# ut-vision/Rot-MVGaze

Hardware: AMD Instinct MI355X
Metric: multi-view samples/sec (fwd+bwd), BxVx3x224x224 (higher is better)
Workload: dtype f32; 1 GPU; C3: ResNet-50, V=4, B=128 per GPU, 3x224x224, fwd+loss+bwd; backbone=ResNet-50, views=4, batch_per_gpu=128, global_batch=128, image=3x224x224, parallelism=dp1, weights=random init, seed 0 (kaiming-normal convs, default Linear), rccl_ranks=1, step_launch=eager: every kernel queued from Python

## Files before the change

### include/rotmvgaze.h

```cpp
#ifndef ROTMVGAZE_H
#define ROTMVGAZE_H

#include <stddef.h>
#include <stdint.h>

#ifdef __cplusplus
extern "C" {
#endif

#define MVG_ABI_VERSION 10

int mvg_abi_version(void);
const char *mvg_last_error(void);
int mvg_device_cus(void);
int mvg_set_scratch(void *ptr, size_t bytes, void *stream);
size_t mvg_scratch_bytes(void);
void *mvg_stream_create_low_priority(void);
int mvg_set_reserved_cus(int n);

enum {
  MVG_K_CONV_FPROP = 0, MVG_K_CONV_DGRAD = 1, MVG_K_CONV_WGRAD = 2, MVG_K_WGRAD_REDUCE = 3,
  MVG_K_BN_FINALIZE = 4, MVG_K_BN_APPLY = 5, MVG_K_BN_BWD_REDUCE = 6, MVG_K_BN_BWD_APPLY = 7,
  MVG_K_POOL = 8, MVG_K_LAYOUT = 9, MVG_K_LINEAR_FPROP = 10, MVG_K_LINEAR_DGRAD = 11,
  MVG_K_LINEAR_WGRAD = 12, MVG_K_ROTCAT = 13, MVG_K_COLSUM = 14, MVG_K_LOSS = 15,
// ... 126 lines not shown
                           int inverse, void *stream);
int mvg_relative_rotation(const float *rot, const int32_t *vi, const int32_t *vj, float *rel,
                          int batch, int views, int dirs, void *stream);

int mvg_rotcat_fwd(const float *img_feat , const float *feat ,
                   const float *rel , const int32_t *view_of,
                   const int32_t *src_of, float *x , int batch, int dirs,
                   int cf, int nvec, void *stream);
int mvg_rotcat_bwd(const float *dx, const float *rel, const int32_t *src_of, float *dfeat, int batch,
                   int dirs, int cf, int nvec, void *stream);
int mvg_rotcat_ext_fwd(const float *img_feat, const float *feat, const float *rel_apply,
                       const float *rel_append, const int32_t *view_of, const int32_t *src_of,
                       float *x, int ld, int batch, int dirs, int cf, int nvec, void *stream);
int mvg_rotcat_ext_bwd(const float *dx, int ld, const float *rel, const int32_t *src_of, float *dfeat,
                       int batch, int dirs, int cf, int nvec, void *stream);
int mvg_ibn_scales(const float *a , const float *feat ,
                   const int32_t *view_of, const int32_t *src_of, float *running_mean, int training,
                   float momentum, float eps, float *scales, int batch, int dirs, int nvec,
                   void *stream);
int mvg_paircat_fwd(const float *a, const float *feat, const float *rel, const float *scales,
                    const int32_t *view_of, const int32_t *src_of, float *x, int batch, int dirs,
                    int nvec, void *stream);
int mvg_paircat_bwd(const float *dx, const float *rel, const float *scales, const int32_t *src_of,
                    float *da_dir, float *dfeat, int batch, int dirs, int nvec, void *stream);
int mvg_segment_sum(const float *x, int64_t row_stride, int width, const int32_t *seg_of, float *out,
                    int batch, int dirs, int segments, int accumulate, void *stream);

int mvg_axpby(const float *x, float *y, float a, float b, int64_t n, void *stream);
int mvg_scale_by(const float *x, const float *scale, float *out, int64_t n, void *stream);

int mvg_linear_skinny_fwd(const float *x, const float *w, const float *bias, float *y, int rows, int k,
                          int nout, void *stream);
int mvg_linear_skinny_bwd(const float *dy, const float *x, const float *w, const float *mask, float *dx,
                          float *dw, float *db, int rows, int k, int nout, int accumulate, float *dx_absmax, void *stream);

int mvg_adam_step(float *param, const float *grad, float *exp_avg, float *exp_avg_sq, int64_t n, float lr,
                  float beta1, float beta2, float eps, float weight_decay, int step, void *stream);
int mvg_adam_step_dev(float *param, const float *grad, float *exp_avg, float *exp_avg_sq, int64_t n, const float *lr_dev,
                      float *state3, float beta1, float beta2, float eps, float weight_decay, void *stream);

int mvg_gaze_angular_loss(const float *pred, const float *gt, int n, float row_weight,
                          float *loss, int accumulate, float *dpred, float *theta_out, void *stream);

int mvg_gaze_lp_loss(const float *pred, const float *label, int n, int p, float *loss, float *dpred, void *stream);
int mvg_gaze_angular_loss_multi(const float *pred, const float *gt, int iters, int dirs, int batch, const float *host_weights,
                                float *loss, float *dpred, void *stream);

int mvg_mt19937_seed(uint32_t *host_state , uint64_t seed);
int64_t mvg_pair_index_build(uint32_t *host_state, const int64_t *host_file_rows, int n_files,
                             int camera_tag, int64_t *host_out , int64_t capacity);


int mvg_cast_weights_bf16(const mvg_conv_desc *d, const float *w, int cin_src, void *w_krsc, void *w_crsk,
                          void *stream);
int mvg_conv_fprop_bf16(const mvg_conv_desc *d, const void *x, const void *wgt, void *y, const float *bias,
                        int relu, float *stats, void *stream);
int mvg_conv_stats_partials_bf16(const mvg_conv_desc *d, int32_t *out_rows_per_partial);
int mvg_conv_fprop_bf16_affine(const mvg_conv_desc *d, const void *x, const void *wgt, void *out, const float *scale,
                               const float *shift, const void *residual, int relu, void *stream);
int mvg_conv_dgrad_bf16(const mvg_conv_desc *d, const void *dy, const void *wgt_crsk, void *dx,
                        const void *mask, const void *addend, void *stream);
int mvg_conv_dgrad_bn_partials_bf16(const mvg_conv_desc *d);
int mvg_conv_dgrad_bf16_bnreduce(const mvg_conv_desc *d, const void *dy, const void *wgt_crsk, void *dx, const void *addend,
                                 const void *bn_y, const uint8_t *bn_bits, const float *bn_mean, const float *bn_invstd,
                                 const float *relu_scale, const float *relu_shift, float *partials, float *s1, float *s2,
                                 float *dgamma, float *dbeta, int accumulate, void *stream);
int mvg_stem_rowwindow_bf16(const float *x_nchw, void *xw, int64_t images, int h, int w, void *stream);
int mvg_stem_fprop_bf16(const mvg_conv_desc *d, const void *xw, const void *w_fold, void *y, float *stats, void *stream);
int mvg_stem_wgrad_splits_bf16(const mvg_conv_desc *d);
int mvg_stem_wgrad_bf16(const mvg_conv_desc *d, const void *xw, const void *dy, float *dw_fold, float *workspace, int splits,
                        int accumulate, void *stream);
int mvg_conv_wgrad_bf16(const mvg_conv_desc *d, const void *x, const void *dy, float *dw, float *workspace,
                        int splits, int accumulate, void *stream);
int mvg_conv_wgrad_splits_bf16(const mvg_conv_desc *d);
int mvg_conv_wgrad_bf16_slabs(const mvg_conv_desc *d, const void *x, const void *dy, float *workspace, int splits, void *stream);
int mvg_linear_fprop_mixed(const float *x, const void *w_bf16, const float *bias, int relu, float *y, int rows, int fin,
                           int fout, void *stream);
int mvg_linear_dgrad_mixed(const float *dy, const void *wt_bf16, const float *mask, const float *addend, float *dx,
                           int rows, int fin, int fout, void *stream);
int mvg_linear_wgrad_mixed(const float *x, const float *dy, float *dw, float *db, int rows, int fin, int fout,
                           float *workspace, int splits, int accumulate, void *stream);
int mvg_bn_apply_bf16(const uint16_t *y, const float *scale, const float *shift, const uint16_t *residual,
                      const float *res_scale, const float *res_shift, int relu, uint16_t *out, int groups,
                      int64_t rows_per_group, int c, void *stream);
int mvg_bn_bwd_reduce_bf16(const uint16_t *g, const uint16_t *act, const uint16_t *y, const float *mean,
                           const float *invstd, const float *relu_scale, const float *relu_shift, int groups,
                           int64_t rows_per_group, int c, float *s1, float *s2, float *dgamma, float *dbeta,
                           int accumulate, float *workspace, uint16_t *dz_out, void *stream);
int mvg_bn_bwd_apply_bf16(const uint16_t *g, const uint16_t *act, const uint16_t *y, const float *mean,
                          const float *invstd, const float *gamma, const float *s1, const float *s2,
                          const float *relu_scale, const float *relu_shift, int groups, int64_t rows_per_group,
                          int c, uint16_t *dy, uint16_t *dz_out, void *stream);
int mvg_bn_relu_maxpool_fwd_bf16(const uint16_t *y, const float *scale, const float *shift, uint16_t *pooled,
                                 uint8_t *argmax, int groups, int n_per_group, int h, int w, int c, int ho,
                                 int wo, void *stream);
int mvg_bn_relu_maxpool_bwd_reduce_bf16(const uint16_t *g_pooled, const uint8_t *argmax, const uint16_t *y,
                                        const float *mean, const float *invstd, const float *scale,
                                        const float *shift, int groups, int n_per_group, int h, int w, int c,
                                        int ho, int wo, float *s1, float *s2, float *dgamma, float *dbeta,
                                        int accumulate, float *workspace, void *stream);
int mvg_bn_relu_maxpool_bwd_apply_bf16(const uint16_t *g_pooled, const uint8_t *argmax, const uint16_t *y,
                                       const float *mean, const float *invstd, const float *gamma,
                                       const float *scale, const float *shift, const float *s1,
                                       const float *s2, int groups, int n_per_group, int h, int w, int c,
                                       int ho, int wo, uint16_t *dy, void *stream);
int mvg_avgpool_fwd_bf16(const uint16_t *x, float *y, int n, int hw, int c, void *stream);
int mvg_avgpool_bwd_bf16(const float *dy, uint16_t *dx, int n, int hw, int c, void *stream);
int mvg_nchw_to_nhwc8_bf16(const float *src, uint16_t *dst, int n, int c, int h, int w, void *stream);
int mvg_preprocess_u8hwc_resize_bf16(const uint8_t *src, uint16_t *dst, int n, int h, int w, int oh, int ow, float mean0,
                                     float mean1, float mean2, float std0, float std1, float std2, int swap_rb,
                                     void *stream);

int mvg_split_f32(const float *x, void *out_sp, int64_t n, float scale, void *stream);
int mvg_merge_sp(const void *x_sp, float *out, int64_t n, float inv_scale, void *stream);
int mvg_split_weights(const mvg_conv_desc *d, const float *w, void *w_krsc_sp, void *w_crsk_sp, float *stat2, void *items_dev,
                      void *stream);
int mvg_weights_prep_batch(const void *items_dev, int n, int mode, int blocks_per_item , void *stream);
int mvg_conv_stats_partials_split(const mvg_conv_desc *d, int32_t *rows_per_partial);
int mvg_conv_fprop_split(const mvg_conv_desc *d, const void *x_sp, const float *x_sinv, const void *w_sp, const float *w_sinv,
                         float *y, float *stats, void *stream);
int mvg_conv_fprop_split_affine(const mvg_conv_desc *d, const void *x_sp, const float *x_sinv, const void *w_sp, const float *w_sinv,
                                void *out, int out_sp, const float *scale, const float *shift, const void *residual,
                                int residual_sp, int relu, void *stream);
int mvg_conv_dgrad_split(const mvg_conv_desc *d, const void *dy_sp, const float *dy_sinv, const void *w_crsk_sp,
                         const float *w_sinv, float *dx, const float *addend, const void *relu_mask_sp, void *stream);
int mvg_bn_apply_split(const float *y, const float *scale, const float *shift, const void *residual, int residual_sp,
                       const float *res_scale, const float *res_shift, int relu, void *out_sp, uint8_t *relu_bits,
                       int groups, int64_t rows_per_group, int c, void *stream);
int mvg_bn_bwd_reduce_split(const float *g, const uint8_t *relu_bits, const float *y, const float *mean, const float *invstd,
                            const float *relu_scale, const float *relu_shift, int groups, int64_t rows_per_group, int c,
                            float *s1, float *s2, float *dgamma, float *dbeta, int accumulate, float *workspace,
                            float *dz_out, float *mx, const float *gamma, float *dy_sinv, void *stream);
int mvg_bn_bwd_apply_split(const float *g, const float *y, const float *mean, const float *invstd, const float *gamma,
                           const float *s1, const float *s2, const float *relu_scale, const float *relu_shift,
                           int groups, int64_t rows_per_group, int c, void *dy_sp, const float *mx, float *dy_sinv,
                           int dy_sinv_ready, void *stream);
int mvg_bn_relu_maxpool_fwd_split(const float *y, const float *scale, const float *shift, void *pooled_sp,
                                  uint8_t *argmax, int groups, int n_per_group, int h, int w, int c, int ho, int wo,
                                  void *stream);
int mvg_avgpool_fwd_split(const void *x_sp, float *y, int n, int hw, int c, void *stream);
int mvg_conv_dgrad_bn_partials_split(const mvg_conv_desc *d);
int mvg_conv_dgrad_split_bnreduce(const mvg_conv_desc *d, const void *dy_sp, const float *dy_sinv, const void *w_crsk_sp,
                                  const float *w_sinv, float *dx, const float *addend, const float *bn_y, const uint8_t *bn_bits,
                                  const float *bn_mean, const float *bn_invstd, const float *relu_scale, const float *relu_shift,
                                  float *partials, float *s1, float *s2, float *dgamma, float *dbeta, int accumulate,
                                  float *mx, const float *bn_gamma, float *dx_dy_sinv, void *stream);
int mvg_stem_rowwindow_split(const float *x_nhwc4, void *xw_sp, int64_t images, int h, int w, void *stream);
int mvg_stem_rowwindow_split_nchw(const float *x_nchw, void *xw_sp, int64_t images, int h, int w, void *stream);
int mvg_stem_fprop_split(const mvg_conv_desc *d, const void *xw_sp, const void *w_sp, const float *w_sinv, float *y, float *stats,
                         void *stream);
int mvg_stem_wgrad_splits_split(const mvg_conv_desc *d);
int mvg_stem_wgrad_split(const mvg_conv_desc *d, const void *xw_sp, const void *dy_sp, const float *dy_sinv, float *dw_rw,
                         float *workspace, int splits, int accumulate, void *stream);
int mvg_bn_relu_maxpool_bwd_reduce_split(const float *g_pooled, const uint8_t *argmax, const float *y, const float *mean,
                                         const float *invstd, const float *scale, const float *shift, int groups,
                                         int n_per_group, int h, int w, int c, int ho, int wo, float *s1, float *s2,
                                         float *dgamma, float *dbeta, int accumulate, float *workspace, float *mx, const float *gamma,
                                         float *dy_sinv, void *stream);
int mvg_bn_relu_maxpool_bwd_apply_split(const float *g_pooled, const uint8_t *argmax, const float *y, const float *mean,
                                        const float *invstd, const float *gamma, const float *scale, const float *shift,
                                        const float *s1, const float *s2, int groups, int n_per_group, int h, int w, int c,
                                        int ho, int wo, void *dy_sp, const float *mx, float *dy_sinv, int dy_sinv_ready, void *stream);
int mvg_conv_wgrad_splits_split(const mvg_conv_desc *d);
int mvg_conv_wgrad_split(const mvg_conv_desc *d, const void *x_sp, const void *dy_sp, const float *dy_sinv, float *dw,
                         float *workspace, int splits, int accumulate, void *stream);
int mvg_conv_wgrad_split_slabs(const mvg_conv_desc *d, const void *x_sp, const void *dy_sp, const float *dy_sinv, float *workspace,
                               int splits, void *stream);
int mvg_wgrad_reduce_batch(const float *const *host_slabs, float *const *host_dw, const int64_t *host_n, const int32_t *host_splits,
                           const int32_t *host_accumulate, int n, void *stream);

int mvg_absmax_multi(const float *const *host_ptrs, const int64_t *host_counts, float *const *host_out_slots, int n, void *stream);
int mvg_fuse_build_split(const float *img_feat, const float *feat, const float *rel, const int32_t *row_img, const int32_t *row_src_f,
                         const int32_t *row_src_h, void *xf_sp, void *xh_sp, const float *am_img, const float *am_feat,
                         float *xf_sinv, float *xh_sinv, int rows, int cf, int nvec, void *stream);
int mvg_fuse_unbuild(const float *dxh, const float *dxn, const float *rel, const int32_t *seg, const int32_t *vi, float *dfeat, float *da,
                     int da_accumulate, int segments, int views, int dirs, int batch, int cf, int nvec, float *absmax, void *stream);
int mvg_linear_fprop_split(int rows, int fin, int fout, const void *x_sp, const float *x_sinv, const void *w_sp, const float *w_sinv,
                           const float *bias, int relu, void *out, int out_sp, float *out_sinv, const float *bias_absmax,
                           float *out_absmax, void *stream);
int mvg_linear_dgrad_split(int rows, int fin, int fout, const void *dy_sp, const float *dy_sinv, const void *wt_sp, const float *w_sinv,
                           float *dx, const float *addend, const void *relu_mask_sp, float *out_absmax, void *stream);
int mvg_linear_wgrad_split(int rows, int fin, int fout, const void *x_sp, const float *x_sinv, const void *dy_sp, const float *dy_sinv,
                           float *dw, float *workspace, int splits, int accumulate, void *stream);
int mvg_split_colsum(const float *g, int rows, int cols, const float *absmax, void *out_sp, float *out_sinv, float *db, int accumulate,
                     void *stream);

#ifdef __cplusplus
}
#endif
#endif
```

### rot-mvgaze_amd/_lib.py

```python
from __future__ import annotations

import ctypes as C
import os

_HERE = os.path.dirname(os.path.abspath(__file__))
LIB_PATH = os.path.join(_HERE, "csrc", "librotmvgaze_hip.so")

K_FAMILIES = 18
ABI_VERSION = 10


class ConvDesc(C.Structure):
    _fields_ = [(n, C.c_int32) for n in
                ("groups", "n", "h", "w", "cin", "cout", "r", "s", "stride", "pad", "ho", "wo")]

    @classmethod
    def make(cls, groups, n, h, w, cin, cout, k, stride, pad):
        ho = (h + 2 * pad - k) // stride + 1
        wo = (w + 2 * pad - k) // stride + 1
        return cls(groups, n, h, w, cin, cout, k, k, stride, pad, ho, wo)

    @classmethod
    def linear(cls, rows, fin, fout):
        return cls(1, rows, 1, 1, fin, fout, 1, 1, 1, 0, 1, 1)


class ProfEntry(C.Structure):
    _fields_ = [("launches", C.c_int64), ("ms", C.c_double), ("flops", C.c_double), ("bytes", C.c_double)]


_P = C.c_void_p
_I = C.c_int
_I64 = C.c_int64
_F = C.c_float
_D = C.POINTER(ConvDesc)

SIGNATURES = {
    "mvg_abi_version": (_I, []),
    "mvg_last_error": (C.c_char_p, []),
    "mvg_device_cus": (_I, []),
    "mvg_set_scratch": (_I, [_P, C.c_size_t, _P]),
    "mvg_scratch_bytes": (C.c_size_t, []),
    "mvg_set_reserved_cus": (_I, [_I]),
    "mvg_stream_create_low_priority": (_P, []),
    "mvg_prof_enable": (_I, [_I]),
    "mvg_prof_reset": (_I, []),
    "mvg_prof_collect": (_I, [C.POINTER(ProfEntry)]),
    "mvg_prof_family_name": (C.c_char_p, [_I]),
    "mvg_conv_fprop": (_I, [_D, _P, _P, _P, _P, _I, _P, _P]),
    "mvg_conv_fprop_affine": (_I, [_D, _P, _P, _P, _P, _P, _P, _I, _P]),
    "mvg_conv_stats_partials": (_I, [_D, C.POINTER(C.c_int32)]),
    "mvg_conv_dgrad": (_I, [_D, _P, _P, _P, _P, _P, _P]),
    "mvg_conv_wgrad": (_I, [_D, _P, _P, _P, _P, _I, _I, _P]),
    "mvg_conv_wgrad_splits": (_I, [_D]),
    "mvg_linear_wgrad": (_I, [_P, _P, _P, _P, _I, _I, _I, _P, _I, _I, _P]),
    "mvg_fuser_fprop": (_I, [_P, _P, _P, _P, _P, _P, _P, _I, _P, _I, _I, _I, _I, _I, _I, _P, C.c_size_t, _P]),
    "mvg_fuser_wgrad": (_I, [_P, _P, _P, _P, _P, _P, _P, _P, _I, _I, _I, _I, _I, _I, _P, _I, _I, _P]),
    "mvg_linear_workspace_floats": (C.c_size_t, [_I, _I, _I]),
    "mvg_linear_fprop": (_I, [_P, _P, _P, _I, _P, _I, _I, _I, _P, C.c_size_t, _P]),
    "mvg_linear_dgrad": (_I, [_P, _P, _P, _P, _P, _I, _I, _I, _P, C.c_size_t, _P]),
    "mvg_bn_finalize": (_I, [_P, _I, _I, _I, _I64, _I, _P, _P, _P, _P, _F, _F, _P, _P, _P, _P, _P]),
    "mvg_bn_eval_affine": (_I, [_I, _I, _P, _P, _P, _P, _F, _P, _P, _P]),
    "mvg_bn_apply": (_I, [_P, _P, _P, _P, _P, _P, _I, _P, _I, _I64, _I, _P]),
    "mvg_bn_bwd_reduce": (_I, [_P, _P, _P, _P, _P, _P, _P, _I, _I64, _I, _P, _P, _P, _P, _I, _P, _P, _P]),
    "mvg_split_f32": (_I, [_P, _P, _I64, _F, _P]),
    "mvg_merge_sp": (_I, [_P, _P, _I64, _F, _P]),
    "mvg_split_weights": (_I, [_D, _P, _P, _P, _P, _P, _P]),
    "mvg_weights_prep_batch": (_I, [_P, _I, _I, _I, _P]),
    "mvg_conv_stats_partials_split": (_I, [_D, C.POINTER(C.c_int32)]),
    "mvg_conv_fprop_split": (_I, [_D, _P, _P, _P, _P, _P, _P, _P]),
    "mvg_conv_fprop_split_affine": (_I, [_D, _P, _P, _P, _P, _P, _I, _P, _P, _P, _I, _I, _P]),
    "mvg_conv_dgrad_split": (_I, [_D, _P, _P, _P, _P, _P, _P, _P, _P]),
    "mvg_bn_apply_split": (_I, [_P, _P, _P, _P, _I, _P, _P, _I, _P, _P, _I, _I64, _I, _P]),
    "mvg_bn_bwd_apply_split": (_I, [_P, _P, _P, _P, _P, _P, _P, _P, _P, _I, _I64, _I, _P, _P, _P, _I, _P]),
    "mvg_bn_bwd_reduce_split": (_I, [_P, _P, _P, _P, _P, _P, _P, _I, _I64, _I, _P, _P, _P, _P, _I, _P, _P, _P, _P, _P, _P]),
    "mvg_bn_relu_maxpool_fwd_split": (_I, [_P, _P, _P, _P, _P, _I, _I, _I, _I, _I, _I, _I, _P]),
    "mvg_avgpool_fwd_split": (_I, [_P, _P, _I, _I, _I, _P]),
    "mvg_stem_rowwindow_split": (_I, [_P, _P, _I64, _I, _I, _P]),
    "mvg_stem_rowwindow_split_nchw": (_I, [_P, _P, _I64, _I, _I, _P]),
    "mvg_stem_fprop_split": (_I, [_D, _P, _P, _P, _P, _P, _P]),
    "mvg_stem_wgrad_splits_split": (_I, [_D]),
    "mvg_stem_wgrad_split": (_I, [_D, _P, _P, _P, _P, _P, _I, _I, _P]),
    "mvg_bn_relu_maxpool_bwd_reduce_split": (_I, [_P, _P, _P, _P, _P, _P, _P, _I, _I, _I, _I, _I, _I, _I, _P, _P, _P, _P, _I, _P, _P, _P, _P, _P]),
    "mvg_bn_relu_maxpool_bwd_apply_split": (_I, [_P, _P, _P, _P, _P, _P, _P, _P, _P, _P, _I, _I, _I, _I, _I, _I, _I, _P, _P, _P, _I, _P]),
    "mvg_conv_dgrad_bn_partials_split": (_I, [_D]),
    "mvg_conv_dgrad_split_bnreduce": (_I, [_D, _P, _P, _P, _P, _P, _P, _P, _P, _P, _P, _P, _P, _P, _P, _P, _P, _P, _I, _P, _P, _P, _P]),
    "mvg_conv_wgrad_splits_split": (_I, [_D]),
    "mvg_conv_wgrad_split": (_I, [_D, _P, _P, _P, _P, _P, _I, _I, _P]),
    "mvg_conv_wgrad_split_slabs": (_I, [_D, _P, _P, _P, _P, _I, _P]),
    "mvg_wgrad_reduce_batch": (_I, [C.POINTER(C.c_void_p), C.POINTER(C.c_void_p), C.POINTER(C.c_int64), C.POINTER(C.c_int32),
                                    C.POINTER(C.c_int32), _I, _P]),
    "mvg_bn_apply_bits": (_I, [_P, _P, _P, _P, _P, _P, _P, _P, _I, _I64, _I, _P]),
    "mvg_bn_bwd_reduce_bits": (_I, [_P, _P, _P, _P, _P, _I, _I64, _I, _P, _P, _P, _P, _I, _P, _P, _P]),
    "mvg_bn_apply_bits_bf16": (_I, [_P, _P, _P, _P, _P, _P, _P, _P, _I, _I64, _I, _P]),
    "mvg_bn_bwd_reduce_bits_bf16": (_I, [_P, _P, _P, _P, _P, _I, _I64, _I, _P, _P, _P, _P, _I, _P, _P, _P]),
    "mvg_bn_bwd_workspace_floats": (C.c_size_t, [_I, _I64, _I]),
    "mvg_bn_bwd_apply": (_I, [_P, _P, _P, _P, _P, _P, _P, _P, _P, _P, _I, _I64, _I, _P, _P, _P]),
    "mvg_maxpool3x3s2_fwd": (_I, [_P, _P, _P, _I, _I, _I, _I, _I, _I, _P]),
    "mvg_maxpool3x3s2_bwd": (_I, [_P, _P, _P, _I, _I, _I, _I, _I, _I, _P]),
    "mvg_bn_relu_maxpool_fwd": (_I, [_P, _P, _P, _P, _P, _I, _I, _I, _I, _I, _I, _I, _P]),
    "mvg_bn_relu_maxpool_bwd_reduce": (_I, [_P, _P, _P, _P, _P, _P, _P, _I, _I, _I, _I, _I, _I, _I, _P, _P, _P, _P, _I, _P,
                                            _P]),
    "mvg_bn_relu_maxpool_bwd_apply": (_I, [_P, _P, _P, _P, _P, _P, _P, _P, _P, _P, _I, _I, _I, _I, _I, _I, _I, _P, _P]),
    "mvg_bn_eval_bwd": (_I, [_P, _P, _P, _P, _P, _P, _P, _P, _P, _F, _I, _I64, _I, _P, _P, _P, _P, _I, _P, _P]),
    "mvg_bn_eval_bwd_workspace_floats": (C.c_size_t, [_I, _I64, _I]),
    "mvg_bn_relu_maxpool_eval_bwd": (_I, [_P, _P, _P, _P, _P, _P, _P, _P, _F, _I, _I, _I, _I, _I, _I, _I, _P, _P, _P, _I, _P,
                                          _P]),
    "mvg_avgpool_fwd": (_I, [_P, _P, _I, _I, _I, _P]),
    "mvg_avgpool_bwd": (_I, [_P, _P, _I, _I, _I, _P]),
    "mvg_nchw_to_nhwc4": (_I, [_P, _P, _I, _I, _I, _I, _P]),
    "mvg_nhwc4_to_nchw": (_I, [_P, _P, _I, _I, _I, _I, _P]),
    "mvg_preprocess_u8hwc": (_I, [_P, _P, _I, _I, _I, _F, _F, _F, _F, _F, _F, _I, _P]),
    "mvg_gaze_lp_loss": (_I, [_P, _P, _I, _I, _P, _P, _P]),
    "mvg_preprocess_u8hwc_resize": (_I, [_P, _P, _I, _I, _I, _I, _I, _F, _F, _F, _F, _F, _F, _I, _P]),
    "mvg_multi_erase_nchw": (_I, [_P, _P, _P, _I, _I, _I, _I, _I, _P]),
    "mvg_rotation_matrix_2d": (_I, [_P, _P, _I, _I, _P]),
    "mvg_relative_rotation": (_I, [_P, _P, _P, _P, _I, _I, _I, _P]),
    "mvg_rotcat_fwd": (_I, [_P, _P, _P, _P, _P, _P, _I, _I, _I, _I, _P]),
    "mvg_rotcat_bwd": (_I, [_P, _P, _P, _P, _I, _I, _I, _I, _P]),
    "mvg_rotcat_ext_fwd": (_I, [_P, _P, _P, _P, _P, _P, _P, _I, _I, _I, _I, _I, _P]),
    "mvg_rotcat_ext_bwd": (_I, [_P, _I, _P, _P, _P, _I, _I, _I, _I, _P]),
    "mvg_ibn_scales": (_I, [_P, _P, _P, _P, _P, _I, _F, _F, _P, _I, _I, _I, _P]),
    "mvg_paircat_fwd": (_I, [_P, _P, _P, _P, _P, _P, _P, _I, _I, _I, _P]),
    "mvg_paircat_bwd": (_I, [_P, _P, _P, _P, _P, _P, _I, _I, _I, _P]),
    "mvg_segment_sum": (_I, [_P, _I64, _I, _P, _P, _I, _I, _I, _I, _P]),
    "mvg_axpby": (_I, [_P, _P, _F, _F, _I64, _P]),
    "mvg_scale_by": (_I, [_P, _P, _P, _I64, _P]),
    "mvg_linear_skinny_fwd": (_I, [_P, _P, _P, _P, _I, _I, _I, _P]),
    "mvg_linear_skinny_bwd": (_I, [_P, _P, _P, _P, _P, _P, _P, _I, _I, _I, _I, _P, _P]),
    "mvg_adam_step": (_I, [_P, _P, _P, _P, _I64, _F, _F, _F, _F, _F, _I, _P]),
    "mvg_gaze_angular_loss": (_I, [_P, _P, _I, _F, _P, _I, _P, _P, _P]),
    "mvg_gaze_angular_loss_multi": (_I, [_P, _P, _I, _I, _I, C.POINTER(C.c_float), _P, _P, _P]),
    "mvg_adam_step_dev": (_I, [_P, _P, _P, _P, _I64, _P, _P, _F, _F, _F, _F, _P]),
    "mvg_absmax_multi": (_I, [C.POINTER(C.c_void_p), C.POINTER(C.c_int64), C.POINTER(C.c_void_p), _I, _P]),
    "mvg_fuse_build_split": (_I, [_P, _P, _P, _P, _P, _P, _P, _P, _P, _P, _P, _P, _I, _I, _I, _P]),
    "mvg_fuse_unbuild": (_I, [_P, _P, _P, _P, _P, _P, _P, _I, _I, _I, _I, _I, _I, _I, _P, _P]),
    "mvg_linear_fprop_split": (_I, [_I, _I, _I, _P, _P, _P, _P, _P, _I, _P, _I, _P, _P, _P, _P]),
    "mvg_linear_dgrad_split": (_I, [_I, _I, _I, _P, _P, _P, _P, _P, _P, _P, _P, _P]),
    "mvg_linear_wgrad_split": (_I, [_I, _I, _I, _P, _P, _P, _P, _P, _P, _I, _I, _P]),
    "mvg_split_colsum": (_I, [_P, _I, _I, _P, _P, _P, _P, _I, _P]),
    "mvg_cast_weights_bf16": (_I, [_D, _P, _I, _P, _P, _P]),
    "mvg_conv_fprop_bf16": (_I, [_D, _P, _P, _P, _P, _I, _P, _P]),
    "mvg_conv_stats_partials_bf16": (_I, [_D, C.POINTER(C.c_int32)]),
    "mvg_conv_fprop_bf16_affine": (_I, [_D, _P, _P, _P, _P, _P, _P, _I, _P]),
    "mvg_conv_dgrad_bf16": (_I, [_D, _P, _P, _P, _P, _P, _P]),
    "mvg_conv_dgrad_bn_partials_bf16": (_I, [_D]),
    "mvg_conv_dgrad_bf16_bnreduce": (_I, [_D, _P, _P, _P, _P, _P, _P, _P, _P, _P, _P, _P, _P, _P, _P, _P, _I, _P]),
    "mvg_conv_wgrad_bf16": (_I, [_D, _P, _P, _P, _P, _I, _I, _P]),
    "mvg_stem_rowwindow_bf16": (_I, [_P, _P, _I64, _I, _I, _P]),
    "mvg_stem_fprop_bf16": (_I, [_D, _P, _P, _P, _P, _P]),
    "mvg_stem_wgrad_splits_bf16": (_I, [_D]),
    "mvg_stem_wgrad_bf16": (_I, [_D, _P, _P, _P, _P, _I, _I, _P]),
    "mvg_conv_wgrad_splits_bf16": (_I, [_D]),
    "mvg_conv_wgrad_bf16_slabs": (_I, [_D, _P, _P, _P, _I, _P]),
    "mvg_linear_fprop_mixed": (_I, [_P, _P, _P, _I, _P, _I, _I, _I, _P]),
    "mvg_linear_dgrad_mixed": (_I, [_P, _P, _P, _P, _P, _I, _I, _I, _P]),
    "mvg_linear_wgrad_mixed": (_I, [_P, _P, _P, _P, _I, _I, _I, _P, _I, _I, _P]),
    "mvg_bn_apply_bf16": (_I, [_P, _P, _P, _P, _P, _P, _I, _P, _I, _I64, _I, _P]),
    "mvg_bn_bwd_reduce_bf16": (_I, [_P, _P, _P, _P, _P, _P, _P, _I, _I64, _I, _P, _P, _P, _P, _I, _P, _P, _P]),
    "mvg_bn_bwd_apply_bf16": (_I, [_P, _P, _P, _P, _P, _P, _P, _P, _P, _P, _I, _I64, _I, _P, _P, _P]),
    "mvg_bn_relu_maxpool_fwd_bf16": (_I, [_P, _P, _P, _P, _P, _I, _I, _I, _I, _I, _I, _I, _P]),
    "mvg_bn_relu_maxpool_bwd_reduce_bf16": (_I, [_P, _P, _P, _P, _P, _P, _P, _I, _I, _I, _I, _I, _I, _I, _P, _P, _P, _P, _I,
                                                 _P, _P]),
    "mvg_bn_relu_maxpool_bwd_apply_bf16": (_I, [_P, _P, _P, _P, _P, _P, _P, _P, _P, _P, _I, _I, _I, _I, _I, _I, _I, _P, _P]),
    "mvg_avgpool_fwd_bf16": (_I, [_P, _P, _I, _I, _I, _P]),
    "mvg_avgpool_bwd_bf16": (_I, [_P, _P, _I, _I, _I, _P]),
    "mvg_nchw_to_nhwc8_bf16": (_I, [_P, _P, _I, _I, _I, _I, _P]),
    "mvg_preprocess_u8hwc_resize_bf16": (_I, [_P, _P, _I, _I, _I, _I, _I, _F, _F, _F, _F, _F, _F, _I, _P]),
    "mvg_mt19937_seed": (_I, [_P, C.c_uint64]),
    "mvg_pair_index_build": (_I64, [_P, _P, _I, _I, _P, _I64]),
}

_lib = None


def lib() -> C.CDLL:
    global _lib
    if _lib is not None:
        return _lib
    if not os.path.exists(LIB_PATH):
        raise RuntimeError(
            f"{LIB_PATH} not found: the HIP extension is required (python rot-mvgaze_amd/csrc/build.py); "
            "this package has no CPU fallback")
    try:
        l = C.CDLL(LIB_PATH, mode=C.RTLD_GLOBAL)
    except OSError as e:
        raise RuntimeError(f"failed to load {LIB_PATH}: {e}") from e
    for name, (res, args) in SIGNATURES.items():
        fn = getattr(l, name)
        fn.restype = res
        fn.argtypes = args
    if l.mvg_abi_version() != ABI_VERSION:
        raise RuntimeError(f"librotmvgaze_hip.so ABI {l.mvg_abi_version()} != binding ABI {ABI_VERSION}")
    _lib = l
    return l


def check(rc: int, what: str = "") -> None:
    if rc != 0:
        msg = lib().mvg_last_error()
        raise RuntimeError(f"librotmvgaze_hip {what} failed (rc={rc}): {msg.decode() if msg else '?'}")
```

### rot-mvgaze_amd/backbone.py

```python
from __future__ import annotations

import os
from typing import Callable, Dict, List, Optional

import torch

from . import ops
from ._lib import ConvDesc
from .arch import BackboneSpec, ConvSpec, backbone_spec

Tensor = torch.Tensor
BN_EPS, BN_MOMENTUM = 1e-5, 0.1
IMAGE_MEAN, IMAGE_STD = (0.485, 0.456, 0.406), (0.229, 0.224, 0.225)


class GradSink:

    def view(self, p: torch.nn.Parameter) -> Tensor:
        raise NotImplementedError

    def accumulate(self, p: torch.nn.Parameter) -> bool:
        raise NotImplementedError

    def publish(self, ps: List[torch.nn.Parameter]) -> None:
        raise NotImplementedError


class _Unit:
    __slots__ = ("spec", "desc", "x_in", "y", "out", "mean", "invstd", "relu", "rows", "w", "trained", "pool",
                 "relu_affine", "fused_s12", "relu_bits", "split", "stem_rw")

    def __init__(self):
        self.split = False
        self.stem_rw = False
        self.relu_bits = None
        self.fused_s12 = None


class Backbone:
    _guard_scale = 1
    _debug_units: Optional[list] = None

    def __init__(self, depth: int, params: Dict[str, Tensor], prefix: str = "_feat_extractor.0."):
        self.spec: BackboneSpec = backbone_spec(depth, prefix)
        self.p = params
        self.fc_dim = self.spec.fc_dim
        self.overlap_wgrad = True
        self.overlap_head = True
        self.wgrad_low_priority = True
        self.grad_streams: List[torch.cuda.Stream] = []
        self._wg_stream: Optional[torch.cuda.Stream] = None
        self._wg_low = True
        self.act_dtype = torch.float32
        self.relu_bits = True
        self.split = os.environ.get("MVG_SPLIT", "1") != "0"
        self.fuse_bn_split = True
        self.stem_rowwindow = True
        self.split_eval = True
        self.bf16_fold_eval = True
        self._wprep_infer_ok = False
        self._wk_cache: Dict[str, tuple] = {}
        self.batch_weight_prep = True
        self._wprep: Optional[Dict[str, tuple]] = None
        self._wprep_state = None
        self._wprep_versions = None
        self._wg_defer: Optional[list] = None
        self._split_now = self.split
        self._stem_rw = False
        self._stem_w8 = None

    @property
    def bf16(self) -> bool:
        return self.act_dtype == torch.bfloat16

    def _weight(self, c: ConvSpec) -> Tensor:
        w = self.p[c.name + ".weight"]
        if c.cin == 3:
            w4 = torch.zeros(c.cout, c.k, c.k, 4, dtype=torch.float32, device=w.device)
            w4[..., :3].copy_(w.detach().permute(0, 2, 3, 1))
            return w4
        assert w.is_contiguous(memory_format=torch.channels_last) or (c.k == 1 and w.is_contiguous()), \
            f"{c.name}.weight must be channels_last (KRSC)"
        return w.detach()

    def _prepare_weights(self, dev, reuse: bool = False) -> Dict[str, tuple]:
        mode = 0 if self.bf16 else 1
        stem_rw = self._stem_rw
        convs = [c for c in self.spec.all_convs() if not (mode == 1 and c.cin == 3 and not stem_rw)]
        key = (mode, stem_rw, str(dev), tuple(self.p[c.name + ".weight"].data_ptr() for c in convs))
        if self._wprep_state is None or self._wprep_state[0] != key:
            out, rows = {}, []
            wstat = torch.zeros(len(convs), 2, dtype=torch.float32, device=dev)
            self._stem_w8 = None
            for ci, c in enumerate(convs):
                wsrc = self.p[c.name + ".weight"]
                assert wsrc.is_contiguous(memory_format=torch.channels_last) or (c.k == 1 and wsrc.is_contiguous())
                rs = c.k * c.k
                if mode == 1 and c.cin == 3:
                    assert c.k == 7
                    self._stem_w8 = torch.zeros(c.cout, 7, 8, 4, dtype=torch.float32, device=dev)
                    wk = ops.sp_empty(c.cout, 7 * 32, device=dev)
                    wk.sinv = wstat[ci, 1:2]
                    out[c.name] = (wk, None)
                    rows.append([self._stem_w8.data_ptr(), wk.data_ptr(), 0, c.cout | (7 << 32), 32 | (32 << 32), wstat[ci].data_ptr()])
                    continue
                if mode == 0 and c.cin == 3 and stem_rw:
                    assert c.k == 7
                    self._stem_w8 = torch.zeros(2 * c.cout, 7, 16, 4, dtype=torch.float32, device=dev)
                    wk = torch.empty(2 * c.cout, 7, 1, 64, dtype=torch.bfloat16, device=dev)
                    out[c.name] = (wk, None)
                    rows.append([self._stem_w8.data_ptr(), wk.data_ptr(), 0, (2 * c.cout) | (7 << 32), 64 | (64 << 32), wstat[ci].data_ptr()])
                    continue
                if mode == 1:
                    wk = ops.sp_empty(c.cout, rs * c.cin, device=dev)
                    wt = ops.sp_empty(c.cin, rs * c.cout, device=dev)
                    wk.sinv = wt.sinv = wstat[ci, 1:2]
                    cin_pad = c.cin
                else:
                    cin_pad = 8 if c.cin == 3 else c.cin
                    wk = torch.empty(c.cout, c.k, c.k, cin_pad, dtype=torch.bfloat16, device=dev)
                    wt = None if c.cin == 3 else torch.empty(cin_pad, c.k, c.k, c.cout, dtype=torch.bfloat16, device=dev)
                out[c.name] = (wk, wt)
                rows.append([wsrc.data_ptr(), wk.data_ptr(), wt.data_ptr() if wt is not None else 0, c.cout | (rs << 32),
                             c.cin | (cin_pad << 32), wstat[ci].data_ptr()])
            table = torch.tensor(rows, dtype=torch.int64).to(dev)
            self._wprep_state = (key, out, table, len(rows), mode, wstat)
        elif (reuse and self._wprep_infer_ok and
              self._wprep_versions == tuple(self.p[c.name + ".weight"]._version for c in self.spec.all_convs())):
            return self._wprep_state[1]
        _, out, table, n, mode, wstat = self._wprep_state
        self._wprep_infer_ok = reuse
        if mode == 1:
            wstat.zero_()
            if self._stem_w8 is not None:
                self._stem_w8[:, :, 1:, :3].copy_(self.p[self.spec.stem.name + ".weight"].detach().permute(0, 2, 3, 1))
        elif self._stem_w8 is not None:
            wsrc, co = self.p[self.spec.stem.name + ".weight"].detach().permute(0, 2, 3, 1), self.spec.stem.cout
            self._stem_w8[:co, :, 1:8, :3].copy_(wsrc)
            self._stem_w8[co:, :, 3:10, :3].copy_(wsrc)
        ops.weights_prep_batch(table, n, mode)
        self._wprep_versions = tuple(self.p[c.name + ".weight"]._version for c in self.spec.all_convs())
        return out

    def invalidate_weight_cache(self):
        self._wk_cache.clear()
        self._wprep_infer_ok = False

    def bn_count_buffers(self) -> List[Tensor]:
        return [self.p[c.bn + ".num_batches_tracked"] for c in self.spec.all_convs()]

    def _unit_fwd(self, c: ConvSpec, x: Tensor, G: int, N: int, H: int, W: int, training: bool, relu: bool,
                  residual: Optional[Tensor], tape: Optional[list], pool: bool = False, residual_affine=None,
                  defer_apply: bool = False):
        bf = self.bf16
        cin = (8 if bf else 4) if c.cin == 3 else c.cin
        d = ConvDesc.make(G, N, H, W, cin, c.cout, c.k, c.stride, c.pad)
        dev = x.device
        sp_out = self._split_now and training and not bf
        sp_in = sp_out and c.cin != 3
        stem_rw = c.cin == 3 and self._stem_rw and (sp_out or bf)
        if (sp_in or bf or stem_rw) and self._wprep is not None:
            w, w_t = self._wprep[c.name]
        elif sp_in:
            wsrc = self.p[c.name + ".weight"].detach()
            assert wsrc.is_contiguous(memory_format=torch.channels_last) or (c.k == 1 and wsrc.is_contiguous())
            w, w_t = ops.split_weights(d, wsrc, need_transposed=tape is not None)
        elif bf:
            wsrc = self.p[c.name + ".weight"].detach()
            assert wsrc.is_contiguous(memory_format=torch.channels_last) or (c.k == 1 and wsrc.is_contiguous())
            w, w_t = ops.cast_weights_bf16(d, wsrc, c.cin, need_transposed=(tape is not None and c.cin != 3))
        else:
            w, w_t = self._weight(c), None
        y = torch.empty(G, N, d.ho, d.wo, c.cout, dtype=self.act_dtype, device=dev)
        rows = N * d.ho * d.wo
        gamma, beta = self.p[c.bn + ".weight"].detach(), self.p[c.bn + ".bias"].detach()
        rm, rv = self.p[c.bn + ".running_mean"], self.p[c.bn + ".running_var"]
        aff = torch.empty(4, G, c.cout, dtype=torch.float32, device=dev)
        mean, invstd, scale, shift = aff[0], aff[1], aff[2], aff[3]

        def fprop(stats_buf):
            if stem_rw and bf:
                ops.stem_fprop_bf16(d, x, w, y, stats_buf)
            elif stem_rw:
                ops.stem_fprop_split(d, x, w, y, stats_buf)
            elif sp_in:
                ops.conv_fprop_split(d, x, w, y, stats_buf)
            else:
                ops.conv_fprop(d, x, w, y, None, False, stats_buf)
        if training:
            if stem_rw and bf:
                P, rpp = ops.conv_stats_partials(ConvDesc.make(G, N, d.ho, d.wo // 2, 64, 2 * c.cout, 1, 1, 0), True)
                P *= 2
            elif stem_rw:
                P, rpp = ops.conv_stats_partials_split(ConvDesc.make(G, N, d.ho, d.wo, 32, c.cout, 1, 1, 0))
            else:
                P, rpp = ops.conv_stats_partials_split(d) if sp_in else ops.conv_stats_partials(d, bf)
            stats = torch.empty(G, P, 2, c.cout, dtype=torch.float32, device=dev)
            fprop(stats)
            ops.bn_finalize(stats, G, P, rpp, rows, c.cout, gamma, beta, rm, rv, BN_MOMENTUM, BN_EPS, mean, invstd,
                            scale, shift)
        elif tape is None and not bf:
            ops.bn_eval_affine(1, c.cout, gamma, beta, rm, rv, BN_EPS, scale[:1], shift[:1])
            sp_eval = self._split_now and self.split_eval
            if sp_eval and c.cin != 3:
                wsrc = self.p[c.name + ".weight"].detach()
                assert wsrc.is_contiguous(memory_format=torch.channels_last) or (c.k == 1 and wsrc.is_contiguous())
                hit = self._wk_cache.get(c.name)
                if hit is not None and hit[0] == wsrc.data_ptr() and hit[1] == wsrc._version:
                    wk = hit[2]
                else:
                    wk, _ = ops.split_weights(d, wsrc, need_transposed=False)
                    self._wk_cache[c.name] = (wsrc.data_ptr(), wsrc._version, wk)
                out = ops.sp_empty(G, N, d.ho, d.wo, c.cout, device=dev) if relu else y
                ops.conv_fprop_split_affine(d, x, wk, out, scale[0], shift[0], residual, relu)
                return out
            ops.conv_fprop_affine(d, x, w, y, scale[0], shift[0], residual, relu)
            if pool:
                pooled, am = self._pool_plain(y, G, N, d.ho, d.wo, c.cout)
                return (ops.split_f32(pooled), am) if sp_eval else (pooled, am)
            return y
        elif tape is None and bf and self.bf16_fold_eval and not pool:
            ops.bn_eval_affine(1, c.cout, gamma, beta, rm, rv, BN_EPS, scale[:1], shift[:1])
            ops.conv_fprop_bf16_affine(d, x, w, y, scale[0], shift[0], residual, relu)
            if self._debug_units is not None:
                self._debug_units.append((c.name, x, residual, y))
            return y
        else:
            fprop(None)
            ops.bn_eval_affine(G, c.cout, gamma, beta, rm, rv, BN_EPS, scale, shift)
        keep = tape is not None
        if defer_apply:
            assert not relu and residual is None and not pool
            if keep:
                u = _Unit()
                u.spec, u.desc, u.x_in, u.y, u.out, u.mean, u.invstd, u.relu, u.rows, u.w = \
                    c, d, x, y, None, mean, invstd, False, rows, (w_t if (bf or sp_in) else w)
                u.trained = training
                u.split = sp_in
                u.relu_affine = None
                tape.append(u)
            return y, (scale, shift)
        if pool:
            assert relu and residual is None
            hp, wp_ = (d.ho + 2 - 3) // 2 + 1, (d.wo + 2 - 3) // 2 + 1
            argmax = torch.empty(G, N, hp, wp_, c.cout, dtype=torch.uint8, device=dev)
            if sp_out:
                out = ops.sp_empty(G, N, hp, wp_, c.cout, device=dev)
                ops.bn_relu_maxpool_fwd_split(y, scale, shift, out, argmax, G, N, d.ho, d.wo, c.cout, hp, wp_)
            else:
                out = torch.empty(G, N, hp, wp_, c.cout, dtype=self.act_dtype, device=dev)
                ops.bn_relu_maxpool_fwd(y, scale, shift, out, argmax, G, N, d.ho, d.wo, c.cout, hp, wp_)
            if self._debug_units is not None and tape is None and not training:
                self._debug_units.append((c.name, x, y, out))
        elif sp_out:
            out = ops.sp_empty(G, N, d.ho, d.wo, c.cout, device=dev)
            bits = ops.bn_apply_split(y, scale, shift, residual, relu, out, G, rows, c.cout, residual_affine,
                                      want_bits=keep and relu and residual is not None)
        else:
            out = torch.empty_like(y) if keep else y
            bits = None
            if keep and relu and residual is not None and self.relu_bits:
                bits = ops.bn_apply_bits(y, scale, shift, residual, out, G, rows, c.cout, residual_affine)
            else:
                ops.bn_apply(y, scale, shift, residual, relu, out, G, rows, c.cout, residual_affine)
        if keep:
            u = _Unit()
            u.spec, u.desc, u.x_in, u.y, u.out, u.mean, u.invstd, u.relu, u.rows, u.w = \
                c, d, x, y, (None if pool else out), mean, invstd, relu, rows, (w_t if (bf or sp_in) else w)
            u.trained = training
            u.split = sp_in
            u.stem_rw = stem_rw
            u.relu_affine = (scale, shift) if (relu and residual is None and not pool) else None
            if pool:
                u.pool = (argmax, scale, shift, d.ho, d.wo, hp, wp_)
            else:
                u.relu_bits = bits
            tape.append(u)
        return (out, argmax) if pool else out

    @staticmethod
    def _pool_plain(a0: Tensor, G: int, N: int, h: int, w: int, c: int):
        hp, wp_ = (h + 2 - 3) // 2 + 1, (w + 2 - 3) // 2 + 1
        x = torch.empty(G, N, hp, wp_, c, dtype=torch.float32, device=a0.device)
        argmax = torch.empty(G, N, hp, wp_, c, dtype=torch.uint8, device=a0.device)
        ops.maxpool_fwd(a0, x, argmax, G * N, h, w, c, hp, wp_)
        return x, argmax

    def forward(self, imgs: List[Tensor], training: bool, keep_tape: bool, input_bgr: bool = False,
                input_size: Optional[int] = None, need_dimg: bool = False):
        V = len(imgs)
        raw = imgs[0].dtype == torch.uint8
        if raw:
            B, Hin, Win, C = imgs[0].shape
            H, W = (input_size, input_size) if input_size else (Hin, Win)
        else:
            B, C, H, W = imgs[0].shape
        assert C == 3
        dev = imgs[0].device
        if self.bf16 and raw and (training or keep_tape):
            raise NotImplementedError("raw uint8 input with the bf16 path is served for inference only (model.eval() under "
                                      "torch.no_grad()): for training steps normalise to fp32 NCHW first")
        biggest_view_elems = B * ((H + 3) // 4) * ((W + 3) // 4) * self.spec.blocks[0].convs[-1].cout
        self._split_now = self.split and 4 * biggest_view_elems * self._guard_scale < 0x7FFFFFF0
        if self.bf16:
            ho, wo = (H - 1) // 2 + 1, W // 2
            self._stem_rw = (self.stem_rowwindow and training and W % 4 == 0 and (B * ho * (wo // 2)) % 64 == 0 and self.batch_weight_prep
                             and self.spec.stem.k == 7)
        else:
            self._stem_rw = (self._split_now and self.stem_rowwindow and training and not need_dimg and W % 2 == 0
                             and self.batch_weight_prep and 32 * B * H * (W // 2) * 4 < 0x7FFFFFF0)
        direct = self._stem_rw and not raw
        if direct and self.bf16:
            x0 = torch.empty(V, B, H, W // 4, 64, dtype=self.act_dtype, device=dev)
        elif direct:
            x0 = ops.sp_empty(V, B, H, W // 2, 32, device=dev)
            x0.sinv = None
        else:
            x0 = torch.empty(V, B, H, W, 8 if self.bf16 else 4, dtype=self.act_dtype, device=dev)
        for v, im in enumerate(imgs):
            assert im.shape == imgs[0].shape and im.is_cuda and im.dtype == imgs[0].dtype
            if direct:
                assert im.dtype == torch.float32
                if self.bf16:
                    ops.stem_rowwindow_bf16(im.detach().contiguous(), x0[v])
                else:
                    ops.stem_rowwindow_split_nchw(im.detach().contiguous(), x0[v])
            elif self.bf16 and raw:
                ops.preprocess_u8hwc_resize_bf16(im.contiguous(), x0[v], B, Hin, Win, H, W, IMAGE_MEAN, IMAGE_STD, input_bgr)
            elif self.bf16:
                assert im.dtype == torch.float32
                ops.nchw_to_nhwc8_bf16(im.detach().contiguous(), x0[v], B, 3, H, W)
            elif raw:
                ops.preprocess_u8hwc_resize(im.contiguous(), x0[v], B, Hin, Win, H, W, IMAGE_MEAN, IMAGE_STD, input_bgr)
            else:
                assert im.dtype == torch.float32
                ops.nchw_to_nhwc4(im.detach().contiguous(), x0[v], B, 3, H, W)
        if self._stem_rw and not direct:
            x0 = ops.stem_rowwindow_split(x0)
        self._wprep = None
        if training:
            self.invalidate_weight_cache()
        if self.batch_weight_prep and (self.bf16 or (self._split_now and training)):
            self._wprep = self._prepare_weights(dev, reuse=self.bf16 and self.bf16_fold_eval and not training and not keep_tape)
        tape: Optional[dict] = {"units": [], "blocks": [], "V": V, "B": B} if keep_tape else None
        if keep_tape and self._wprep is not None:
            tape["wprep_versions"] = self._wprep_versions
        ulist = tape["units"] if keep_tape else None
        if training:
            torch._foreach_add_(self.bn_count_buffers(), V)
        s = self.spec
        x, argmax = self._unit_fwd(s.stem, x0, V, B, H, W, training, True, None, ulist, pool=True)
        Hc, Wc = x.shape[2], x.shape[3]
        for blk in s.blocks:
            first = len(ulist) if keep_tape else 0
            identity = x
            out = x
            h, w = Hc, Wc
            for c in blk.convs[:-1]:
                out = self._unit_fwd(c, out, V, B, h, w, training, True, None, ulist)
                h, w = out.shape[2], out.shape[3]
            ds_idx = None
            ident_affine = None
            if blk.downsample is not None:
                if training or keep_tape or (self.bf16 and not self.bf16_fold_eval):
                    identity, ident_affine = self._unit_fwd(blk.downsample, x, V, B, Hc, Wc, training, False, None, ulist,
                                                            defer_apply=True)
                else:
                    identity = self._unit_fwd(blk.downsample, x, V, B, Hc, Wc, training, False, None, ulist)
                ds_idx = len(ulist) - 1 if keep_tape else None
            out = self._unit_fwd(blk.convs[-1], out, V, B, h, w, training, True, identity, ulist,
                                 residual_affine=ident_affine)
            if keep_tape:
                n_main = len(blk.convs)
                idx = list(range(first, first + n_main - 1)) + [len(ulist) - 1]
                tape["blocks"].append((idx, ds_idx))
            x = out
            Hc, Wc = out.shape[2], out.shape[3]
        feat = torch.empty(V, B, self.fc_dim, dtype=torch.float32, device=dev)
        if x.dtype == torch.float16:
            ops.avgpool_fwd_split(x, feat, V * B, Hc * Wc, self.fc_dim)
        else:
            ops.avgpool_fwd(x, feat, V * B, Hc * Wc, self.fc_dim)
        if keep_tape:
            tape["final_hw"] = (Hc, Wc)
        return feat, tape

    def _bn_bwd(self, u: _Unit, g: Tensor, need_dz: bool, sink: GradSink):
        if not u.trained:
            return self._bn_bwd_eval(u, g, need_dz, sink)
        c = u.spec
        G = u.y.shape[0]
        gp, bp = self.p[c.bn + ".weight"], self.p[c.bn + ".bias"]
        if u.fused_s12 is not None and u.split:
            (s12, sinv), u.fused_s12 = u.fused_s12, None
            dy = ops.sp_empty(*u.y.shape, device=g.device)
            ops.bn_bwd_apply_split(g, u.y, u.mean, u.invstd, gp.detach(), s12[0], s12[1], G, u.rows, c.cout, dy, None, s12[2], sinv)
            return dy, (g if need_dz else None)
        if u.fused_s12 is not None:
            s12, u.fused_s12 = u.fused_s12, None
            dy = torch.empty_like(g) if need_dz else g
            ops.bn_bwd_apply(g, None, u.y, u.mean, u.invstd, gp.detach(), s12[0], s12[1], G, u.rows, c.cout, dy, None, None)
            return dy, (g if need_dz else None)
        s12 = torch.empty(3 if u.split else 2, G, c.cout, dtype=torch.float32, device=g.device)
        ra = u.relu_affine
        act = u.out if (u.relu and ra is None) else None
        acc = sink.accumulate(gp)
        assert acc == sink.accumulate(bp)
        if u.split:
            assert not (u.relu and ra is None) or u.relu_bits is not None
            sinv = torch.empty(1, dtype=torch.float32, device=g.device)
            if u.relu_bits is not None:
                ops.bn_bwd_reduce_split(g, u.relu_bits, u.y, u.mean, u.invstd, G, u.rows, c.cout, s12[0], s12[1], sink.view(gp),
                                        sink.view(bp), acc, s12[2], None, dz_out=g, gamma=gp.detach(), dy_sinv=sinv)
            else:
                ops.bn_bwd_reduce_split(g, None, u.y, u.mean, u.invstd, G, u.rows, c.cout, s12[0], s12[1], sink.view(gp),
                                        sink.view(bp), acc, s12[2], ra, gamma=gp.detach(), dy_sinv=sinv)
            dy = ops.sp_empty(*u.y.shape, device=g.device)
            ops.bn_bwd_apply_split(g, u.y, u.mean, u.invstd, gp.detach(), s12[0], s12[1], G, u.rows, c.cout, dy,
                                   None if u.relu_bits is not None else ra, s12[2], sinv)
            return dy, (g if need_dz else None)
        if need_dz:
            if u.relu_bits is not None:
                ops.bn_bwd_reduce_bits(g, u.relu_bits, u.y, u.mean, u.invstd, G, u.rows, c.cout, s12[0], s12[1], sink.view(gp),
                                       sink.view(bp), acc, dz_out=g)
            else:
                ops.bn_bwd_reduce(g, act, u.y, u.mean, u.invstd, G, u.rows, c.cout, s12[0], s12[1], sink.view(gp),
                                  sink.view(bp), acc, ra, dz_out=g)
            dy = torch.empty_like(g)
            ops.bn_bwd_apply(g, None, u.y, u.mean, u.invstd, gp.detach(), s12[0], s12[1], G, u.rows, c.cout, dy, None, None)
            return dy, g
        ops.bn_bwd_reduce(g, act, u.y, u.mean, u.invstd, G, u.rows, c.cout, s12[0], s12[1], sink.view(gp), sink.view(bp),
                          acc, ra)
        ops.bn_bwd_apply(g, act, u.y, u.mean, u.invstd, gp.detach(), s12[0], s12[1], G, u.rows, c.cout, g, None, ra)
        return g, None

    def _bn_bwd_eval(self, u: _Unit, g: Tensor, need_dz: bool, sink: GradSink):
        c = u.spec
        G = u.y.shape[0]
        gp, bp = self.p[c.bn + ".weight"], self.p[c.bn + ".bias"]
        rm, rv = self.p[c.bn + ".running_mean"], self.p[c.bn + ".running_var"]
        acc = sink.accumulate(gp)
        assert acc == sink.accumulate(bp)
        if u.relu_bits is not None:
            mask = {"relu_bits": u.relu_bits}
        elif u.relu_affine is not None:
            mask = {"relu_affine": u.relu_affine}
        elif u.relu:
            mask = {"act": u.out}
        else:
            mask = {}
        dy = torch.empty_like(g) if need_dz else g
        ops.bn_eval_bwd(g, u.y, gp.detach(), rm, rv, BN_EPS, G, u.rows, c.cout, dy, sink.view(gp), sink.view(bp), acc,
                        dz_out=g if need_dz else None, **mask)
        return dy, (g if need_dz else None)

    def _side(self, dev) -> "torch.cuda.Stream":
        if self._wg_stream is None or self._wg_stream.device != dev or self._wg_low != self.wgrad_low_priority:
            old = self._wg_stream if (self._wg_stream is not None and self._wg_stream.device == dev) else None
            self._wg_low = self.wgrad_low_priority
            try:
                if not self._wg_low:
                    raise RuntimeError
                self._wg_stream = ops.low_priority_stream(dev)
            except RuntimeError:
                self._wg_stream = torch.cuda.Stream(device=dev)
            if old is not None:
                self._wg_stream.wait_stream(old)
            self.grad_streams[:] = [self._wg_stream]
        return self._wg_stream

    def _conv_bwd(self, u: _Unit, dy: Tensor, need_dx: bool, addend: Optional[Tensor], sink: GradSink,
                  fuse_for: Optional[_Unit] = None):
        if self.overlap_wgrad and dy.is_cuda:
            side = self._side(dy.device)
            side.wait_stream(torch.cuda.current_stream())
            with torch.cuda.stream(side):
                self._wgrad(u, dy, sink)
            if getattr(dy, "sinv", None) is not None:
                dy.sinv.record_stream(side)
            dy.record_stream(side)
            u.x_in.record_stream(side)
        else:
            self._wgrad(u, dy, sink)
        dx = None
        if need_dx:
            dx = torch.empty(ops.sp_shape(u.x_in), dtype=torch.float32, device=dy.device) if u.split else torch.empty_like(u.x_in)
            self._dgrad(u, dy, dx, addend, fuse_for, sink)
        return dx

    def _wgrad(self, u: _Unit, dy: Tensor, sink: GradSink):
        c = u.spec
        wp = self.p[c.name + ".weight"]
        if u.split:
            ops.conv_wgrad_split(u.desc, u.x_in, dy, sink.view(wp), sink.accumulate(wp), defer=self._wg_defer)
        elif u.stem_rw and self.bf16:
            dw16 = torch.empty(2 * c.cout, 7, 16, 4, dtype=torch.float32, device=dy.device)
            ops.stem_wgrad_bf16(u.desc, u.x_in, dy, dw16, False)
            gv = sink.view(wp).permute(0, 2, 3, 1)
            if sink.accumulate(wp):
                gv.add_(dw16[:c.cout, :, 1:8, :3])
            else:
                gv.copy_(dw16[:c.cout, :, 1:8, :3])
            gv.add_(dw16[c.cout:, :, 3:10, :3])
        elif u.stem_rw:
            dw8 = torch.empty(c.cout, 7, 8, 4, dtype=torch.float32, device=dy.device)
            ops.stem_wgrad_split(u.desc, u.x_in, dy, dw8, False)
            gv = sink.view(wp).permute(0, 2, 3, 1)
            if sink.accumulate(wp):
                gv.add_(dw8[:, :, 1:, :3])
            else:
                gv.copy_(dw8[:, :, 1:, :3])
        elif c.cin == 3:
            dw4 = torch.empty(c.cout, c.k, c.k, u.desc.cin, dtype=torch.float32, device=dy.device)
            ops.conv_wgrad(u.desc, u.x_in, dy, dw4, False)
            gv = sink.view(wp).permute(0, 2, 3, 1)
            if sink.accumulate(wp):
                gv.add_(dw4[..., :3])
            else:
                gv.copy_(dw4[..., :3])
        else:
            ops.conv_wgrad(u.desc, u.x_in, dy, sink.view(wp), sink.accumulate(wp), defer=self._wg_defer if self.bf16 else None)

    def _flush_wgrad_reduces(self, dev):
        if not self._wg_defer:
            return
        if self.overlap_wgrad and dev.type == "cuda":
            with torch.cuda.stream(self._side(dev)):
                ops.wgrad_reduce_batch(self._wg_defer)
        else:
            ops.wgrad_reduce_batch(self._wg_defer)

    def _dgrad(self, u: _Unit, dy: Tensor, dx: Tensor, addend: Optional[Tensor], fuse_for: Optional[_Unit] = None,
               sink: Optional[GradSink] = None):
        U = fuse_for
        if (self.bf16 and U is not None and self.fuse_bn_split and u.spec.cin != 3 and u.desc.cin % 64 == 0 and u.desc.cout % 64 == 0
                and (not U.relu or U.relu_bits is not None or U.relu_affine is not None)):
            c = U.spec
            gp, bp = self.p[c.bn + ".weight"], self.p[c.bn + ".bias"]
            acc = sink.accumulate(gp)
            assert acc == sink.accumulate(bp)
            s12 = torch.empty(2, dx.shape[0], c.cout, dtype=torch.float32, device=dx.device)
            ops.conv_dgrad_bf16_bnreduce(u.desc, dy, u.w, dx, addend, U.y, U.relu_bits, U.mean, U.invstd,
                                         None if U.relu_bits is not None else U.relu_affine, s12[0], s12[1], sink.view(gp),
                                         sink.view(bp), acc)
            U.fused_s12 = s12
            return
        if u.split:
            if U is not None and U.split and self.fuse_bn_split:
                c = U.spec
                gp, bp = self.p[c.bn + ".weight"], self.p[c.bn + ".bias"]
                acc = sink.accumulate(gp)
                assert acc == sink.accumulate(bp)
                s12 = torch.empty(3, dx.shape[0], c.cout, dtype=torch.float32, device=dx.device)
                sinv = torch.empty(1, dtype=torch.float32, device=dx.device)
                ops.conv_dgrad_split_bnreduce(u.desc, dy, u.w, dx, addend, U.y, U.relu_bits, U.mean, U.invstd,
                                              None if U.relu_bits is not None else U.relu_affine, s12[0], s12[1], sink.view(gp),
                                              sink.view(bp), acc, s12[2], gp.detach(), sinv)
                U.fused_s12 = (s12, sinv)
                return
            ops.conv_dgrad_split(u.desc, dy, u.w, dx, addend)
            return
        ops.conv_dgrad(u.desc, dy, u.w, dx, None, addend)

    def backward(self, tape: dict, dfeat: Tensor, sink: GradSink, need_dimg: bool = False):
        V, B = tape["V"], tape["B"]
        units: List[_Unit] = tape["units"]
        if self.bf16 and not all(u.trained for u in units):
            raise NotImplementedError("backward through eval-mode BatchNorm (running statistics) is not implemented on the "
                                      "bf16 path: call model.train() for gradient steps, or use the fp32 model")
        Hc, Wc = tape["final_hw"]
        if need_dimg and self.bf16:
            raise NotImplementedError("d(loss)/d(img) is not produced by the bf16 path")
        if tape.get("wprep_versions") is not None and tape["wprep_versions"] != getattr(self, "_wprep_versions", None):
            raise RuntimeError("backward of a tape whose bf16 / sp weight copies were overwritten by a later forward with "
                               "DIFFERENT weights (forward, optimizer step, forward, then backward of the first call): "
                               "backward-data would run with the new weights.  Run backward before the weights change "
                               "(PyTorch raises its version-counter error in the same situation)")
        g = torch.empty(V, B, Hc, Wc, self.fc_dim, dtype=self.act_dtype, device=dfeat.device)
        ops.avgpool_bwd(dfeat.contiguous(), g, V * B, Hc * Wc, self.fc_dim)
        self._wg_defer = []
        P = self.p
        blocks = tape["blocks"]
        for bi in range(len(blocks) - 1, -1, -1):
            idx, ds_idx = blocks[bi]
            last = units[idx[-1]]
            prev_last = units[blocks[bi - 1][0][-1]] if bi > 0 else None
            done: List[torch.nn.Parameter] = []
            dy, dz = self._bn_bwd(last, g, True, sink)
            d = self._conv_bwd(last, dy, True, None, sink, fuse_for=units[idx[-2]])
            done += [P[last.spec.name + ".weight"], P[last.spec.bn + ".weight"], P[last.spec.bn + ".bias"]]
            last.y = last.out = None
            del dy
            for k in range(len(idx) - 2, -1, -1):
                u = units[idx[k]]
                dy, _ = self._bn_bwd(u, d, False, sink)
                if k == 0:
                    d = self._conv_bwd(u, dy, True, dz if ds_idx is None else None, sink,
                                       fuse_for=prev_last if ds_idx is None else None)
                else:
                    d = self._conv_bwd(u, dy, True, None, sink, fuse_for=units[idx[k - 1]])
                done += [P[u.spec.name + ".weight"], P[u.spec.bn + ".weight"], P[u.spec.bn + ".bias"]]
                u.y = u.out = None
            if ds_idx is not None:
                ud = units[ds_idx]
                dyd, _ = self._bn_bwd(ud, dz, False, sink)
                self._conv_bwd(ud, dyd, False, None, sink)
                self._dgrad(ud, dyd, d, d, prev_last, sink)
                done += [P[ud.spec.name + ".weight"], P[ud.spec.bn + ".weight"], P[ud.spec.bn + ".bias"]]
                ud.y = ud.out = None
            self._flush_wgrad_reduces(g.device)
            sink.publish(done)
            g = d
            if "debug" in tape:
                tape["debug"].append(g.clone())
        stem = units[0]
        argmax, scale, shift, H1, W1, Hp, Wp = stem.pool
        sc = stem.spec
        gp, bp = P[sc.bn + ".weight"], P[sc.bn + ".bias"]
        stem_sp = stem.stem_rw and not self.bf16
        s12 = torch.empty(3 if stem_sp else 2, V, sc.cout, dtype=torch.float32, device=g.device)
        acc = sink.accumulate(gp)
        assert acc == sink.accumulate(bp)
        if not stem.trained:
            dy = torch.empty_like(stem.y)
            ops.bn_relu_maxpool_eval_bwd(g, argmax, stem.y, scale, shift, gp.detach(), P[sc.bn + ".running_mean"],
                                         P[sc.bn + ".running_var"], BN_EPS, V, B, H1, W1, sc.cout, Hp, Wp, dy, sink.view(gp),
                                         sink.view(bp), acc)
        elif stem_sp:
            sinv = torch.empty(1, dtype=torch.float32, device=g.device)
            ops.bn_relu_maxpool_bwd_reduce_split(g, argmax, stem.y, stem.mean, stem.invstd, scale, shift, V, B, H1, W1, sc.cout, Hp, Wp,
                                                 s12[0], s12[1], sink.view(gp), sink.view(bp), acc, s12[2], gp.detach(), sinv)
            dy = ops.sp_empty(*stem.y.shape, device=g.device)
            ops.bn_relu_maxpool_bwd_apply_split(g, argmax, stem.y, stem.mean, stem.invstd, gp.detach(), scale, shift, s12[0], s12[1],
                                                V, B, H1, W1, sc.cout, Hp, Wp, dy, s12[2], sinv)
        else:
            ops.bn_relu_maxpool_bwd_reduce(g, argmax, stem.y, stem.mean, stem.invstd, scale, shift, V, B, H1, W1, sc.cout, Hp, Wp,
                                           s12[0], s12[1], sink.view(gp), sink.view(bp), acc)
            dy = torch.empty_like(stem.y)
            ops.bn_relu_maxpool_bwd_apply(g, argmax, stem.y, stem.mean, stem.invstd, gp.detach(), scale, shift, s12[0], s12[1],
                                          V, B, H1, W1, sc.cout, Hp, Wp, dy)
        dx0 = self._conv_bwd(stem, dy, need_dimg, None, sink)
        self._flush_wgrad_reduces(g.device)
        self._wg_defer = None
        sink.publish([P[stem.spec.name + ".weight"], P[stem.spec.bn + ".weight"], P[stem.spec.bn + ".bias"]])
        if self._wg_stream is not None and dy.is_cuda and (self.overlap_wgrad or not torch.cuda.is_current_stream_capturing()):
            torch.cuda.current_stream().wait_stream(self._wg_stream)
        if not need_dimg:
            return None
        H, W = dx0.shape[2], dx0.shape[3]
        outs = []
        for v in range(V):
            o = torch.empty(B, 3, H, W, dtype=torch.float32, device=dx0.device)
            ops.nhwc4_to_nchw(dx0[v], o, B, 3, H, W)
            outs.append(o)
        return outs
```

### rot-mvgaze_amd/csrc/conv_shared.h

```cpp
#pragma once
#include <stdlib.h>

#include "common.h"

namespace mvg {


typedef float f32x16 __attribute__((ext_vector_type(16)));
typedef unsigned int u32x4 __attribute__((ext_vector_type(4)));

__device__ __forceinline__ unsigned pred_off(unsigned off, bool ok) { return off | ((unsigned)(!ok) << 31); }
__device__ __forceinline__ float4 buf_ld16(__amdgpu_buffer_rsrc_t r, unsigned byte_off) {
  const u32x4 v = __builtin_amdgcn_raw_buffer_load_b128(r, byte_off, 0, 0);
  return make_float4(__uint_as_float(v.x), __uint_as_float(v.y), __uint_as_float(v.z), __uint_as_float(v.w));
}
__device__ __forceinline__ __amdgpu_buffer_rsrc_t make_rsrc(const void *base, long long bytes) {
  unsigned n = bytes > 0x7FFFFFF0ll ? 0x7FFFFFF0u : (bytes < 0 ? 0u : (unsigned)bytes);
  const unsigned long long b = (unsigned long long)base;
  const unsigned lo = __builtin_amdgcn_readfirstlane((unsigned)b);
  const unsigned hi = __builtin_amdgcn_readfirstlane((unsigned)(b >> 32));
  n = __builtin_amdgcn_readfirstlane(n);
  void *ub = (void *)(((unsigned long long)hi << 32) | lo);
  return __builtin_amdgcn_make_buffer_rsrc(ub, 0, (int)n, 0x00020000);
}

struct FastDiv {
  unsigned mul, sh1, sh2, d;
};
static FastDiv make_fastdiv(unsigned d) {
  FastDiv f;
  unsigned l = 0;
  while ((1ull << l) < d) ++l;
  f.mul = (unsigned)(((1ull << 32) * ((1ull << l) - d)) / d + 1);
  f.sh1 = l < 1 ? l : 1;
  f.sh2 = l > 0 ? l - 1 : 0;
  f.d = d;
  return f;
}
__device__ __forceinline__ unsigned fdiv(unsigned n, const FastDiv &f) {
  const unsigned t = __umulhi(f.mul, n);
  return (t + ((n - t) >> f.sh1)) >> f.sh2;
}

struct IgemmClass {
  int out_h, out_w;
  int ntaps, tap_ns, tap_r0, tap_s0;
  int ktotal;
  int cls_py, cls_px, cls_cy, cls_cx;
  int mtiles_per_group;
  long long rows_per_group;
  FastDiv tap_ns_div, ohw_div, ow_div;
  int korder;
  FastDiv per_div;
  long long unit0;
  int tile0;
  int KT;
  int part0;
};

struct IgemmParams {
  const float *a;
  const float *b;
  float *out;
  const float *bias;
  const float *scale;
  const float *mask;
  const float *addend;
  float *stats;
  int relu;
  int groups;
  int out_h, out_w;
  int src_h, src_w;
  int src_c;
  int src_c_shift;
  int ncols;
  int r, s, stride_shift, stride, pad;
  int ktotal;
  int cin;
  int rs;
  long long rows_per_group;
  long long src_img_stride;
  int imgs_per_group;
  int mtiles_per_group, ntiles;
  int ntaps, tap_ns, tap_r0, tap_s0, tap_step;
  int cls_step, cls_py, cls_px, cls_cy, cls_cx;
  int full_h, full_w;
  long long a_group_bytes;
  long long b_bytes;
  FastDiv tap_ns_div;
  FastDiv ohw_div, ow_div;
  int splits, ktiles_per_split;
  float *slab;
  int sk_tiles;
  int no_remap;
  int nt_out;
  int ncls;
  IgemmClass cls[4];
  int b_row_len;
  int stats_partials;
  const float *bn_y, *bn_mean, *bn_invstd, *bn_rscale, *bn_rshift;
  float *bn_part;
  int bn_parts;
  int addend_sp, out_sp, mask_sp;
  const float *a_sinv, *b_sinv;
  unsigned *out_absmax;
  float *out_sinv;
  const float *bias_absmax;
  int stride_w, pad_w;
  int stats_fold;
  int bn_part_rows;
  const unsigned char *bn_bits;
  const float *rc_feat, *rc_rel;
  const int *rc_row_img, *rc_row_src;
  int rc_cf, rc_nvec, rc_nvec_shift;
  long long rc_img_bytes, rc_feat_bytes;
};

__device__ __forceinline__ int xcd_remap(int orig, int nwg) {
  const int q = nwg >> 3, rr = nwg & 7, xcd = orig & 7;
  const int base = (xcd < rr) ? xcd * (q + 1) : rr * (q + 1) + (xcd - rr) * q;
  return base + (orig >> 3);
}


struct WgradParams {
  const float *x;
  const float *dy;
  float *out;
  int h, w, cin, cout, r, s, stride, pad, ho, wo;
  int ncols;
  long long pixels;
  long long pixels_per_split;
  long long x_bytes;
  int mtiles, ntiles;
  int accumulate;
  float *db;
  const float *rc_feat, *rc_rel;
  const int *rc_row_img, *rc_row_src;
  int rc_cf, rc_nvec;
  long long rc_img_bytes, rc_feat_bytes;
  FastDiv ohw_div, wo_div, cin_div, s_div;
  const float *dy_sinv;
  const float *x_sinv;
  int stride_w, pad_w;
};

static __global__ __launch_bounds__(256) void wgrad_reduce_kernel(const float *__restrict__ slabs, float *__restrict__ dw,
                                                           long long n4, int splits, int accumulate, int lanes) {
  __shared__ float4 sh[256];
  const int cols = 256 / lanes;
  const int c = threadIdx.x % cols, l = threadIdx.x / cols;
  const long long i = (long long)blockIdx.x * cols + c;
  float4 s = make_float4(0.f, 0.f, 0.f, 0.f);
  if (i < n4)
    for (int k = l; k < splits; k += lanes) {
      const float4 v = reinterpret_cast<const float4 *>(slabs)[(long long)k * n4 + i];
      s.x += v.x;
      s.y += v.y;
      s.z += v.z;
      s.w += v.w;
    }
  sh[threadIdx.x] = s;
  __syncthreads();
  if (l == 0 && i < n4) {
    float4 t = accumulate ? reinterpret_cast<const float4 *>(dw)[i] : make_float4(0.f, 0.f, 0.f, 0.f);
    for (int k = 0; k < lanes; ++k) {
      const float4 v = sh[k * cols + c];
      t.x += v.x;
      t.y += v.y;
      t.z += v.z;
      t.w += v.w;
    }
    reinterpret_cast<float4 *>(dw)[i] = t;
  }
}

static double alg_cin(const mvg_conv_desc *d) { return d->cin == 4 ? 3.0 : (double)d->cin; }

static int ilog2_exact(int v) {
  int s = 0;
  while ((1 << s) < v) ++s;
  return ((1 << s) == v) ? s : -1;
}

static int validate(const mvg_conv_desc *d) {
  MVG_REQUIRE(d != nullptr, "conv: null descriptor");
  MVG_REQUIRE(d->groups > 0 && d->n > 0 && d->h > 0 && d->w > 0 && d->cin > 0 && d->cout > 0, "conv: bad sizes");
  MVG_REQUIRE(d->stride == 1 || d->stride == 2, "conv: stride must be 1 or 2 (got %d)", d->stride);
  MVG_REQUIRE(d->ho == (d->h + 2 * d->pad - d->r) / d->stride + 1 && d->wo == (d->w + 2 * d->pad - d->s) / d->stride + 1,
              "conv: ho/wo inconsistent with h/w/pad/stride");
  MVG_REQUIRE(d->cin % 4 == 0, "conv: cin %% 4 != 0 (%d)", d->cin);
  if (d->r * d->s > 1) {
    MVG_REQUIRE(ilog2_exact(d->cin) >= 0 && ilog2_exact(d->cout) >= 0, "conv: r*s>1 needs power-of-two channels");
  }
  MVG_REQUIRE((long long)d->n * d->ho * d->wo < (1LL << 31) && (long long)d->n * d->h * d->w < (1LL << 31),
              "conv: rows per group overflow int32");
  return 0;
}

[[maybe_unused]] static int dgrad_bn_partials(const mvg_conv_desc *d, int bm) {
  int parts = 0;
  for (int py = 0; py < d->stride; ++py)
    for (int px = 0; px < d->stride; ++px) {
      const int sub_h = (d->h - py + d->stride - 1) / d->stride, sub_w = (d->w - px + d->stride - 1) / d->stride;
      if (sub_h > 0 && sub_w > 0) parts += ceil_div((long long)d->n * sub_h * sub_w, bm);
    }
  return parts;
}

static IgemmClass make_class(int n, int out_h, int out_w, int ntaps, int tap_ns, int tap_r0, int tap_s0, int src_c) {
  IgemmClass c;
  memset(&c, 0, sizeof(c));
  c.out_h = out_h;
  c.out_w = out_w;
  c.ntaps = ntaps;
  c.tap_ns = tap_ns;
  c.tap_r0 = tap_r0;
  c.tap_s0 = tap_s0;
  c.ktotal = ntaps * src_c;
  c.rows_per_group = (long long)n * out_h * out_w;
  c.tap_ns_div = make_fastdiv((unsigned)tap_ns);
  c.ohw_div = make_fastdiv((unsigned)(out_h * out_w));
  c.ow_div = make_fastdiv((unsigned)out_w);
  c.KT = c.ktotal > 0 ? ceil_div(c.ktotal, 16) : 1;
  c.korder = (ntaps > 1 && src_c % 32 == 0) ? 1 : 0;
  c.per_div = make_fastdiv((unsigned)(ntaps > 0 ? 2 * ntaps : 1));
  return c;
}

static int fprop_geometry(IgemmParams &p, const mvg_conv_desc *d, int a_elem, int b_elem, const char *what, int stride_w = -1,
                          int pad_w = -1) {
  p.groups = d->groups;
  p.out_h = d->ho;
  p.out_w = d->wo;
  p.src_h = d->h;
  p.src_w = d->w;
  p.src_c = d->cin;
  p.src_c_shift = (d->r * d->s > 1) ? ilog2_exact(d->cin) : 0;
  p.ncols = d->cout;
  p.r = d->r;
  p.s = d->s;
  p.rs = d->r * d->s;
  p.stride = d->stride;
  p.stride_shift = d->stride == 2 ? 1 : 0;
  p.pad = d->pad;
  p.stride_w = stride_w >= 0 ? stride_w : d->stride;
  p.pad_w = stride_w >= 0 ? pad_w : d->pad;
  p.ktotal = d->r * d->s * d->cin;
  p.b_row_len = p.ktotal;
  p.cin = d->cin;
  p.rows_per_group = (long long)d->n * d->ho * d->wo;
  p.src_img_stride = (long long)d->h * d->w * d->cin;
  p.imgs_per_group = d->n;
  p.ntaps = d->r * d->s;
  p.tap_ns = d->s;
  p.tap_step = 1;
  p.cls_step = 1;
  p.a_group_bytes = (long long)a_elem * d->n * p.src_img_stride;
  p.b_bytes = (long long)b_elem * d->cout * p.ktotal;
  MVG_REQUIRE(p.a_group_bytes < 0x7FFFFFF0ll && p.b_bytes < 0x7FFFFFF0ll, "%s: a group / the weights exceed 2 GiB", what);
  p.ncls = 1;
  p.cls[0] = make_class(d->n, d->ho, d->wo, p.ntaps, d->s, 0, 0, d->cin);
  p.tap_ns_div = p.cls[0].tap_ns_div;
  p.ohw_div = p.cls[0].ohw_div;
  p.ow_div = p.cls[0].ow_div;
  return 0;
}

static int dgrad_geometry(IgemmParams &p, const mvg_conv_desc *d, int a_elem, int b_elem, const char *what) {
  p.groups = d->groups;
  p.out_h = d->h;
  p.out_w = d->w;
  p.src_h = d->ho;
  p.src_w = d->wo;
  p.src_c = d->cout;
  p.src_c_shift = (d->r * d->s > 1) ? ilog2_exact(d->cout) : 0;
  p.ncols = d->cin;
  p.r = d->r;
  p.s = d->s;
  p.rs = d->r * d->s;
  p.stride = d->stride;
  p.stride_shift = d->stride == 2 ? 1 : 0;
  p.pad = d->pad;
  p.ktotal = d->r * d->s * d->cout;
  p.b_row_len = p.ktotal;
  p.cin = d->cin;
  p.src_img_stride = (long long)d->ho * d->wo * d->cout;
  p.imgs_per_group = d->n;
  p.full_h = d->h;
  p.full_w = d->w;
  p.a_group_bytes = (long long)a_elem * d->n * p.src_img_stride;
  p.b_bytes = (long long)b_elem * d->cin * p.b_row_len;
  MVG_REQUIRE(p.a_group_bytes < 0x7FFFFFF0ll && p.b_bytes < 0x7FFFFFF0ll, "%s: a group / the weights exceed 2 GiB", what);
  return 0;
}

static __global__ __launch_bounds__(256) void dgrad_empty_class_kernel(uint4 *__restrict__ dx, const uint4 *__restrict__ addend,
                                                                       long long n, int sub_h, int sub_w, int full_h, int full_w,
                                                                       int cv, int py, int px) {
  const long long stride = (long long)gridDim.x * blockDim.x;
  for (long long i = (long long)blockIdx.x * blockDim.x + threadIdx.x; i < n; i += stride) {
    const int cc = (int)(i % cv);
    long long t = i / cv;
    const int x2 = (int)(t % sub_w);
    t /= sub_w;
    const int y2 = (int)(t % sub_h);
    const long long img = t / sub_h;
    const long long off = ((img * full_h + 2 * y2 + py) * full_w + 2 * x2 + px) * cv + cc;
    dx[off] = addend ? addend[off] : make_uint4(0u, 0u, 0u, 0u);
  }
}

static int dgrad_classes(IgemmParams &p, const mvg_conv_desc *d, bool keep_tapless, int dx_elem, void *dx, const void *addend,
                         hipStream_t st) {
  const int step = d->stride;
  p.ncls = 0;
  for (int py = 0; py < step; ++py)
    for (int px = 0; px < step; ++px) {
      const int sub_h = (d->h - py + step - 1) / step, sub_w = (d->w - px + step - 1) / step;
      if (sub_h <= 0 || sub_w <= 0) continue;
      const int r0 = (py + d->pad) % step, s0 = (px + d->pad) % step;
      const int nr = r0 < d->r ? (d->r - r0 + step - 1) / step : 0;
      const int ns = s0 < d->s ? (d->s - s0 + step - 1) / step : 0;
      if (nr * ns == 0 && !keep_tapless) {
        if (addend != dx || !addend) {
          const int cv = d->cin * dx_elem / 16;
          const long long n = (long long)d->groups * d->n * sub_h * sub_w * cv;
          long long blocks = (n + 255) / 256;
          if (blocks > 4096) blocks = 4096;
          hipLaunchKernelGGL(dgrad_empty_class_kernel, dim3((unsigned)blocks), dim3(256), 0, st, (uint4 *)dx, (const uint4 *)addend, n,
                             sub_h, sub_w, d->h, d->w, cv, py, px);
          if (check_launch("dgrad(empty class)")) return 1;
        }
        continue;
      }
      IgemmClass &c = p.cls[p.ncls++];
      c = make_class(d->n, sub_h, sub_w, nr * ns, ns > 0 ? ns : 1, r0, s0, d->cout);
      c.cls_py = py;
      c.cls_px = px;
      c.cls_cy = (py + d->pad - r0) / step;
      c.cls_cx = (px + d->pad - s0) / step;
      if (p.ncls == 1) {
        p.tap_step = step;
        p.cls_step = step;
        p.rows_per_group = c.rows_per_group;
        p.ktotal = c.ktotal;
        p.out_h = sub_h;
        p.out_w = sub_w;
      }
    }
  for (int i = 1; i < p.ncls; ++i)
    for (int j = i; j > 0 && p.cls[j].ktotal > p.cls[j - 1].ktotal; --j) {
      const IgemmClass t = p.cls[j];
      p.cls[j] = p.cls[j - 1];
      p.cls[j - 1] = t;
    }
  p.no_remap = p.ncls > 1;
  return 0;
}

static int wgrad_geometry(WgradParams &p, const mvg_conv_desc *d, int elem, int px_align, float *dw, float *db, float *workspace,
                          int splits, int accumulate, const char *what, int stride_w = -1, int pad_w = -1) {
  MVG_REQUIRE(splits >= 1, "%s: splits < 1", what);
  MVG_REQUIRE(splits == 1 || workspace != nullptr, "%s: workspace required for splits > 1", what);
  p.h = d->h;
  p.w = d->w;
  p.cin = d->cin;
  p.cout = d->cout;
  p.r = d->r;
  p.s = d->s;
  p.stride = d->stride;
  p.pad = d->pad;
  p.stride_w = stride_w >= 0 ? stride_w : d->stride;
  p.pad_w = stride_w >= 0 ? pad_w : d->pad;
  p.ho = d->ho;
  p.wo = d->wo;
  p.ncols = d->r * d->s * d->cin;
  p.pixels = (long long)d->groups * d->n * d->ho * d->wo;
  p.pixels_per_split = ((p.pixels + splits - 1) / splits + px_align - 1) / px_align * px_align;
  p.x_bytes = (long long)elem * d->groups * d->n * d->h * d->w * d->cin;
  p.ohw_div = make_fastdiv((unsigned)(d->ho * d->wo));
  p.wo_div = make_fastdiv((unsigned)d->wo);
  p.cin_div = make_fastdiv((unsigned)d->cin);
  p.s_div = make_fastdiv((unsigned)d->s);
  MVG_REQUIRE(p.pixels_per_split * d->cout * elem < 0x7FFFFFF0ll, "%s: split too large for 32-bit offsets", what);
  MVG_REQUIRE((long long)elem * (p.pixels_per_split / (d->ho * d->wo) + 2) * d->h * d->w * d->cin < 0x7FFFFFF0ll,
              "%s: split too large for 32-bit offsets", what);
  p.out = splits == 1 ? dw : workspace;
  p.accumulate = (splits == 1) ? accumulate : 0;
  p.db = db ? (splits == 1 ? db : workspace + (size_t)splits * d->cout * p.ncols) : nullptr;
  return 0;
}

static int wgrad_reduce_slabs(const WgradParams &p, float *workspace, float *dw, float *db, int splits, int accumulate, hipStream_t st,
                              const char *what) {
  const long long n = (long long)p.cout * p.ncols;
  MVG_REQUIRE(n % 4 == 0, "%s: weight elements %% 4 != 0", what);
  ProfScope ps(MVG_K_WGRAD_REDUCE, st, 0.0, 4.0 * n * (splits + 1));
  const int lanes = splits >= 32 ? 16 : (splits >= 8 ? 4 : 1);
  const long long blocks = (n / 4 + 256 / lanes - 1) / (256 / lanes);
  hipLaunchKernelGGL(wgrad_reduce_kernel, dim3((unsigned)blocks), dim3(256), 0, st, workspace, dw, n / 4, splits, accumulate, lanes);
  if (check_launch("wgrad_reduce")) return 1;
  if (!db) return 0;
  const long long nb = p.cout;
  const long long bblocks = (nb / 4 + 256 / lanes - 1) / (256 / lanes);
  hipLaunchKernelGGL(wgrad_reduce_kernel, dim3((unsigned)bblocks), dim3(256), 0, st, workspace + (size_t)splits * n, db, nb / 4, splits,
                     accumulate, lanes);
  return check_launch("wgrad_reduce(bias)");
}

static int wgrad_split_count(long long tiles, long long pixels, int workgroups_per_cu, int min_pixels) {
  long long want = ((long long)workgroups_per_cu * compute_cus()) / tiles;
  long long maxs = pixels / min_pixels;
  if (maxs < 1) maxs = 1;
  if (want > maxs) want = maxs;
  if (want < 1) want = 1;
  if (want > 1024) want = 1024;
  return (int)want;
}

}
```

### rot-mvgaze_amd/csrc/conv_split.hip

```cpp
#include "bf16_tile.h"
#include "elem.h"

namespace mvg {

typedef _Float16 f16x8 __attribute__((ext_vector_type(8)));

#define SPLIT_ONE(PA, PB, av, bv, acc)                                                                         \
  _Pragma("unroll") for (int i = 0; i < TM; ++i) _Pragma("unroll") for (int j = 0; j < TN; ++j)                \
      acc[i][j] = __builtin_amdgcn_mfma_f32_32x32x16_f16(av[PA][i], bv[PB][j], acc[i][j], 0, 0, 0);
#define SPLIT_PRODUCTS(av, bv, acc) SPLIT_ONE(0, 1, av, bv, acc) SPLIT_ONE(1, 0, av, bv, acc) SPLIT_ONE(0, 0, av, bv, acc)

constexpr int SP_BM = 128, SP_BK = 32;

__global__ __launch_bounds__(256) void split_f32_kernel(const float4 *__restrict__ x, uint4 *__restrict__ out, long long n8, float scale) {
  const long long stride = (long long)gridDim.x * 256;
  for (long long i = (long long)blockIdx.x * 256 + threadIdx.x; i < n8; i += stride) {
    const float4 lo = x[2 * i], hi = x[2 * i + 1];
    const float v[8] = {lo.x * scale, lo.y * scale, lo.z * scale, lo.w * scale, hi.x * scale, hi.y * scale, hi.z * scale, hi.w * scale};
    uint4 q1, q2;
    split2_chunk(v, q1, q2);
    out[2 * i] = q1;
    out[2 * i + 1] = q2;
  }
}
// ... 88 lines not shown
      if (i < nk) {
        const float4 *src = reinterpret_cast<const float4 *>(w + i * 8);
        const float4 lo = src[0], hi = src[1];
        v[0] = lo.x; v[1] = lo.y; v[2] = lo.z; v[3] = lo.w; v[4] = hi.x; v[5] = hi.y; v[6] = hi.z; v[7] = hi.w;
        dst = wk + SP_NP * i;
      } else {
        const long long j = i - nk;
        const int o8 = (int)(j % o8n);
        const long long t = j / o8n;
        const int tap = (int)(t % rs), c = (int)(t / rs);
#pragma unroll
        for (int k = 0; k < 8; ++k) v[k] = w[((long long)(o8 * 8 + k) * rs + tap) * cin + c];
        dst = wt + SP_NP * j;
      }
#pragma unroll
      for (int k = 0; k < 8; ++k) v[k] *= scale;
      uint4 q1, q2;
      split2_chunk(v, q1, q2);
      dst[0] = q1;
      dst[1] = q2;
    }
    if (tiled) {
      const int tc = cin / 64, ntiles = (cout / 64) * tc;
      for (int t = blockIdx.x; t < ntiles; t += gridDim.x) {
        const int o0 = (t / tc) * 64, c0 = (t % tc) * 64;
        __syncthreads();
#pragma unroll
        for (int ps = 0; ps < 4; ++ps) {
          const int r = (threadIdx.x >> 4) + 16 * ps, cq = threadIdx.x & 15;
          const float4 x = *reinterpret_cast<const float4 *>(w + (long long)(o0 + r) * cin + c0 + 4 * cq);
          tile[r][4 * cq] = x.x;
          tile[r][4 * cq + 1] = x.y;
          tile[r][4 * cq + 2] = x.z;
          tile[r][4 * cq + 3] = x.w;
        }
        __syncthreads();
#pragma unroll
        for (int q = 0; q < 2; ++q) {
          const int idx = threadIdx.x + 256 * q, cl = idx >> 3, o8 = idx & 7;
          float v[8];
#pragma unroll
          for (int k = 0; k < 8; ++k) v[k] = tile[o8 * 8 + k][cl] * scale;
          uint4 q1, q2;
          split2_chunk(v, q1, q2);
          uint4 *dst = wt + SP_NP * ((long long)(c0 + cl) * o8n + (o0 >> 3) + o8);
          dst[0] = q1;
          dst[1] = q2;
        }
      }
    }
    return;
  }
  unsigned short *wk = reinterpret_cast<unsigned short *>(it.wk), *wt = reinterpret_cast<unsigned short *>(it.wt);
  const int cin_pad = it.cin_pad;
  const long long total = (long long)cout * rs * cin_pad;
  if (rs == 1 && cin == cin_pad && (cin % 64) == 0 && (cout % 64) == 0) {
    uint4 *wk4 = reinterpret_cast<uint4 *>(wk);
    for (long long i = (long long)blockIdx.x * 256 + threadIdx.x; i < total / 8; i += (long long)gridDim.x * 256) {
      const float4 lo = reinterpret_cast<const float4 *>(w + i * 8)[0], hi = reinterpret_cast<const float4 *>(w + i * 8)[1];
      wk4[i] = make_uint4(bf16_pack2(lo.x, lo.y), bf16_pack2(lo.z, lo.w), bf16_pack2(hi.x, hi.y), bf16_pack2(hi.z, hi.w));
    }
    if (wt) {
      const int tc = cin / 64, ntiles = (cout / 64) * tc;
      for (int t = blockIdx.x; t < ntiles; t += gridDim.x) {
        const int o0 = (t / tc) * 64, c0 = (t % tc) * 64;
        __syncthreads();
#pragma unroll
        for (int ps = 0; ps < 4; ++ps) {
          const int r = (threadIdx.x >> 4) + 16 * ps, cq = threadIdx.x & 15;
          const float4 x = *reinterpret_cast<const float4 *>(w + (long long)(o0 + r) * cin + c0 + 4 * cq);
          tile[r][4 * cq] = x.x;
          tile[r][4 * cq + 1] = x.y;
          tile[r][4 * cq + 2] = x.z;
          tile[r][4 * cq + 3] = x.w;
        }
        __syncthreads();
#pragma unroll
        for (int q = 0; q < 2; ++q) {
          const int idx = threadIdx.x + 256 * q, cl = idx >> 3, o8 = idx & 7;
          float v[8];
#pragma unroll
          for (int k = 0; k < 8; ++k) v[k] = tile[o8 * 8 + k][cl];
          *reinterpret_cast<uint4 *>(wt + (long long)(c0 + cl) * cout + o0 + o8 * 8) =
              make_uint4(bf16_pack2(v[0], v[1]), bf16_pack2(v[2], v[3]), bf16_pack2(v[4], v[5]), bf16_pack2(v[6], v[7]));
        }
      }
    }
    return;
  }
  for (long long i = (long long)blockIdx.x * 256 + threadIdx.x; i < total; i += (long long)gridDim.x * 256) {
    const int c = (int)(i % cin_pad);
    const long long t = i / cin_pad;
    const int tap = (int)(t % rs), o = (int)(t / rs);
    const float v = c < cin ? w[((long long)o * rs + tap) * cin + c] : 0.f;
    const __bf16 b = (__bf16)v;
    const unsigned short u = __builtin_bit_cast(unsigned short, b);
    wk[i] = u;
    if (wt) wt[((long long)c * rs + tap) * cout + o] = u;
  }
}

typedef float f32x4 __attribute__((ext_vector_type(4)));

#define SPLIT16_ONE(PA, PB)                                                                       \
  _Pragma("unroll") for (int i = 0; i < TM; ++i) _Pragma("unroll") for (int j = 0; j < TN; ++j)   \
      acc[i][j] = __builtin_amdgcn_mfma_f32_16x16x32_f16(av[PA][i], bv[PB][j], acc[i][j], 0, 0, 0);

__device__ __forceinline__ int sp_row_swz(int R) { return ((R >> 1) & 1) | (((R >> 2) & 1) << 2); }

template <int BN, bool DGRAD, bool LIN = false, int WGM = 2, int STAGES = 1>
__global__ __launch_bounds__(256, STAGES == 2 ? 2 : (DGRAD || WGM == 4) ? 3 : 4) void igemm_split16_kernel(IgemmParams p) {
  constexpr int BM = 64 * WGM, WGN = 4 / WGM, NW = 4;
  static_assert(WGM == 2 || (WGM == 4 && BN == 64), "tiles: 128 x BN (2 x 2 waves) or 256 x 64 (4 x 1)");
  static_assert(STAGES == 1 || STAGES == 2, "one LDS stage, or the two-stage pipeline");
  constexpr int WTM = BM / WGM, WTN = BN / WGN;
  constexpr int TM = WTM / 16, TN = WTN / 16;
  constexpr int SLOTS = 4 * SP_NP;
  constexpr int ROWB = 16 * SLOTS, ROWS = BM + BN, STAGE_B = ROWS * ROWB;
  constexpr int NQ = ROWS * SLOTS / 64;
  constexpr int QA = BM * SLOTS / 64;
  constexpr int A_PER = QA / NW, B_PER = (NQ - QA) / NW;
  static_assert(QA % NW == 0 && (NQ - QA) % NW == 0, "whole instructions per wave");
  constexpr int EPI_B = bf16_epilogue_bytes<BM, BN, WGM, DGRAD>();
  constexpr int INFO_OFF = STAGES * STAGE_B > EPI_B ? STAGES * STAGE_B : EPI_B;
  constexpr int SMEM_B = INFO_OFF + BM * 8;
  __shared__ __attribute__((aligned(16))) unsigned char smem[SMEM_B];

  const int tid = threadIdx.x;
  const int lane = tid & 63, wave = __builtin_amdgcn_readfirstlane(tid >> 6);
  const int wm = wave / WGN, wn = wave % WGN;
  const int nwg = gridDim.x;
  const int wg_all = p.no_remap ? (int)blockIdx.x : xcd_remap(blockIdx.x, nwg);
  int ci = 0;
  for (int i = 1; i < p.ncls; ++i) ci += wg_all >= p.cls[i].tile0;
  const IgemmClass &c = p.cls[ci];
  const int wg = wg_all - c.tile0;
  const int ntile = wg % p.ntiles;
  const int mt_all = wg / p.ntiles;
  const int g = mt_all / c.mtiles_per_group;
  const int mtile = mt_all - g * c.mtiles_per_group;
  const int KT = c.KT;
  const int ohw = c.out_h * c.out_w;

  uint2 *rowinfo = reinterpret_cast<uint2 *>(smem + INFO_OFF);
  if (tid < BM) {
    const long long m = (long long)mtile * BM + tid;
    const bool ok = m < c.rows_per_group;
    const int mm = ok ? (int)m : 0;
    const int img = (int)fdiv((unsigned)mm, c.ohw_div);
    const int rem = mm - img * ohw;
    const int oy = (int)fdiv((unsigned)rem, c.ow_div), ox = rem - oy * c.out_w;
    const int y0 = DGRAD ? oy + c.cls_cy : oy * p.stride - p.pad;
    const int x0 = DGRAD ? ox + c.cls_cx : ox * p.stride_w - p.pad_w;
    const unsigned base = (unsigned)(img * p.src_img_stride * SP_BYTES) + (unsigned)((y0 * p.src_w + x0) * p.src_c) * (unsigned)SP_BYTES;
    unsigned msk = 0;
    for (int t = 0; t < c.ntaps; ++t) {
      const int fr = (int)fdiv((unsigned)t, c.tap_ns_div), fs = t - fr * c.tap_ns;
      const int iy = DGRAD ? y0 - fr : y0 + fr;
      const int ix = DGRAD ? x0 - fs : x0 + fs;
      msk |= (unsigned)(((unsigned)iy < (unsigned)p.src_h) & ((unsigned)ix < (unsigned)p.src_w)) << t;
    }
    rowinfo[tid] = make_uint2(base, ok ? msk : 0u);
  }
  __syncthreads();
  unsigned a_base[A_PER], a_vmask[A_PER], b_base[B_PER];
#pragma unroll
  for (int i = 0; i < A_PER; ++i) {
    const int sl = (wave + NW * i) * 64 + lane;
    const int row = sl / SLOTS, j = (sl % SLOTS) ^ sp_row_swz(row);
    const uint2 ri = rowinfo[row];
    a_base[i] = ri.x + 16u * (unsigned)j;
    a_vmask[i] = ri.y;
  }
#pragma unroll
  for (int i = 0; i < B_PER; ++i) {
    const int sl = (wave + NW * (A_PER + i)) * 64 + lane - BM * SLOTS;
    const int row = sl / SLOTS, j = (sl % SLOTS) ^ sp_row_swz(row);
    const int n = ntile * BN + row;
    b_base[i] = pred_off(((unsigned)n * (unsigned)p.b_row_len) * (unsigned)SP_BYTES + 16u * (unsigned)j, n < p.ncols);
  }
  const __amdgpu_buffer_rsrc_t rs_a =
      make_rsrc(reinterpret_cast<const char *>(p.a) + (long long)g * p.imgs_per_group * p.src_img_stride * SP_BYTES, p.a_group_bytes);
  const __amdgpu_buffer_rsrc_t rs_b = make_rsrc(p.b, p.b_bytes);
  typedef __attribute__((address_space(3))) void *lds_vp;

  auto issue = [&](int kt, int stage_off) {
    int kstart = kt * SP_BK;
    if (c.korder) {
      const int cblk = (int)fdiv((unsigned)kt, c.per_div), rem = kt - cblk * c.ntaps;
      kstart = (rem << p.src_c_shift) + cblk * SP_BK;
    }
    const int ks = __builtin_amdgcn_readfirstlane(kstart);
    const int tap_u = c.ntaps > 1 ? (ks >> p.src_c_shift) : 0;
    const int chb = ks - (tap_u << p.src_c_shift);
    const int fru = (int)fdiv((unsigned)tap_u, c.tap_ns_div), fsu = tap_u - fru * c.tap_ns;
    const int disp = (fru * p.src_w + fsu) * p.src_c;
    const unsigned sdelta = (unsigned)(((DGRAD ? -disp : disp) + chb) * SP_BYTES);
    unsigned kb = (unsigned)ks * (unsigned)SP_BYTES;
    if (DGRAD) {
      const int btap = (c.tap_r0 + p.tap_step * fru) * p.s + c.tap_s0 + p.tap_step * fsu;
      kb = (unsigned)(btap * p.src_c + chb) * (unsigned)SP_BYTES;
    }
#pragma unroll
    for (int i = 0; i < A_PER; ++i) {
      const bool ok = ((a_vmask[i] >> tap_u) & 1u) != 0u;
      __builtin_amdgcn_raw_ptr_buffer_load_lds(rs_a, (lds_vp)(smem + stage_off + (wave + NW * i) * 1024), 16, (int)pred_off(a_base[i] + sdelta, ok), 0, 0, 0);
    }
#pragma unroll
    for (int i = 0; i < B_PER; ++i)
      __builtin_amdgcn_raw_ptr_buffer_load_lds(rs_b, (lds_vp)(smem + stage_off + (wave + NW * (A_PER + i)) * 1024), 16, (int)(b_base[i] + kb), 0, 0, 0);
  };

  f32x4 acc[TM][TN];
#pragma unroll
  for (int i = 0; i < TM; ++i)
#pragma unroll
    for (int j = 0; j < TN; ++j)
#pragma unroll
      for (int e = 0; e < 4; ++e) acc[i][j][e] = 0.f;

  const int cc_l = lane >> 4;
  int a_off[TM][SP_NP], b_off[TN][SP_NP];
#pragma unroll
  for (int i = 0; i < TM; ++i) {
    const int R = wm * WTM + i * 16 + (lane & 15);
#pragma unroll
    for (int pc = 0; pc < SP_NP; ++pc) a_off[i][pc] = R * ROWB + (((2 * cc_l + pc) ^ sp_row_swz(R)) << 4);
  }
#pragma unroll
  for (int j = 0; j < TN; ++j) {
    const int R = wn * WTN + j * 16 + (lane & 15);
#pragma unroll
    for (int pc = 0; pc < SP_NP; ++pc) b_off[j][pc] = (BM + R) * ROWB + (((2 * cc_l + pc) ^ sp_row_swz(R)) << 4);
  }

  auto load_frags = [&](const unsigned char *stage, f16x8 (&av)[SP_NP][TM], f16x8 (&bv)[SP_NP][TN]) {
#pragma unroll
    for (int pc = 0; pc < SP_NP; ++pc) {
#pragma unroll
      for (int i = 0; i < TM; ++i) av[pc][i] = *reinterpret_cast<const f16x8 *>(stage + a_off[i][pc]);
#pragma unroll
      for (int j = 0; j < TN; ++j) bv[pc][j] = *reinterpret_cast<const f16x8 *>(stage + b_off[j][pc]);
    }
  };
  auto products = [&](const f16x8 (&av)[SP_NP][TM], const f16x8 (&bv)[SP_NP][TN]) { SPLIT16_ONE(0, 1) SPLIT16_ONE(1, 0) SPLIT16_ONE(0, 0) };
  if constexpr (STAGES == 1) {
    for (int kt = 0; kt < KT; ++kt) {
      issue(kt, 0);
      asm volatile("s_waitcnt vmcnt(0)" ::: "memory");
      __syncthreads();
      {
        f16x8 av[SP_NP][TM], bv[SP_NP][TN];
        load_frags(smem, av, bv);
        products(av, bv);
      }
      __syncthreads();
    }
  } else {
    constexpr int G = A_PER + B_PER;
    if (KT > 0) issue(0, 0);
    if (KT > 1) {
      issue(1, STAGE_B);
      asm volatile("s_waitcnt vmcnt(%0)\n\ts_barrier" ::"n"(G) : "memory");
    } else {
      asm volatile("s_waitcnt vmcnt(0)\n\ts_barrier" ::: "memory");
    }
    f16x8 a0[SP_NP][TM], b0[SP_NP][TN], a1[SP_NP][TM], b1[SP_NP][TN];
    load_frags(smem, a0, b0);
    int cur = 0;
    auto step = [&](int kt, const f16x8 (&ca)[SP_NP][TM], const f16x8 (&cb)[SP_NP][TN], f16x8 (&na)[SP_NP][TM], f16x8 (&nb)[SP_NP][TN]) {
      if (kt + 1 < KT) {
        asm volatile("s_waitcnt vmcnt(0) lgkmcnt(0)\n\ts_barrier" ::: "memory");
        if (kt + 2 < KT) issue(kt + 2, cur);
        cur ^= STAGE_B;
        load_frags(smem + cur, na, nb);
      }
      products(ca, cb);
    };
    for (int kt = 0; kt < KT; kt += 2) {
      step(kt, a0, b0, a1, b1);
      if (kt + 1 < KT) step(kt + 1, a1, b1, a0, b0);
    }
    __syncthreads();
  }
  bf16_epilogue<BM, BN, WGM, DGRAD, true, WGM, true, DGRAD, LIN, WGN>(p, c, acc, reinterpret_cast<unsigned short *>(smem), tid, g, mtile, ntile);
}

template <int BM, int BN, bool INCR>
__global__ __launch_bounds__(256, BN >= 256 ? 2 : 3) void wgrad_split_kernel(WgradParams p) {
  constexpr int BK = 16, WGM = 2, WGN = 2;
  constexpr int WTM = BM / WGM, WTN = BN / WGN;
  constexpr int TM = WTM / 32, TN = WTN / 32;
  constexpr int LDA = BM + 32, LDB = BN + 32;
  constexpr int MV = BM / 8, NVB = BN / 8;
  constexpr int A_TPR = 256 / BK;
  constexpr int A_CPT = MV / A_TPR > 0 ? MV / A_TPR : 1;
  constexpr int B_CPT = (NVB + A_TPR - 1) / A_TPR;
  constexpr int A_ELEMS = BK * LDA, B_ELEMS = BK * LDB;
  constexpr int STAGE = SP_NP * (A_ELEMS + B_ELEMS);
  __shared__ __attribute__((aligned(16))) unsigned short smem[2 * STAGE];

  const int tid = threadIdx.x;
  const int lane = tid & 63, wave = tid >> 6;
  const int wm = wave / WGN, wn = wave % WGN;
  const int li = lane & 31, lh = lane >> 5;
  const int tiles = p.mtiles * p.ntiles;
  const int logical = xcd_remap(blockIdx.x, gridDim.x);
  const int split = logical / tiles;
  const int tile = logical - split * tiles;
  const int ntile = tile % p.ntiles, mtile = tile / p.ntiles;
  const long long m_begin = (long long)split * p.pixels_per_split;
  long long m_end = m_begin + p.pixels_per_split;
  if (m_end > p.pixels) m_end = p.pixels;
  const int m_count = m_end > m_begin ? (int)(m_end - m_begin) : 0;
  const int ohw = p.ho * p.wo;
  const long long img0 = m_begin / ohw;
  const unsigned rem0 = (unsigned)(m_begin - img0 * ohw);

  const char *dy = reinterpret_cast<const char *>(p.dy);
  const char *x = reinterpret_cast<const char *>(p.x);
  const __amdgpu_buffer_rsrc_t rs_a = make_rsrc(dy + m_begin * p.cout * SP_BYTES, (long long)SP_BYTES * m_count * p.cout);
  const long long x_img_elems = (long long)p.h * p.w * p.cin;
  const __amdgpu_buffer_rsrc_t rs_b = make_rsrc(x + img0 * x_img_elems * SP_BYTES, p.x_bytes - (long long)SP_BYTES * img0 * x_img_elems);
  const int i_row = tid / A_TPR, i_v0 = tid % A_TPR;
  unsigned a_off[A_CPT];
  bool a_on[A_CPT];
#pragma unroll
  for (int j = 0; j < A_CPT; ++j) {
    const int cv = i_v0 + j * A_TPR;
    const int col = mtile * BM + cv * 8;
    a_on[j] = cv < MV;
    a_off[j] = (a_on[j] && col < p.cout) ? (unsigned)(i_row * p.cout + col) * (unsigned)SP_BYTES : 0x80000000u;
  }
  int i_dy[B_CPT], i_dx[B_CPT];
  unsigned i_tconst[B_CPT];
  bool i_cok[B_CPT], b_on[B_CPT];
#pragma unroll
  for (int j = 0; j < B_CPT; ++j) {
    const int cv = i_v0 + j * A_TPR;
    const int col = ntile * BN + cv * 8;
    b_on[j] = cv < NVB;
    i_cok[j] = b_on[j] && col < p.ncols;
    const int tap = (int)fdiv((unsigned)(i_cok[j] ? col : 0), p.cin_div);
    const int cc = (i_cok[j] ? col : 0) - tap * p.cin;
    const int fr = (int)fdiv((unsigned)tap, p.s_div), fs = tap - fr * p.s;
    i_dy[j] = fr - p.pad;
    i_dx[j] = fs - p.pad_w;
    i_tconst[j] = (unsigned)((i_dy[j] * p.w + i_dx[j]) * p.cin + cc) * (unsigned)SP_BYTES;
  }
  const unsigned row_bytes = (unsigned)(p.stride * p.w * p.cin) * (unsigned)SP_BYTES, col_bytes = (unsigned)(p.stride_w * p.cin) * (unsigned)SP_BYTES;
  const unsigned img_bytes = (unsigned)x_img_elems * (unsigned)SP_BYTES;
  int s_oy = 0, s_ox = 0;
  unsigned s_imgoff = 0;
  if (INCR) {
    const unsigned pix = rem0 + (unsigned)i_row;
    const unsigned img = fdiv(pix, p.ohw_div);
    const unsigned rem = pix - img * (unsigned)ohw;
    const unsigned oy = fdiv(rem, p.wo_div);
    s_oy = (int)oy;
    s_ox = (int)(rem - oy * (unsigned)p.wo);
    s_imgoff = img * img_bytes;
  }
  u32x4 a_reg[A_CPT][SP_NP], b_reg[B_CPT][SP_NP];
  auto load_tiles = [&](int kt) {
#pragma unroll
    for (int j = 0; j < A_CPT; ++j) {
#pragma unroll
      for (int pc = 0; pc < SP_NP; ++pc)
        a_reg[j][pc] = __builtin_amdgcn_raw_buffer_load_b128(rs_a, a_off[j] + 16u * pc, 0, 0);
      a_off[j] += (unsigned)(BK * p.cout) * (unsigned)SP_BYTES;
    }
    const bool mok = kt * BK + i_row < m_count;
    int oy, ox;
    unsigned imgoff;
    if constexpr (INCR) {
      oy = s_oy;
      ox = s_ox;
      imgoff = s_imgoff;
    } else {
      const unsigned pix = rem0 + (unsigned)(kt * BK + i_row);
      const unsigned img = fdiv(pix, p.ohw_div);
      const unsigned rem = pix - img * (unsigned)ohw;
      const unsigned uy = fdiv(rem, p.wo_div);
      oy = (int)uy;
      ox = (int)(rem - uy * (unsigned)p.wo);
      imgoff = img * img_bytes;
    }
    const int iy0 = oy * p.stride, ix0 = ox * p.stride_w;
    const unsigned pixoff = imgoff + (unsigned)oy * row_bytes + (unsigned)ox * col_bytes;
#pragma unroll
    for (int j = 0; j < B_CPT; ++j) {
      const bool ok = mok & i_cok[j] & ((unsigned)(iy0 + i_dy[j]) < (unsigned)p.h) & ((unsigned)(ix0 + i_dx[j]) < (unsigned)p.w);
#pragma unroll
      for (int pc = 0; pc < SP_NP; ++pc)
        b_reg[j][pc] = __builtin_amdgcn_raw_buffer_load_b128(rs_b, pred_off(pixoff + i_tconst[j] + 16u * pc, ok), 0, 0);
    }
    if constexpr (INCR) {
      unsigned nx = (unsigned)s_ox + BK;
      const unsigned q = fdiv(nx, p.wo_div);
      nx -= q * (unsigned)p.wo;
      s_ox = (int)nx;
      const int noy = s_oy + (int)q;
      const bool wrap = noy >= p.ho;
      s_oy = wrap ? noy - p.ho : noy;
      s_imgoff += wrap ? img_bytes : 0u;
    }
  };
  auto store_tiles = [&](int buf) {
    unsigned short *As = smem + buf * STAGE;
    unsigned short *Bs = As + SP_NP * A_ELEMS;
#pragma unroll
    for (int j = 0; j < A_CPT; ++j)
      if (a_on[j]) {
#pragma unroll
        for (int pc = 0; pc < SP_NP; ++pc)
          *reinterpret_cast<u32x4 *>(As + pc * A_ELEMS + i_row * LDA + (i_v0 + j * A_TPR) * 8) = a_reg[j][pc];
      }
#pragma unroll
    for (int j = 0; j < B_CPT; ++j)
      if (b_on[j]) {
#pragma unroll
        for (int pc = 0; pc < SP_NP; ++pc)
          *reinterpret_cast<u32x4 *>(Bs + pc * B_ELEMS + i_row * LDB + (i_v0 + j * A_TPR) * 8) = b_reg[j][pc];
      }
  };

  f32x16 acc[TM][TN];
#pragma unroll
  for (int i = 0; i < TM; ++i)
#pragma unroll
    for (int j = 0; j < TN; ++j)
#pragma unroll
      for (int e = 0; e < 16; ++e) acc[i][j][e] = 0.f;

  const int KT = (m_count + BK - 1) / BK;
  load_tiles(0);
  store_tiles(0);
  load_tiles(1);
  __syncthreads();
  for (int kt = 0; kt < KT; ++kt) {
    const int cur = kt & 1;
    store_tiles(cur ^ 1);
    load_tiles(kt + 2);
    const unsigned short *As = smem + cur * STAGE;
    const unsigned short *Bs = As + SP_NP * A_ELEMS;
    f16x8 av[SP_NP][TM], bv[SP_NP][TN];
#pragma unroll
    for (int pc = 0; pc < SP_NP; ++pc) {
#pragma unroll
      for (int i = 0; i < TM; ++i) av[pc][i] = __builtin_bit_cast(f16x8, tr_frag(As + pc * A_ELEMS, LDA, 0, wm * WTM + i * 32, lane));
#pragma unroll
      for (int j = 0; j < TN; ++j) bv[pc][j] = __builtin_bit_cast(f16x8, tr_frag(Bs + pc * B_ELEMS, LDB, 0, wn * WTN + j * 32, lane));
    }
    SPLIT_PRODUCTS(av, bv, acc)
    __syncthreads();
  }

  float *out = p.out + (long long)split * p.cout * p.ncols;
  const float osc = (p.dy_sinv ? *p.dy_sinv : 1.f) * (p.x_sinv ? *p.x_sinv : 1.f);
#pragma unroll
  for (int i = 0; i < TM; ++i)
#pragma unroll
    for (int j = 0; j < TN; ++j) {
      const int col = ntile * BN + wn * WTN + j * 32 + li;
#pragma unroll
      for (int e = 0; e < 16; ++e) {
        const int row = mtile * BM + wm * WTM + i * 32 + (e & 3) + 8 * (e >> 2) + 4 * lh;
        if (row < p.cout && col < p.ncols) {
          const long long off = (long long)row * p.ncols + col;
          float v = acc[i][j][e] * osc;
          if (p.accumulate) v += out[off];
          out[off] = v;
        }
      }
    }
}

struct ReduceItem {
  const float *slabs;
  float *dw;
  long long n4;
  int splits, accumulate, lanes, block0;
};
struct ReduceBatch {
  ReduceItem it[8];
  int n;
};
__global__ __launch_bounds__(256) void wgrad_reduce_batch_kernel(ReduceBatch b) {
  __shared__ float4 sh[256];
  int k = 0;
  for (int i = 1; i < b.n; ++i) k += (int)blockIdx.x >= b.it[i].block0;
  const ReduceItem &r = b.it[k];
  const int cols = 256 / r.lanes;
  const int c = threadIdx.x % cols, l = threadIdx.x / cols;
  const long long i = (long long)(blockIdx.x - r.block0) * cols + c;
  float4 s = make_float4(0.f, 0.f, 0.f, 0.f);
  if (i < r.n4)
    for (int q = l; q < r.splits; q += r.lanes) {
      const float4 v = reinterpret_cast<const float4 *>(r.slabs)[(long long)q * r.n4 + i];
      s.x += v.x;
      s.y += v.y;
      s.z += v.z;
      s.w += v.w;
    }
  sh[threadIdx.x] = s;
  __syncthreads();
  if (l == 0 && i < r.n4) {
    float4 t = r.accumulate ? reinterpret_cast<const float4 *>(r.dw)[i] : make_float4(0.f, 0.f, 0.f, 0.f);
    for (int q = 0; q < r.lanes; ++q) {
      const float4 v = sh[q * cols + c];
      t.x += v.x;
      t.y += v.y;
      t.z += v.z;
      t.w += v.w;
    }
    reinterpret_cast<float4 *>(r.dw)[i] = t;
  }
}

__global__ __launch_bounds__(256) void stem_rowwindow_kernel(const float4 *__restrict__ x, uint4 *__restrict__ xw, long long n, int h, int w) {
  const int wo = w >> 1;
  for (long long i = (long long)blockIdx.x * 256 + threadIdx.x; i < n; i += (long long)gridDim.x * 256) {
    const int q = (int)(i & 3);
    const long long t = i >> 2;
    const int ox = (int)(t % wo);
    const long long row = t / wo;
    const int c0 = 2 * ox - 4 + 2 * q;
    float v[8] = {0.f, 0.f, 0.f, 0.f, 0.f, 0.f, 0.f, 0.f};
    if (c0 >= 0 && c0 < w) {
      const float4 a = x[row * w + c0], b = x[row * w + c0 + 1];
      v[0] = a.x; v[1] = a.y; v[2] = a.z; v[3] = a.w; v[4] = b.x; v[5] = b.y; v[6] = b.z; v[7] = b.w;
    }
    uint4 q1, q2;
    split2_chunk(v, q1, q2);
    xw[SP_NP * i] = q1;
    xw[SP_NP * i + 1] = q2;
  }
}

__global__ __launch_bounds__(256) void stem_rowwindow_nchw_kernel(const float *__restrict__ x, uint4 *__restrict__ xw, long long n, int h, int w) {
  const int wo = w >> 1;
  const long long plane = (long long)h * w;
  for (long long i = (long long)blockIdx.x * 256 + threadIdx.x; i < n; i += (long long)gridDim.x * 256) {
    const int q = (int)(i & 3);
    const long long t = i >> 2;
    const int ox = (int)(t % wo);
    const long long row = t / wo;
    const long long img = row / h;
    const int yy = (int)(row - img * h);
    const int c0 = 2 * ox - 4 + 2 * q;
    float v[8] = {0.f, 0.f, 0.f, 0.f, 0.f, 0.f, 0.f, 0.f};
    if (c0 >= 0 && c0 < w) {
      const float *src = x + img * 3 * plane + (long long)yy * w + c0;
      const float2 r = *reinterpret_cast<const float2 *>(src), g = *reinterpret_cast<const float2 *>(src + plane),
                   b = *reinterpret_cast<const float2 *>(src + 2 * plane);
      v[0] = r.x; v[1] = g.x; v[2] = b.x; v[4] = r.y; v[5] = g.y; v[6] = b.y;
    }
    uint4 q1, q2;
    split2_chunk(v, q1, q2);
    xw[SP_NP * i] = q1;
    xw[SP_NP * i + 1] = q2;
  }
}

static int validate_split(const mvg_conv_desc *d) {
  if (validate(d)) return 2;
  MVG_REQUIRE(d->cin % 32 == 0 && d->cout % 32 == 0, "split conv: cin and cout must be multiples of 32 (got %d, %d)", d->cin,
              d->cout);
  MVG_REQUIRE(d->r * d->s <= 32, "split conv: at most 32 filter taps");
  return 0;
}

static int split_tile_rows(int ncols, int taps, long long rows) { return (ncols < 128 && taps > 1 && rows >= 65536) ? 256 : SP_BM; }

template <bool DGRAD>
static int launch_igemm_split(IgemmParams &p, hipStream_t st, bool lin = false, int bm = SP_BM) {
  int bn = p.ncols >= 128 ? 128 : 64;
  if (lin && bn == 128 && p.ncls == 1) {
    const long long t128 = (long long)p.groups * ceil_div(p.cls[0].rows_per_group, bm) * ceil_div(p.ncols, 128);
    if (2 * t128 <= compute_cus()) bn = 64;
  }
  MVG_REQUIRE(bm == SP_BM || (bm == 256 && bn == 64 && !lin), "split conv: 256-row tiles go with 64 columns");
  p.ntiles = ceil_div(p.ncols, bn);
  p.splits = 1;
  p.sk_tiles = 0;
  long long tiles = 0;
  p.bn_parts = 0;
  for (int i = 0; i < p.ncls; ++i) {
    IgemmClass &c = p.cls[i];
    c.mtiles_per_group = ceil_div(c.rows_per_group, bm);
    c.KT = ceil_div(c.ktotal, SP_BK);
    c.korder = c.ntaps > 1 ? 1 : 0;
    c.per_div = make_fastdiv((unsigned)(c.ntaps > 0 ? c.ntaps : 1));
    c.tile0 = (int)tiles;
    c.unit0 = 0;
    c.part0 = p.bn_parts;
    p.bn_parts += c.mtiles_per_group;
    tiles += (long long)p.groups * c.mtiles_per_group * p.ntiles;
    MVG_REQUIRE((c.ntaps >= 1 || (DGRAD && p.bn_part)) && c.ntaps <= 32 && c.ktotal % SP_BK == 0, "split conv: class shape not covered");
  }
  MVG_REQUIRE(tiles < (1LL << 31), "split conv: grid too large");
  if (tiles <= 0) return 0;
  p.nt_out = (!lin && !(DGRAD && p.cls_step == 2)) ? 1 : 0;
  dim3 grid((unsigned)tiles), block(256);
  int kt_max = 0;
  for (int i = 0; i < p.ncls; ++i) kt_max = p.cls[i].KT > kt_max ? p.cls[i].KT : kt_max;
  const bool pipelined = tiles <= 2LL * compute_cus() || (tiles <= 4LL * compute_cus() && kt_max >= 48);
  if (lin) {
    if (bn == 128 && pipelined) hipLaunchKernelGGL((igemm_split16_kernel<128, DGRAD, true, 2, 2>), grid, block, 0, st, p);
    else if (bn == 128) hipLaunchKernelGGL((igemm_split16_kernel<128, DGRAD, true>), grid, block, 0, st, p);
    else if (pipelined) hipLaunchKernelGGL((igemm_split16_kernel<64, DGRAD, true, 2, 2>), grid, block, 0, st, p);
    else hipLaunchKernelGGL((igemm_split16_kernel<64, DGRAD, true>), grid, block, 0, st, p);
  } else if (bm == 256) hipLaunchKernelGGL((igemm_split16_kernel<64, DGRAD, false, 4>), grid, block, 0, st, p);
  else if (bn == 128 && pipelined) hipLaunchKernelGGL((igemm_split16_kernel<128, DGRAD, false, 2, 2>), grid, block, 0, st, p);
  else if (bn == 128) hipLaunchKernelGGL((igemm_split16_kernel<128, DGRAD>), grid, block, 0, st, p);
  else hipLaunchKernelGGL((igemm_split16_kernel<64, DGRAD>), grid, block, 0, st, p);
  return check_launch(DGRAD ? "conv_dgrad_split" : "conv_fprop_split");
}

}

using namespace mvg;

extern "C" {

int mvg_split_f32(const float *x, void *out_sp, int64_t n, float scale, void *stream) {
  MVG_REQUIRE(x && out_sp && n >= 0 && n % 8 == 0, "split_f32: null argument or n %% 8 != 0");
  MVG_REQUIRE(scale > 0.f, "split_f32: scale must be positive (a power of two keeps the round trip exact)");
  if (n == 0) return 0;
  hipStream_t st = (hipStream_t)stream;
  ProfScope ps(MVG_K_LAYOUT, st, 0.0, (4.0 + SP_BYTES) * (double)n);
  long long blocks = (n / 8 + 255) / 256;
  if (blocks > 8192) blocks = 8192;
  hipLaunchKernelGGL(split_f32_kernel, dim3((unsigned)blocks), dim3(256), 0, st, (const float4 *)x, (uint4 *)out_sp, (long long)(n / 8), scale);
  return check_launch("split_f32");
}

int mvg_merge_sp(const void *x_sp, float *out, int64_t n, float inv_scale, void *stream) {
  MVG_REQUIRE(x_sp && out && n >= 0 && n % 8 == 0, "merge_sp: null argument or n %% 8 != 0");
  if (n == 0) return 0;
  hipStream_t st = (hipStream_t)stream;
  ProfScope ps(MVG_K_LAYOUT, st, 0.0, (4.0 + SP_BYTES) * (double)n);
  long long blocks = (n / 8 + 255) / 256;
  if (blocks > 8192) blocks = 8192;
  hipLaunchKernelGGL(merge_sp_kernel, dim3((unsigned)blocks), dim3(256), 0, st, (const uint4 *)x_sp, (float4 *)out, (long long)(n / 8), inv_scale);
  return check_launch("merge_sp");
}

int mvg_split_weights(const mvg_conv_desc *d, const float *w, void *w_krsc_sp, void *w_crsk_sp, float *stat2, void *items_dev,
                      void *stream) {
  MVG_REQUIRE(d && w && w_krsc_sp && stat2 && items_dev, "split_weights: null argument");
  if (validate_split(d)) return 2;
  hipStream_t st = (hipStream_t)stream;
  WPrepItem it;
  memset(&it, 0, sizeof(it));
  it.w = w;
  it.wk = w_krsc_sp;
  it.wt = w_crsk_sp;
  it.cout = d->cout;
  it.rs = d->r * d->s;
  it.cin = d->cin;
  it.cin_pad = d->cin;
  it.stat = stat2;
  static_assert(sizeof(WPrepItem) <= 64, "WPrepItem grew: update the callers' table record size");
  hipLaunchKernelGGL(wprep_stage_item_kernel, dim3(1), dim3(64), 0, st, it, (WPrepItem *)items_dev);
  if (check_launch("split_weights: staging the table record")) return 1;
  const long long n8 = (long long)d->cout * it.rs * d->cin / 8;
  long long blocks = (n8 + 256 * 8 - 1) / (256 * 8);
  return mvg_weights_prep_batch(items_dev, 1, 1, (int)(blocks < 16 ? 16 : (blocks > 2048 ? 2048 : blocks)), stream);
}

int mvg_weights_prep_batch(const void *items_dev, int n, int mode, int blocks_per_item, void *stream) {
  MVG_REQUIRE(items_dev != nullptr && n > 0 && (mode == 0 || mode == 1) && blocks_per_item >= 0 && blocks_per_item <= 4096,
              "weights_prep_batch: bad arguments");
  hipStream_t st = (hipStream_t)stream;
  ProfScope ps(MVG_K_LAYOUT, st, 0.0, 0.0);
  const unsigned bx = blocks_per_item > 0 ? (unsigned)blocks_per_item : 64u;
  if (mode == 1) {
    hipLaunchKernelGGL(weights_absmax_kernel, dim3(bx > 64 ? bx / 2 : 16, (unsigned)n), dim3(256), 0, st, (const WPrepItem *)items_dev);
    if (check_launch("weights_absmax")) return 1;
  }
  hipLaunchKernelGGL(weights_prep_batch_kernel, dim3(bx, (unsigned)n), dim3(256), 0, st, (const WPrepItem *)items_dev, mode);
  return check_launch("weights_prep_batch");
}

int mvg_conv_stats_partials_split(const mvg_conv_desc *d, int32_t *rows_per_partial) {
  if (validate_split(d)) return -1;
  const long long rows = (long long)d->n * d->ho * d->wo;
  if (rows_per_partial) *rows_per_partial = 64;
  return ceil_div(rows, SP_BM) * 2;
}

struct SplitAffine {
  const float *scale, *shift;
  const void *residual;
  int residual_sp, relu, out_sp;
  int lin;
  float *out_absmax, *out_sinv;
  const float *bias_absmax;
};

static int fprop_split_impl(const mvg_conv_desc *d, const void *x_sp, const float *x_sinv, const void *w_sp, const float *w_sinv,
                            void *y, float *stats, void *stream, const SplitAffine *aff, int stride_w = -1, int pad_w = -1) {
  if (stride_w < 0 && validate_split(d)) return 2;
  IgemmParams p;
  memset(&p, 0, sizeof(p));
  p.a = (const float *)x_sp;
  p.b = (const float *)w_sp;
  p.a_sinv = x_sinv;
  p.b_sinv = w_sinv;
  p.out = (float *)y;
  p.stats = stats;
  if (aff) {
    p.scale = aff->scale;
    p.bias = aff->shift;
    p.addend = (const float *)aff->residual;
    p.addend_sp = aff->residual_sp;
    p.relu = aff->relu;
    p.out_sp = aff->out_sp;
    p.out_absmax = (unsigned *)aff->out_absmax;
    p.out_sinv = aff->out_sinv;
    p.bias_absmax = aff->bias_absmax;
  }
  if (fprop_geometry(p, d, SP_BYTES, SP_BYTES, "split conv", stride_w, pad_w)) return 2;
  MVG_REQUIRE(p.rows_per_group * (long long)d->cout < (1ll << 31), "split conv: a group of the output exceeds 2^31 elements");
  const double flops = 2.0 * d->groups * (double)p.rows_per_group * d->cout * d->r * d->s * d->cin * (stride_w >= 0 ? 147.0 / 224.0 : 1.0);
  const double bytes = (double)SP_BYTES * (d->groups * (double)d->n * d->h * d->w * d->cin + (double)d->cout * d->r * d->s * d->cin) +
                       4.0 * d->groups * (double)p.rows_per_group * d->cout;
  const bool lin = d->r == 1 && d->s == 1 && d->h == 1 && d->w == 1;
  ProfScope ps(lin ? MVG_K_LINEAR_FPROP : MVG_K_CONV_FPROP, (hipStream_t)stream, flops, bytes);
  p.stats_partials = ceil_div(p.rows_per_group, SP_BM) * 2;
  const bool lin_k = aff && aff->lin;
  return launch_igemm_split<false>(p, (hipStream_t)stream, lin_k, lin_k ? SP_BM : split_tile_rows(d->cout, d->r * d->s, p.rows_per_group));
}

int mvg_conv_fprop_split(const mvg_conv_desc *d, const void *x_sp, const float *x_sinv, const void *w_sp, const float *w_sinv, float *y,
                         float *stats, void *stream) {
  return fprop_split_impl(d, x_sp, x_sinv, w_sp, w_sinv, y, stats, stream, nullptr);
}

int mvg_conv_fprop_split_affine(const mvg_conv_desc *d, const void *x_sp, const float *x_sinv, const void *w_sp, const float *w_sinv,
                                void *out, int out_sp, const float *scale, const float *shift, const void *residual, int residual_sp,
                                int relu, void *stream) {
  MVG_REQUIRE(scale && shift && out, "fprop_split_affine: scale, shift and out are required");
  const SplitAffine a = {scale, shift, residual, residual_sp, relu, out_sp, 0, nullptr, nullptr, nullptr};
  return fprop_split_impl(d, x_sp, x_sinv, w_sp, w_sinv, out, nullptr, stream, &a);
}

struct SplitBnFuse {
  const float *y;
  const uint8_t *bits;
  const float *mean, *invstd, *rscale, *rshift;
  float *part;
  int part_rows;
};

static int dgrad_split_impl(const mvg_conv_desc *d, const void *dy_sp, const float *dy_sinv, const void *w_crsk_sp, const float *w_sinv,
                            float *dx, const float *addend, void *stream, const SplitBnFuse *bnf, const void *relu_mask_sp = nullptr,
                            bool lin_kernel = false, float *out_absmax = nullptr) {
  if (validate_split(d)) return 2;
  IgemmParams p;
  memset(&p, 0, sizeof(p));
  p.a = (const float *)dy_sp;
  p.b = (const float *)w_crsk_sp;
  p.a_sinv = dy_sinv;
  p.b_sinv = w_sinv;
  p.out = dx;
  p.addend = addend;
  p.mask = (const float *)relu_mask_sp;
  p.mask_sp = relu_mask_sp != nullptr;
  p.out_absmax = (unsigned *)out_absmax;
  if (bnf) {
    p.bn_y = bnf->y;
    p.bn_bits = bnf->bits;
    p.bn_mean = bnf->mean;
    p.bn_invstd = bnf->invstd;
    p.bn_rscale = bnf->rscale;
    p.bn_rshift = bnf->rshift;
    p.bn_part = bnf->part;
    p.bn_part_rows = bnf->part_rows;
  }
  if (dgrad_geometry(p, d, SP_BYTES, SP_BYTES, "split conv")) return 2;
  MVG_REQUIRE((long long)d->n * d->h * d->w * d->cin < (1ll << 31), "split conv: a group of dx exceeds 2^31 elements");
  const double flops = 2.0 * d->groups * (double)d->n * d->ho * d->wo * d->cout * d->r * d->s * d->cin;
  const double bytes = (double)SP_BYTES * (d->groups * (double)d->n * d->ho * d->wo * d->cout + (double)d->cout * d->r * d->s * d->cin) +
                       (bnf ? 8.25 : 4.0) * d->groups * (double)d->n * d->h * d->w * d->cin;
  const bool lin = d->r == 1 && d->s == 1 && d->h == 1 && d->w == 1;
  ProfScope ps(lin ? MVG_K_LINEAR_DGRAD : MVG_K_CONV_DGRAD, (hipStream_t)stream, flops, bytes);
  if (int e = dgrad_classes(p, d, bnf != nullptr, 4, dx, addend, (hipStream_t)stream)) return e;
  if (p.ncls == 0) return 0;
  return launch_igemm_split<true>(p, (hipStream_t)stream, lin_kernel,
                                  lin_kernel ? SP_BM : split_tile_rows(d->cin, d->r * d->s, (long long)d->n * d->h * d->w));
}

int mvg_conv_dgrad_split(const mvg_conv_desc *d, const void *dy_sp, const float *dy_sinv, const void *w_crsk_sp, const float *w_sinv,
                         float *dx, const float *addend, const void *relu_mask_sp, void *stream) {
  MVG_REQUIRE(!relu_mask_sp || d->stride == 1, "dgrad_split: the sp ReLU mask is for stride-1 launches (Linear layers)");
  return dgrad_split_impl(d, dy_sp, dy_sinv, w_crsk_sp, w_sinv, dx, addend, stream, nullptr, relu_mask_sp);
}

int mvg_conv_dgrad_bn_partials_split(const mvg_conv_desc *d) {
  if (validate_split(d)) return -1;
  return dgrad_bn_partials(d, split_tile_rows(d->cin, d->r * d->s, (long long)d->n * d->h * d->w));
}

int mvg_conv_dgrad_split_bnreduce(const mvg_conv_desc *d, const void *dy_sp, const float *dy_sinv, const void *w_crsk_sp,
                                  const float *w_sinv, float *dx, const float *addend, const float *bn_y, const uint8_t *bn_bits,
                                  const float *bn_mean, const float *bn_invstd, const float *relu_scale, const float *relu_shift,
                                  float *partials, float *s1, float *s2, float *dgamma, float *dbeta, int accumulate,
                                  float *mx, const float *bn_gamma, float *dx_dy_sinv, void *stream) {
  MVG_REQUIRE(bn_y && bn_mean && bn_invstd && partials && s1 && s2, "dgrad_split_bnreduce: null argument");
  MVG_REQUIRE((bn_gamma == nullptr) == (dx_dy_sinv == nullptr) && (!dx_dy_sinv || mx), "dgrad_split_bnreduce: bn_gamma, dx_dy_sinv (and mx) go together");
  MVG_REQUIRE(!(bn_bits && relu_scale) && ((relu_scale == nullptr) == (relu_shift == nullptr)),
              "dgrad_split_bnreduce: give the ReLU mask either as bits or as (relu_scale, relu_shift)");
  const int P = mvg_conv_dgrad_bn_partials_split(d);
  MVG_REQUIRE(P > 0, "dgrad_split_bnreduce: bad descriptor");
  const SplitBnFuse f = {bn_y, bn_bits, bn_mean, bn_invstd, relu_scale, relu_shift, partials, mx ? 3 : 2};
  if (dgrad_split_impl(d, dy_sp, dy_sinv, w_crsk_sp, w_sinv, dx, addend, stream, &f)) return 1;
  ProfScope ps(MVG_K_BN_BWD_REDUCE, (hipStream_t)stream, 0.0, 8.0 * d->groups * (double)P * d->cin);
  return bn_bwd_finalize_launch(partials, d->groups, P, d->cin, s1, s2, dgamma, dbeta, accumulate, (hipStream_t)stream, mx, nullptr, nullptr,
                                bn_gamma, bn_invstd, (long long)d->n * d->h * d->w, dx_dy_sinv);
}

static void wgrad_split_tile(const mvg_conv_desc *d, int &bm, int &bn) {
  const int ncols = d->r * d->s * d->cin;
  bm = d->cout >= 128 ? 128 : 64;
  bn = ncols >= 128 ? 128 : 64;
  if (bm == 128 && ncols >= 256 && ncols % 256 == 0) bn = 256;
  else if (ncols % 192 == 0) bn = 192;
}

int mvg_conv_wgrad_splits_split(const mvg_conv_desc *d) {
  if (validate_split(d)) return -1;
  int bm, bn;
  wgrad_split_tile(d, bm, bn);
  const long long tiles = (long long)ceil_div(d->cout, bm) * ceil_div(d->r * d->s * d->cin, bn);
  return wgrad_split_count(tiles, (long long)d->groups * d->n * d->ho * d->wo, bn == 256 ? 2 : 3, 256);
}

static int wgrad_split_impl(const mvg_conv_desc *d, const void *x_sp, const void *dy_sp, const float *dy_sinv, float *dw, float *workspace,
                            int splits, int accumulate, void *stream, int stride_w = -1, int pad_w = -1, const float *x_sinv = nullptr,
                            bool slabs_only = false) {
  if (stride_w < 0 && validate_split(d)) return 2;
  WgradParams p;
  memset(&p, 0, sizeof(p));
  p.x = (const float *)x_sp;
  p.dy = (const float *)dy_sp;
  p.dy_sinv = dy_sinv;
  p.x_sinv = x_sinv;
  if (wgrad_geometry(p, d, SP_BYTES, 16, dw, nullptr, workspace, splits, accumulate, "wgrad_split", stride_w, pad_w)) return 2;
  int bm, bn;
  wgrad_split_tile(d, bm, bn);
  p.mtiles = ceil_div(d->cout, bm);
  p.ntiles = ceil_div(p.ncols, bn);
  hipStream_t st = (hipStream_t)stream;
  const bool lin = d->r == 1 && d->s == 1 && d->h == 1 && d->w == 1;
  {
    const double flops = 2.0 * (double)p.pixels * d->cout * d->r * d->s * d->cin * (stride_w >= 0 ? 147.0 / 224.0 : 1.0);
    const double bytes = (double)SP_BYTES * ((double)d->groups * d->n * d->h * d->w * d->cin + (double)p.pixels * d->cout) +
                         4.0 * (double)d->cout * d->r * d->s * d->cin;
    ProfScope ps(lin ? MVG_K_LINEAR_WGRAD : MVG_K_CONV_WGRAD, st, flops, bytes);
    MVG_REQUIRE((long long)p.mtiles * p.ntiles * splits < (1LL << 31), "wgrad_split: grid too large");
    dim3 grid(p.mtiles * p.ntiles * splits), block(256);
    const bool incr = (long long)d->ho * d->wo >= 32;
#define MVG_WGRAD_SPLIT(BM_, BN_)                                                                  \
  do {                                                                                             \
    if (incr) hipLaunchKernelGGL((wgrad_split_kernel<BM_, BN_, true>), grid, block, 0, st, p);     \
    else hipLaunchKernelGGL((wgrad_split_kernel<BM_, BN_, false>), grid, block, 0, st, p);         \
  } while (0)
    if (bm == 128 && bn == 256) MVG_WGRAD_SPLIT(128, 256);
    else if (bm == 128 && bn == 192) MVG_WGRAD_SPLIT(128, 192);
    else if (bm == 64 && bn == 192) MVG_WGRAD_SPLIT(64, 192);
    else if (bm == 128 && bn == 128) MVG_WGRAD_SPLIT(128, 128);
    else if (bm == 64 && bn == 128) MVG_WGRAD_SPLIT(64, 128);
    else if (bm == 128 && bn == 64) MVG_WGRAD_SPLIT(128, 64);
    else MVG_WGRAD_SPLIT(64, 64);
#undef MVG_WGRAD_SPLIT
    if (check_launch("conv_wgrad_split")) return 1;
  }
  return splits > 1 && !slabs_only ? wgrad_reduce_slabs(p, workspace, dw, nullptr, splits, accumulate, st, "wgrad_split") : 0;
}

int mvg_conv_wgrad_split(const mvg_conv_desc *d, const void *x_sp, const void *dy_sp, const float *dy_sinv, float *dw, float *workspace,
                         int splits, int accumulate, void *stream) {
  return wgrad_split_impl(d, x_sp, dy_sp, dy_sinv, dw, workspace, splits, accumulate, stream);
}

int mvg_conv_wgrad_split_slabs(const mvg_conv_desc *d, const void *x_sp, const void *dy_sp, const float *dy_sinv, float *workspace, int splits,
                               void *stream) {
  MVG_REQUIRE(splits > 1 && workspace, "wgrad_split_slabs: splits > 1 and a workspace (the slabs ARE the result)");
  return wgrad_split_impl(d, x_sp, dy_sp, dy_sinv, workspace, workspace, splits, 0, stream, -1, -1, nullptr, true);
}

int mvg_wgrad_reduce_batch(const float *const *host_slabs, float *const *host_dw, const int64_t *host_n, const int32_t *host_splits,
                           const int32_t *host_accumulate, int n, void *stream) {
  MVG_REQUIRE(host_slabs && host_dw && host_n && host_splits && host_accumulate && n >= 1 && n <= 8, "wgrad_reduce_batch: 1..8 items");
  ReduceBatch b;
  memset(&b, 0, sizeof(b));
  b.n = n;
  long long blocks = 0;
  double bytes = 0.0;
  for (int i = 0; i < n; ++i) {
    MVG_REQUIRE(host_slabs[i] && host_dw[i] && host_n[i] > 0 && host_n[i] % 4 == 0 && host_splits[i] > 1, "wgrad_reduce_batch: bad item");
    ReduceItem &r = b.it[i];
    r.slabs = host_slabs[i];
    r.dw = host_dw[i];
    r.n4 = host_n[i] / 4;
    r.splits = host_splits[i];
    r.accumulate = host_accumulate[i];
    r.lanes = r.splits >= 32 ? 16 : (r.splits >= 8 ? 4 : 1);
    r.block0 = (int)blocks;
    blocks += (r.n4 + 256 / r.lanes - 1) / (256 / r.lanes);
    bytes += 4.0 * host_n[i] * (r.splits + 1);
  }
  MVG_REQUIRE(blocks < (1LL << 31), "wgrad_reduce_batch: grid too large");
  hipStream_t st = (hipStream_t)stream;
  ProfScope ps(MVG_K_WGRAD_REDUCE, st, 0.0, bytes);
  hipLaunchKernelGGL(wgrad_reduce_batch_kernel, dim3((unsigned)blocks), dim3(256), 0, st, b);
  return check_launch("wgrad_reduce_batch");
}

static mvg_conv_desc linear_desc(int rows, int fin, int fout) {
  mvg_conv_desc d;
  memset(&d, 0, sizeof(d));
  d.groups = 1; d.n = rows; d.h = d.w = d.ho = d.wo = 1; d.cin = fin; d.cout = fout; d.r = d.s = 1; d.stride = 1; d.pad = 0;
  return d;
}

int mvg_split_colsum(const float *g, int rows, int cols, const float *absmax, void *out_sp, float *out_sinv, float *db, int accumulate,
                     void *stream) {
  MVG_REQUIRE(g && absmax && out_sp && out_sinv && rows > 0 && cols > 0 && cols % 32 == 0, "split_colsum: null argument or cols %% 32 != 0");
  hipStream_t st = (hipStream_t)stream;
  ProfScope ps(MVG_K_COLSUM, st, 0.0, (4.0 + SP_BYTES) * (double)rows * cols);
  hipLaunchKernelGGL(split_colsum_kernel, dim3(cols / 32), dim3(256), 0, st, g, rows, cols, (const unsigned *)absmax, (uint4 *)out_sp, out_sinv,
                     db, accumulate);
  return check_launch("split_colsum");
}

int mvg_linear_fprop_split(int rows, int fin, int fout, const void *x_sp, const float *x_sinv, const void *w_sp, const float *w_sinv,
                           const float *bias, int relu, void *out, int out_sp, float *out_sinv, const float *bias_absmax,
                           float *out_absmax, void *stream) {
  MVG_REQUIRE(bias != nullptr && out != nullptr, "linear_fprop_split: bias and out are required");
  MVG_REQUIRE(!out_sp || out_sinv, "linear_fprop_split: an sp result needs out_sinv (it is stored scaled)");
  MVG_REQUIRE(!(out_sp && out_absmax), "linear_fprop_split: out_absmax is for fp32 results");
  const mvg_conv_desc d = linear_desc(rows, fin, fout);
  const SplitAffine a = {nullptr, bias, nullptr, 0, relu, out_sp, 1, out_absmax, out_sinv, bias_absmax};
  return fprop_split_impl(&d, x_sp, x_sinv, w_sp, w_sinv, out, nullptr, stream, &a);
}

int mvg_linear_dgrad_split(int rows, int fin, int fout, const void *dy_sp, const float *dy_sinv, const void *wt_sp, const float *w_sinv,
                           float *dx, const float *addend, const void *relu_mask_sp, float *out_absmax, void *stream) {
  const mvg_conv_desc d = linear_desc(rows, fin, fout);
  return dgrad_split_impl(&d, dy_sp, dy_sinv, wt_sp, w_sinv, dx, addend, stream, nullptr, relu_mask_sp, true, out_absmax);
}

int mvg_linear_wgrad_split(int rows, int fin, int fout, const void *x_sp, const float *x_sinv, const void *dy_sp, const float *dy_sinv,
                           float *dw, float *workspace, int splits, int accumulate, void *stream) {
  const mvg_conv_desc d = linear_desc(rows, fin, fout);
  return wgrad_split_impl(&d, x_sp, dy_sp, dy_sinv, dw, workspace, splits, accumulate, stream, -1, -1, x_sinv);
}

static int stem_desc(const mvg_conv_desc *d, mvg_conv_desc *rw) {
  MVG_REQUIRE(d != nullptr, "stem (row-window): null descriptor");
  MVG_REQUIRE(d->r == 7 && d->s == 7 && d->stride == 2 && d->pad == 3 && d->cin == 4, "stem (row-window): 7x7 stride 2 pad 3, 4 stored channels");
  MVG_REQUIRE(d->w % 2 == 0 && d->ho == (d->h - 1) / 2 + 1 && d->wo == d->w / 2, "stem (row-window): even width; ho, wo inconsistent");
  MVG_REQUIRE(d->cout % 32 == 0 && d->groups > 0 && d->n > 0, "stem (row-window): cout must be a multiple of 32");
  *rw = *d;
  rw->w = d->wo;
  rw->cin = 32;
  rw->s = 1;
  return 0;
}

int mvg_stem_rowwindow_split(const float *x_nhwc4, void *xw_sp, int64_t images, int h, int w, void *stream) {
  MVG_REQUIRE(x_nhwc4 && xw_sp && images > 0 && h > 0 && w > 0 && w % 2 == 0, "stem_rowwindow: bad arguments (even width)");
  hipStream_t st = (hipStream_t)stream;
  const long long n = images * h * (w / 2) * 4;
  ProfScope ps(MVG_K_LAYOUT, st, 0.0, 16.0 * (double)images * h * w + 32.0 * (double)n);
  long long blocks = (n + 255) / 256;
  if (blocks > 16384) blocks = 16384;
  hipLaunchKernelGGL(stem_rowwindow_kernel, dim3((unsigned)blocks), dim3(256), 0, st, (const float4 *)x_nhwc4, (uint4 *)xw_sp, n, h, w);
  return check_launch("stem_rowwindow");
}

int mvg_stem_rowwindow_split_nchw(const float *x_nchw, void *xw_sp, int64_t images, int h, int w, void *stream) {
  MVG_REQUIRE(x_nchw && xw_sp && images > 0 && h > 0 && w > 0 && w % 2 == 0, "stem_rowwindow (NCHW): bad arguments (even width)");
  hipStream_t st = (hipStream_t)stream;
  const long long n = images * h * (w / 2) * 4;
  ProfScope ps(MVG_K_LAYOUT, st, 0.0, 12.0 * (double)images * h * w + 32.0 * (double)n);
  long long blocks = (n + 255) / 256;
  if (blocks > 16384) blocks = 16384;
  hipLaunchKernelGGL(stem_rowwindow_nchw_kernel, dim3((unsigned)blocks), dim3(256), 0, st, x_nchw, (uint4 *)xw_sp, n, h, w);
  return check_launch("stem_rowwindow_nchw");
}

int mvg_stem_fprop_split(const mvg_conv_desc *d, const void *xw_sp, const void *w_sp, const float *w_sinv, float *y, float *stats,
                         void *stream) {
  mvg_conv_desc rw;
  if (stem_desc(d, &rw)) return 2;
  return fprop_split_impl(&rw, xw_sp, nullptr, w_sp, w_sinv, y, stats, stream, nullptr, 1, 0);
}

int mvg_stem_wgrad_splits_split(const mvg_conv_desc *d) {
  mvg_conv_desc rw;
  if (stem_desc(d, &rw)) return -1;
  const long long tiles = (long long)ceil_div(rw.cout, rw.cout >= 128 ? 128 : 64) * ceil_div(7 * 32, 128);
  return wgrad_split_count(tiles, (long long)rw.groups * rw.n * rw.ho * rw.wo, 3, 256);
}

int mvg_stem_wgrad_split(const mvg_conv_desc *d, const void *xw_sp, const void *dy_sp, const float *dy_sinv, float *dw_rw, float *workspace,
                         int splits, int accumulate, void *stream) {
  mvg_conv_desc rw;
  if (stem_desc(d, &rw)) return 2;
  return wgrad_split_impl(&rw, xw_sp, dy_sp, dy_sinv, dw_rw, workspace, splits, accumulate, stream, 1, 0);
}

}
```

### rot-mvgaze_amd/ops.py

```python
from __future__ import annotations

import ctypes as C
from typing import Optional

import torch

from ._lib import ConvDesc, K_FAMILIES, ProfEntry, check, lib

Tensor = torch.Tensor


def _p(t: Optional[Tensor]):
    if t is None:
        return None
    assert t.is_cuda and t.dtype in _PTR_DTYPES, (t.device, t.dtype)
    return t.data_ptr()


_PTR_DTYPES = frozenset((torch.float32, torch.int32, torch.uint8, torch.int16, torch.bfloat16, torch.float16))
_workspaces = {}
_MAX_WORKSPACES = 8
_raw_stream = getattr(torch._C, "_cuda_getCurrentRawStream", None)


# ... 70 lines not shown


def cast_weights_bf16(d: ConvDesc, w: Tensor, cin_src: int, need_transposed: bool = True):
    wk = torch.empty(d.cout, d.r, d.s, d.cin, dtype=torch.bfloat16, device=w.device)
    wt = torch.empty(d.cin, d.r, d.s, d.cout, dtype=torch.bfloat16, device=w.device) if need_transposed else None
    check(lib().mvg_cast_weights_bf16(C.byref(d), _p(w), cin_src, _p(wk), _p(wt), _s()), "cast_weights_bf16")
    return wk, wt


def _wgrad_slabs(splits_fn, what: str, d: ConvDesc, n: int, device):
    splits = splits_fn(C.byref(d))
    if splits < 1:
        check(1, what)
    return splits, (torch.empty(splits * n, dtype=torch.float32, device=device) if splits > 1 else None)


def conv_wgrad(d: ConvDesc, x: Tensor, dy: Tensor, dw: Tensor, accumulate: bool = False, defer: Optional[list] = None):
    splits, ws = _wgrad_slabs(_fn("mvg_conv_wgrad_splits", x), "conv_wgrad_splits", d, d.cout * d.r * d.s * d.cin, x.device)
    if defer is not None and splits > 1 and x.dtype == torch.bfloat16 and dw.numel() == d.cout * d.r * d.s * d.cin and dw.numel() % 4 == 0:
        check(lib().mvg_conv_wgrad_bf16_slabs(C.byref(d), _p(x), _p(dy), _p(ws), splits, _s()), "conv_wgrad_bf16_slabs")
        defer.append((ws, dw, splits, bool(accumulate)))
        return
    check(_fn("mvg_conv_wgrad", x)(C.byref(d), _p(x), _p(dy), _p(dw), _p(ws), splits, int(accumulate), _s()), "conv_wgrad")


def linear_wgrad(x: Tensor, dy: Tensor, dw: Tensor, db: Optional[Tensor], rows: int, fin: int, fout: int, accumulate: bool = False):
    d = ConvDesc.linear(rows, fin, fout)
    splits, ws = _wgrad_slabs(lib().mvg_conv_wgrad_splits, "conv_wgrad_splits", d, fout * fin + fout, x.device)
    check(lib().mvg_linear_wgrad(_p(x), _p(dy), _p(dw), _p(db), rows, fin, fout, _p(ws), splits, int(accumulate), _s()),
          "linear_wgrad")


def fuser_fprop(img_feat, feat, rel, row_img, row_src, w, bias, relu, y, rows, cf, nvec, fout):
    ws, n = _linear_ws(img_feat, rows, cf + 3 * nvec, fout)
    check(lib().mvg_fuser_fprop(_p(img_feat), _p(feat), _p(rel), _p(row_img), _p(row_src), _p(w), _p(bias), int(relu), _p(y), rows,
                                cf, nvec, fout, img_feat.numel() // cf, feat.numel() // (3 * nvec), _p(ws), n, _s(True)), "fuser_fprop")


def fuser_wgrad(img_feat, feat, rel, row_img, row_src, dy, dw, db, rows, cf, nvec, fout, accumulate=False):
    fin = cf + 3 * nvec
    d = ConvDesc.linear(rows, fin, fout)
    splits, ws = _wgrad_slabs(lib().mvg_conv_wgrad_splits, "conv_wgrad_splits", d, fout * fin + fout, dy.device)
    check(lib().mvg_fuser_wgrad(_p(img_feat), _p(feat), _p(rel), _p(row_img), _p(row_src), _p(dy), _p(dw), _p(db), rows, cf, nvec,
                                fout, img_feat.numel() // cf, feat.numel() // (3 * nvec), _p(ws), splits, int(accumulate), _s()),
          "fuser_wgrad")


def _sinv(t: Optional[Tensor]):
    return _p(getattr(t, "sinv", None)) if t is not None else None


def sp_empty(*shape, device) -> Tensor:
    assert shape[-1] % 8 == 0
    return torch.empty(*shape[:-1], shape[-1] // 8, 2, 8, dtype=torch.float16, device=device)


def sp_shape(x_sp: Tensor):
    return tuple(x_sp.shape[:-3]) + (x_sp.shape[-3] * 8,)


def is_sp(t: Optional[Tensor]) -> bool:
    return t is not None and t.dtype == torch.float16


def split_f32(x: Tensor, scale: float = 1.0) -> Tensor:
    assert x.dtype == torch.float32 and x.is_contiguous() and x.shape[-1] % 8 == 0
    out = sp_empty(*x.shape, device=x.device)
    check(lib().mvg_split_f32(_p(x), _p(out), x.numel(), float(scale), _s()), "split_f32")
    out.sinv = None if scale == 1.0 else torch.full((1,), 1.0 / scale, dtype=torch.float32, device=x.device)
    return out


def merge_sp(x: Tensor) -> Tensor:
    assert is_sp(x) and x.is_contiguous() and x.shape[-1] == 8 and x.shape[-2] == 2
    out = torch.empty(sp_shape(x), dtype=torch.float32, device=x.device)
    sinv = getattr(x, "sinv", None)
    check(lib().mvg_merge_sp(_p(x), _p(out), out.numel(), float(sinv.item()) if sinv is not None else 1.0, _s()), "merge_sp")
    return out


_items_scratch = {}


def split_weights(d: ConvDesc, w: Tensor, need_transposed: bool = True):
    assert w.dtype == torch.float32 and w.is_cuda
    rs = d.r * d.s
    wk = sp_empty(d.cout, rs * d.cin, device=w.device)
    wt = sp_empty(d.cin, rs * d.cout, device=w.device) if need_transposed else None
    stat = torch.empty(2, dtype=torch.float32, device=w.device)
    items = torch.empty(64, dtype=torch.uint8, device=w.device)
    check(lib().mvg_split_weights(C.byref(d), _p(w), _p(wk), _p(wt), _p(stat), _p(items), _s()), "split_weights")
    wk.sinv = stat[1:2]
    if wt is not None:
        wt.sinv = stat[1:2]
    return wk, wt


def weights_prep_batch(table: Tensor, n: int, mode: int, blocks_per_item: int = 0):
    assert table.is_cuda and table.dtype == torch.int64 and table.is_contiguous() and table.shape == (n, 6)
    check(lib().mvg_weights_prep_batch(C.c_void_p(table.data_ptr()), n, mode, blocks_per_item, _s()), "weights_prep_batch")


def conv_stats_partials_split(d: ConvDesc):
    rpp = C.c_int32(0)
    n = lib().mvg_conv_stats_partials_split(C.byref(d), C.byref(rpp))
    if n < 0:
        check(1, "conv_stats_partials_split")
    return n, rpp.value


def conv_fprop_split(d: ConvDesc, x_sp: Tensor, w_sp: Tensor, y: Tensor, stats: Optional[Tensor] = None):
    check(lib().mvg_conv_fprop_split(C.byref(d), _p(x_sp), _sinv(x_sp), _p(w_sp), _sinv(w_sp), _p(y), _p(stats), _s()), "conv_fprop_split")


def conv_fprop_split_affine(d: ConvDesc, x_sp: Tensor, w_sp: Tensor, out: Tensor, scale: Tensor, shift: Tensor,
                            residual: Optional[Tensor], relu: bool):
    check(lib().mvg_conv_fprop_split_affine(C.byref(d), _p(x_sp), _sinv(x_sp), _p(w_sp), _sinv(w_sp), _p(out), int(is_sp(out)), _p(scale),
                                            _p(shift), _p(residual), int(is_sp(residual)), int(relu), _s()), "conv_fprop_split_affine")


def conv_dgrad_split(d: ConvDesc, dy_sp: Tensor, wt_sp: Tensor, dx: Tensor, addend: Optional[Tensor] = None,
                     relu_mask_sp: Optional[Tensor] = None):
    assert relu_mask_sp is None or (is_sp(relu_mask_sp) and getattr(relu_mask_sp, "sinv", None) is None)
    check(lib().mvg_conv_dgrad_split(C.byref(d), _p(dy_sp), _sinv(dy_sp), _p(wt_sp), _sinv(wt_sp), _p(dx), _p(addend), _p(relu_mask_sp),
                                     _s()), "conv_dgrad_split")


def stem_rowwindow_split(x_nhwc4: Tensor) -> Tensor:
    G, N, H, W, C = x_nhwc4.shape
    assert C == 4 and W % 2 == 0 and x_nhwc4.dtype == torch.float32 and x_nhwc4.is_contiguous()
    xw = sp_empty(G, N, H, W // 2, 32, device=x_nhwc4.device)
    check(lib().mvg_stem_rowwindow_split(_p(x_nhwc4), _p(xw), G * N, H, W, _s()), "stem_rowwindow_split")
    xw.sinv = None
    return xw


def stem_rowwindow_split_nchw(x_nchw: Tensor, out: Tensor):
    B, Cc, H, W = x_nchw.shape
    assert Cc == 3 and W % 2 == 0 and x_nchw.dtype == torch.float32 and x_nchw.is_contiguous() and is_sp(out) and out.is_contiguous()
    assert sp_shape(out) == (B, H, W // 2, 32)
    check(lib().mvg_stem_rowwindow_split_nchw(_p(x_nchw), _p(out), B, H, W, _s()), "stem_rowwindow_split_nchw")


def stem_fprop_split(d: ConvDesc, xw: Tensor, w_sp: Tensor, y: Tensor, stats: Optional[Tensor]):
    check(lib().mvg_stem_fprop_split(C.byref(d), _p(xw), _p(w_sp), _sinv(w_sp), _p(y), _p(stats), _s()), "stem_fprop_split")


def stem_wgrad_split(d: ConvDesc, xw: Tensor, dy_sp: Tensor, dw_rw: Tensor, accumulate: bool = False):
    splits, ws = _wgrad_slabs(lib().mvg_stem_wgrad_splits_split, "stem_wgrad_splits_split", d, d.cout * 224, xw.device)
    check(lib().mvg_stem_wgrad_split(C.byref(d), _p(xw), _p(dy_sp), _sinv(dy_sp), _p(dw_rw), _p(ws), splits, int(accumulate), _s()),
          "stem_wgrad_split")


def bn_relu_maxpool_bwd_reduce_split(g_pooled, argmax, y, mean, invstd, scale, shift, groups, n_per_group, h, w, c, ho, wo, s1, s2,
                                     dgamma, dbeta, accumulate, mx, gamma=None, dy_sinv=None):
    n = lib().mvg_bn_bwd_workspace_floats(groups, n_per_group * h * w, c)
    ws = torch.empty(n, dtype=torch.float32, device=y.device)
    check(lib().mvg_bn_relu_maxpool_bwd_reduce_split(_p(g_pooled), _p(argmax), _p(y), _p(mean), _p(invstd), _p(scale), _p(shift), groups,
                                                     n_per_group, h, w, c, ho, wo, _p(s1), _p(s2), _p(dgamma), _p(dbeta), int(accumulate),
                                                     _p(ws), _p(mx), _p(gamma), _p(dy_sinv), _s(True)), "bn_relu_maxpool_bwd_reduce_split")


def bn_relu_maxpool_bwd_apply_split(g_pooled, argmax, y, mean, invstd, gamma, scale, shift, s1, s2, groups, n_per_group, h, w, c, ho, wo,
                                    dy_sp, mx, dy_sinv=None):
    ready = dy_sinv is not None
    dy_sp.sinv = dy_sinv if ready else torch.empty(1, dtype=torch.float32, device=y.device)
    check(lib().mvg_bn_relu_maxpool_bwd_apply_split(_p(g_pooled), _p(argmax), _p(y), _p(mean), _p(invstd), _p(gamma), _p(scale), _p(shift),
                                                    _p(s1), _p(s2), groups, n_per_group, h, w, c, ho, wo, _p(dy_sp), _p(mx), _p(dy_sp.sinv),
                                                    int(ready), _s()), "bn_relu_maxpool_bwd_apply_split")


def stem_rowwindow_bf16(x_nchw: Tensor, out: Tensor):
    B, Cc, H, W = x_nchw.shape
    assert Cc == 3 and W % 4 == 0 and x_nchw.dtype == torch.float32 and x_nchw.is_contiguous()
    assert out.dtype == torch.bfloat16 and out.shape == (B, H, W // 4, 64) and out.is_contiguous()
    check(lib().mvg_stem_rowwindow_bf16(_p(x_nchw), _p(out), B, H, W, _s()), "stem_rowwindow_bf16")


def stem_fprop_bf16(d: ConvDesc, xw: Tensor, w_fold: Tensor, y: Tensor, stats: Optional[Tensor]):
    check(lib().mvg_stem_fprop_bf16(C.byref(d), _p(xw), _p(w_fold), _p(y), _p(stats), _s()), "stem_fprop_bf16")


def stem_wgrad_bf16(d: ConvDesc, xw: Tensor, dy: Tensor, dw_fold: Tensor, accumulate: bool = False):
    splits, ws = _wgrad_slabs(lib().mvg_stem_wgrad_splits_bf16, "stem_wgrad_splits_bf16", d, 2 * d.cout * 448, xw.device)
    check(lib().mvg_stem_wgrad_bf16(C.byref(d), _p(xw), _p(dy), _p(dw_fold), _p(ws), splits, int(accumulate), _s()), "stem_wgrad_bf16")


def conv_dgrad_bn_partials_split(d: ConvDesc) -> int:
    n = lib().mvg_conv_dgrad_bn_partials_split(C.byref(d))
    if n < 0:
        check(1, "conv_dgrad_bn_partials_split")
    return n


def conv_dgrad_split_bnreduce(d: ConvDesc, dy_sp, wt_sp, dx, addend, bn_y, bn_bits, bn_mean, bn_invstd, relu_affine, s1, s2, dgamma,
                              dbeta, accumulate: bool, mx: Optional[Tensor] = None, bn_gamma: Optional[Tensor] = None,
                              dx_dy_sinv: Optional[Tensor] = None):
    P = conv_dgrad_bn_partials_split(d)
    part = torch.empty(d.groups * P * 3 * d.cin, dtype=torch.float32, device=dx.device)
    rs, rh = relu_affine if relu_affine is not None else (None, None)
    check(lib().mvg_conv_dgrad_split_bnreduce(C.byref(d), _p(dy_sp), _sinv(dy_sp), _p(wt_sp), _sinv(wt_sp), _p(dx), _p(addend), _p(bn_y),
                                              _p(bn_bits), _p(bn_mean), _p(bn_invstd), _p(rs), _p(rh), _p(part), _p(s1), _p(s2),
                                              _p(dgamma), _p(dbeta), int(accumulate), _p(mx), _p(bn_gamma), _p(dx_dy_sinv), _s(True)),
          "conv_dgrad_split_bnreduce")


def conv_dgrad_bf16_bnreduce(d: ConvDesc, dy, wt, dx, addend, bn_y, bn_bits, bn_mean, bn_invstd, relu_affine, s1, s2, dgamma, dbeta,
                             accumulate: bool):
    P = lib().mvg_conv_dgrad_bn_partials_bf16(C.byref(d))
    if P < 1:
        check(1, "conv_dgrad_bn_partials_bf16")
    part = torch.empty(d.groups * P * 2 * d.cin, dtype=torch.float32, device=dx.device)
    rs, rh = relu_affine if relu_affine is not None else (None, None)
    check(lib().mvg_conv_dgrad_bf16_bnreduce(C.byref(d), _p(dy), _p(wt), _p(dx), _p(addend), _p(bn_y), _p(bn_bits), _p(bn_mean),
                                             _p(bn_invstd), _p(rs), _p(rh), _p(part), _p(s1), _p(s2), _p(dgamma), _p(dbeta),
                                             int(accumulate), _s()), "conv_dgrad_bf16_bnreduce")


def conv_wgrad_split(d: ConvDesc, x_sp: Tensor, dy_sp: Tensor, dw: Tensor, accumulate: bool = False, defer: Optional[list] = None):
    splits, ws = _wgrad_slabs(lib().mvg_conv_wgrad_splits_split, "conv_wgrad_splits_split", d, dw.numel(), dw.device)
    assert getattr(x_sp, "sinv", None) is None, "conv_wgrad_split: the activation operand is stored unscaled"
    if defer is not None and splits > 1:
        check(lib().mvg_conv_wgrad_split_slabs(C.byref(d), _p(x_sp), _p(dy_sp), _sinv(dy_sp), _p(ws), splits, _s()), "conv_wgrad_split_slabs")
        defer.append((ws, dw, splits, bool(accumulate)))
        return
    check(lib().mvg_conv_wgrad_split(C.byref(d), _p(x_sp), _p(dy_sp), _sinv(dy_sp), _p(dw), _p(ws), splits, int(accumulate), _s()),
          "conv_wgrad_split")


def wgrad_reduce_batch(items: list):
    for i in range(0, len(items), 8):
        chunk = items[i:i + 8]
        n = len(chunk)
        for ws, dw, splits, acc in chunk:
            assert dw.dtype == torch.float32 and ws.numel() == splits * dw.numel() and dw.numel() % 4 == 0
        check(lib().mvg_wgrad_reduce_batch((C.c_void_p * n)(*[c[0].data_ptr() for c in chunk]), (C.c_void_p * n)(*[c[1].data_ptr() for c in chunk]),
                                           (C.c_int64 * n)(*[c[1].numel() for c in chunk]), (C.c_int32 * n)(*[c[2] for c in chunk]),
                                           (C.c_int32 * n)(*[int(c[3]) for c in chunk]), n, _s()), "wgrad_reduce_batch")
    items.clear()


def bn_apply_split(y, scale, shift, residual, relu, out_sp, groups, rows_per_group, c, residual_affine=None, want_bits=False):
    bits = torch.empty(groups * rows_per_group * c // 4, dtype=torch.uint8, device=y.device) if want_bits else None
    rs, rh = residual_affine if residual_affine is not None else (None, None)
    res_sp = is_sp(residual)
    check(lib().mvg_bn_apply_split(_p(y), _p(scale), _p(shift), _p(residual), int(res_sp), _p(rs), _p(rh), int(relu), _p(out_sp),
                                   _p(bits), groups, rows_per_group, c, _s()), "bn_apply_split")
    return bits


def bn_bwd_reduce_split(g, relu_bits, y, mean, invstd, groups, rows_per_group, c, s1, s2, dgamma, dbeta, accumulate, mx,
                        relu_affine=None, dz_out=None, gamma=None, dy_sinv=None):
    rs, rh = relu_affine if relu_affine is not None else (None, None)
    n = lib().mvg_bn_bwd_workspace_floats(groups, rows_per_group, c)
    ws = torch.empty(n, dtype=torch.float32, device=g.device)
    check(lib().mvg_bn_bwd_reduce_split(_p(g), _p(relu_bits), _p(y), _p(mean), _p(invstd), _p(rs), _p(rh), groups, rows_per_group, c,
                                        _p(s1), _p(s2), _p(dgamma), _p(dbeta), int(accumulate), _p(ws), _p(dz_out), _p(mx), _p(gamma),
                                        _p(dy_sinv), _s(True)), "bn_bwd_reduce_split")


def bn_bwd_apply_split(g, y, mean, invstd, gamma, s1, s2, groups, rows_per_group, c, dy_sp, relu_affine=None, mx=None, dy_sinv=None):
    rs, rh = relu_affine if relu_affine is not None else (None, None)
    assert mx is not None and mx.dtype == torch.float32 and mx.numel() == groups * c
    ready = dy_sinv is not None
    dy_sp.sinv = dy_sinv if ready else torch.empty(1, dtype=torch.float32, device=g.device)
    check(lib().mvg_bn_bwd_apply_split(_p(g), _p(y), _p(mean), _p(invstd), _p(gamma), _p(s1), _p(s2), _p(rs), _p(rh), groups,
                                       rows_per_group, c, _p(dy_sp), _p(mx), _p(dy_sp.sinv), int(ready), _s()), "bn_bwd_apply_split")


def bn_relu_maxpool_fwd_split(y, scale, shift, pooled_sp, argmax, groups, n_per_group, h, w, c, ho, wo):
    check(lib().mvg_bn_relu_maxpool_fwd_split(_p(y), _p(scale), _p(shift), _p(pooled_sp), _p(argmax), groups, n_per_group, h, w, c,
                                              ho, wo, _s()), "bn_relu_maxpool_fwd_split")


def avgpool_fwd_split(x_sp, y, n, hw, c):
    check(lib().mvg_avgpool_fwd_split(_p(x_sp), _p(y), n, hw, c, _s()), "avgpool_fwd_split")


def linear_fprop_mixed(x, w_bf16, bias, relu, y, rows, fin, fout):
    check(lib().mvg_linear_fprop_mixed(_p(x), _p(w_bf16), _p(bias), int(relu), _p(y), rows, fin, fout, _s()), "linear_fprop_mixed")


def linear_dgrad_mixed(dy, wt_bf16, mask, addend, dx, rows, fin, fout):
    check(lib().mvg_linear_dgrad_mixed(_p(dy), _p(wt_bf16), _p(mask), _p(addend), _p(dx), rows, fin, fout, _s()), "linear_dgrad_mixed")


def linear_wgrad_mixed(x, dy, dw, db, rows, fin, fout, accumulate=False):
    d = ConvDesc.linear(rows, fin, fout)
    splits, ws = _wgrad_slabs(lib().mvg_conv_wgrad_splits_bf16, "conv_wgrad_splits_bf16", d, fout * fin + fout, x.device)
    check(lib().mvg_linear_wgrad_mixed(_p(x), _p(dy), _p(dw), _p(db), rows, fin, fout, _p(ws), splits, int(accumulate), _s()),
          "linear_wgrad_mixed")


def _linear_ws(x: Tensor, rows: int, fin: int, fout: int):
    n = lib().mvg_linear_workspace_floats(rows, fin, fout)
    return torch.empty(n, dtype=torch.float32, device=x.device), n


def linear_fprop(x: Tensor, w: Tensor, bias: Optional[Tensor], relu: bool, y: Tensor, rows: int, fin: int, fout: int):
    ws, n = _linear_ws(x, rows, fin, fout)
    check(lib().mvg_linear_fprop(_p(x), _p(w), _p(bias), int(relu), _p(y), rows, fin, fout, _p(ws), n, _s(True)),
          "linear_fprop")


def linear_dgrad(dy: Tensor, w: Tensor, mask: Optional[Tensor], addend: Optional[Tensor], dx: Tensor, rows: int,
                 fin: int, fout: int):
# ... 310 lines not shown
```

Baseline: 1632 samples/s.

## Pack stem input as padded pixel pairs with pitch-based addressing instead of row windows

Replaces the stem's 32-channel row-window materialization with a compact packed layout of padded pixel pairs (8 channels per pair plus four zero pad pairs per row). It adds x_pitch and row_pitch to the implicit-GEMM fprop and wgrad addressing so the stem convolution can read overlapping windows straight from the packed buffer. The goal is to shrink the stem input buffer and the traffic spent writing and reading it. In exchange, more addressing arithmetic runs in the conv kernels, and the window reads overlap, which may hurt load coalescing.

```diff
diff --git a/include/rotmvgaze.h b/include/rotmvgaze.h
--- a/include/rotmvgaze.h
+++ b/include/rotmvgaze.h
@@ -302,6 +302,12 @@
 int mvg_stem_wgrad_splits_split(const mvg_conv_desc *d);
 int mvg_stem_wgrad_split(const mvg_conv_desc *d, const void *xw_sp, const void *dy_sp, const float *dy_sinv, float *dw_rw,
                          float *workspace, int splits, int accumulate, void *stream);
+int mvg_stem_pack_split(const float *x_nhwc4, void *xp_sp, int64_t images, int h, int w, void *stream);
+int mvg_stem_pack_split_nchw(const float *x_nchw, void *xp_sp, int64_t images, int h, int w, void *stream);
+int mvg_stem_fprop_split_packed(const mvg_conv_desc *d, const void *xp_sp, const void *w_sp, const float *w_sinv, float *y,
+                                float *stats, void *stream);
+int mvg_stem_wgrad_split_packed(const mvg_conv_desc *d, const void *xp_sp, const void *dy_sp, const float *dy_sinv, float *dw_rw,
+                                float *workspace, int splits, int accumulate, void *stream);
 int mvg_bn_relu_maxpool_bwd_reduce_split(const float *g_pooled, const uint8_t *argmax, const float *y, const float *mean,
                                          const float *invstd, const float *scale, const float *shift, int groups,
                                          int n_per_group, int h, int w, int c, int ho, int wo, float *s1, float *s2,
diff --git a/rot-mvgaze_amd/_lib.py b/rot-mvgaze_amd/_lib.py
--- a/rot-mvgaze_amd/_lib.py
+++ b/rot-mvgaze_amd/_lib.py
@@ -81,6 +81,10 @@
     "mvg_stem_fprop_split": (_I, [_D, _P, _P, _P, _P, _P, _P]),
     "mvg_stem_wgrad_splits_split": (_I, [_D]),
     "mvg_stem_wgrad_split": (_I, [_D, _P, _P, _P, _P, _P, _I, _I, _P]),
+    "mvg_stem_pack_split": (_I, [_P, _P, _I64, _I, _I, _P]),
+    "mvg_stem_pack_split_nchw": (_I, [_P, _P, _I64, _I, _I, _P]),
+    "mvg_stem_fprop_split_packed": (_I, [_D, _P, _P, _P, _P, _P, _P]),
+    "mvg_stem_wgrad_split_packed": (_I, [_D, _P, _P, _P, _P, _P, _I, _I, _P]),
     "mvg_bn_relu_maxpool_bwd_reduce_split": (_I, [_P, _P, _P, _P, _P, _P, _P, _I, _I, _I, _I, _I, _I, _I, _P, _P, _P, _P, _I, _P, _P, _P, _P, _P]),
     "mvg_bn_relu_maxpool_bwd_apply_split": (_I, [_P, _P, _P, _P, _P, _P, _P, _P, _P, _P, _I, _I, _I, _I, _I, _I, _I, _P, _P, _P, _I, _P]),
     "mvg_conv_dgrad_bn_partials_split": (_I, [_D]),
diff --git a/rot-mvgaze_amd/backbone.py b/rot-mvgaze_amd/backbone.py
--- a/rot-mvgaze_amd/backbone.py
+++ b/rot-mvgaze_amd/backbone.py
@@ -28,17 +28,19 @@
 
 class _Unit:
     __slots__ = ("spec", "desc", "x_in", "y", "out", "mean", "invstd", "relu", "rows", "w", "trained", "pool",
-                 "relu_affine", "fused_s12", "relu_bits", "split", "stem_rw")
+                 "relu_affine", "fused_s12", "relu_bits", "split", "stem_rw", "stem_packed")
 
     def __init__(self):
         self.split = False
         self.stem_rw = False
+        self.stem_packed = False
         self.relu_bits = None
         self.fused_s12 = None
 
 
 class Backbone:
     _guard_scale = 1
+    _stem_packed = True
     _debug_units: Optional[list] = None
 
     def __init__(self, depth: int, params: Dict[str, Tensor], prefix: str = "_feat_extractor.0."):
@@ -67,6 +69,7 @@
         self._wg_defer: Optional[list] = None
         self._split_now = self.split
         self._stem_rw = False
+        self._stem_pk = False
         self._stem_w8 = None
 
     @property
@@ -159,6 +162,7 @@
         sp_out = self._split_now and training and not bf
         sp_in = sp_out and c.cin != 3
         stem_rw = c.cin == 3 and self._stem_rw and (sp_out or bf)
+        stem_pk = stem_rw and not bf and self._stem_pk
         if (sp_in or bf or stem_rw) and self._wprep is not None:
             w, w_t = self._wprep[c.name]
         elif sp_in:
@@ -181,6 +185,8 @@
         def fprop(stats_buf):
             if stem_rw and bf:
                 ops.stem_fprop_bf16(d, x, w, y, stats_buf)
+            elif stem_pk:
+                ops.stem_fprop_split_packed(d, x, w, y, stats_buf)
             elif stem_rw:
                 ops.stem_fprop_split(d, x, w, y, stats_buf)
             elif sp_in:
@@ -270,6 +276,7 @@
             u.trained = training
             u.split = sp_in
             u.stem_rw = stem_rw
+            u.stem_packed = stem_pk
             u.relu_affine = (scale, shift) if (relu and residual is None and not pool) else None
             if pool:
                 u.pool = (argmax, scale, shift, d.ho, d.wo, hp, wp_)
@@ -307,11 +314,15 @@
             self._stem_rw = (self.stem_rowwindow and training and W % 4 == 0 and (B * ho * (wo // 2)) % 64 == 0 and self.batch_weight_prep
                              and self.spec.stem.k == 7)
         else:
+            op_bytes = B * H * (W + 8) * 16 if self._stem_packed else 32 * B * H * (W // 2) * 4
             self._stem_rw = (self._split_now and self.stem_rowwindow and training and not need_dimg and W % 2 == 0
-                             and self.batch_weight_prep and 32 * B * H * (W // 2) * 4 < 0x7FFFFFF0)
+                             and self.batch_weight_prep and op_bytes < 0x7FFFFFF0)
+        self._stem_pk = self._stem_rw and not self.bf16 and self._stem_packed
         direct = self._stem_rw and not raw
         if direct and self.bf16:
             x0 = torch.empty(V, B, H, W // 4, 64, dtype=self.act_dtype, device=dev)
+        elif direct and self._stem_pk:
+            x0 = ops.stem_packed_empty(V, B, H=H, W=W, device=dev)
         elif direct:
             x0 = ops.sp_empty(V, B, H, W // 2, 32, device=dev)
             x0.sinv = None
@@ -323,6 +334,8 @@
                 assert im.dtype == torch.float32
                 if self.bf16:
                     ops.stem_rowwindow_bf16(im.detach().contiguous(), x0[v])
+                elif self._stem_pk:
+                    ops.stem_pack_split_nchw(im.detach().contiguous(), x0[v])
                 else:
                     ops.stem_rowwindow_split_nchw(im.detach().contiguous(), x0[v])
             elif self.bf16 and raw:
@@ -336,7 +349,7 @@
                 assert im.dtype == torch.float32
                 ops.nchw_to_nhwc4(im.detach().contiguous(), x0[v], B, 3, H, W)
         if self._stem_rw and not direct:
-            x0 = ops.stem_rowwindow_split(x0)
+            x0 = ops.stem_pack_split(x0) if self._stem_pk else ops.stem_rowwindow_split(x0)
         self._wprep = None
         if training:
             self.invalidate_weight_cache()
@@ -504,7 +517,7 @@
             gv.add_(dw16[c.cout:, :, 3:10, :3])
         elif u.stem_rw:
             dw8 = torch.empty(c.cout, 7, 8, 4, dtype=torch.float32, device=dy.device)
-            ops.stem_wgrad_split(u.desc, u.x_in, dy, dw8, False)
+            (ops.stem_wgrad_split_packed if u.stem_packed else ops.stem_wgrad_split)(u.desc, u.x_in, dy, dw8, False)
             gv = sink.view(wp).permute(0, 2, 3, 1)
             if sink.accumulate(wp):
                 gv.add_(dw8[:, :, 1:, :3])
diff --git a/rot-mvgaze_amd/csrc/conv_shared.h b/rot-mvgaze_amd/csrc/conv_shared.h
--- a/rot-mvgaze_amd/csrc/conv_shared.h
+++ b/rot-mvgaze_amd/csrc/conv_shared.h
@@ -114,6 +114,7 @@
   const int *rc_row_img, *rc_row_src;
   int rc_cf, rc_nvec, rc_nvec_shift;
   long long rc_img_bytes, rc_feat_bytes;
+  int x_pitch, row_pitch;
 };
 
 __device__ __forceinline__ int xcd_remap(int orig, int nwg) {
@@ -143,6 +144,8 @@
   const float *dy_sinv;
   const float *x_sinv;
   int stride_w, pad_w;
+  int x_pitch, row_pitch;
+  long long x_img_stride;
 };
 
 static __global__ __launch_bounds__(256) void wgrad_reduce_kernel(const float *__restrict__ slabs, float *__restrict__ dw,
@@ -229,7 +232,7 @@
 }
 
 static int fprop_geometry(IgemmParams &p, const mvg_conv_desc *d, int a_elem, int b_elem, const char *what, int stride_w = -1,
-                          int pad_w = -1) {
+                          int pad_w = -1, int x_pitch = 0, int row_pitch = 0) {
   p.groups = d->groups;
   p.out_h = d->ho;
   p.out_w = d->wo;
@@ -250,7 +253,9 @@
   p.b_row_len = p.ktotal;
   p.cin = d->cin;
   p.rows_per_group = (long long)d->n * d->ho * d->wo;
-  p.src_img_stride = (long long)d->h * d->w * d->cin;
+  p.x_pitch = x_pitch > 0 ? x_pitch : d->cin;
+  p.row_pitch = row_pitch > 0 ? row_pitch : d->w * d->cin;
+  p.src_img_stride = (long long)d->h * p.row_pitch;
   p.imgs_per_group = d->n;
   p.ntaps = d->r * d->s;
   p.tap_ns = d->s;
@@ -285,6 +290,8 @@
   p.ktotal = d->r * d->s * d->cout;
   p.b_row_len = p.ktotal;
   p.cin = d->cin;
+  p.x_pitch = d->cout;
+  p.row_pitch = d->wo * d->cout;
   p.src_img_stride = (long long)d->ho * d->wo * d->cout;
   p.imgs_per_group = d->n;
   p.full_h = d->h;
@@ -360,7 +367,8 @@
 }
 
 static int wgrad_geometry(WgradParams &p, const mvg_conv_desc *d, int elem, int px_align, float *dw, float *db, float *workspace,
-                          int splits, int accumulate, const char *what, int stride_w = -1, int pad_w = -1) {
+                          int splits, int accumulate, const char *what, int stride_w = -1, int pad_w = -1, int x_pitch = 0,
+                          int row_pitch = 0) {
   MVG_REQUIRE(splits >= 1, "%s: splits < 1", what);
   MVG_REQUIRE(splits == 1 || workspace != nullptr, "%s: workspace required for splits > 1", what);
   p.h = d->h;
@@ -378,13 +386,16 @@
   p.ncols = d->r * d->s * d->cin;
   p.pixels = (long long)d->groups * d->n * d->ho * d->wo;
   p.pixels_per_split = ((p.pixels + splits - 1) / splits + px_align - 1) / px_align * px_align;
-  p.x_bytes = (long long)elem * d->groups * d->n * d->h * d->w * d->cin;
+  p.x_pitch = x_pitch > 0 ? x_pitch : d->cin;
+  p.row_pitch = row_pitch > 0 ? row_pitch : d->w * d->cin;
+  p.x_img_stride = (long long)d->h * p.row_pitch;
+  p.x_bytes = (long long)elem * d->groups * d->n * p.x_img_stride;
   p.ohw_div = make_fastdiv((unsigned)(d->ho * d->wo));
   p.wo_div = make_fastdiv((unsigned)d->wo);
   p.cin_div = make_fastdiv((unsigned)d->cin);
   p.s_div = make_fastdiv((unsigned)d->s);
   MVG_REQUIRE(p.pixels_per_split * d->cout * elem < 0x7FFFFFF0ll, "%s: split too large for 32-bit offsets", what);
-  MVG_REQUIRE((long long)elem * (p.pixels_per_split / (d->ho * d->wo) + 2) * d->h * d->w * d->cin < 0x7FFFFFF0ll,
+  MVG_REQUIRE((long long)elem * (p.pixels_per_split / (d->ho * d->wo) + 2) * p.x_img_stride < 0x7FFFFFF0ll,
               "%s: split too large for 32-bit offsets", what);
   p.out = splits == 1 ? dw : workspace;
   p.accumulate = (splits == 1) ? accumulate : 0;
diff --git a/rot-mvgaze_amd/csrc/conv_split.hip b/rot-mvgaze_amd/csrc/conv_split.hip
--- a/rot-mvgaze_amd/csrc/conv_split.hip
+++ b/rot-mvgaze_amd/csrc/conv_split.hip
@@ -264,7 +264,7 @@
     const int oy = (int)fdiv((unsigned)rem, c.ow_div), ox = rem - oy * c.out_w;
     const int y0 = DGRAD ? oy + c.cls_cy : oy * p.stride - p.pad;
     const int x0 = DGRAD ? ox + c.cls_cx : ox * p.stride_w - p.pad_w;
-    const unsigned base = (unsigned)(img * p.src_img_stride * SP_BYTES) + (unsigned)((y0 * p.src_w + x0) * p.src_c) * (unsigned)SP_BYTES;
+    const unsigned base = (unsigned)(img * p.src_img_stride * SP_BYTES) + (unsigned)(y0 * p.row_pitch + x0 * p.x_pitch) * (unsigned)SP_BYTES;
     unsigned msk = 0;
     for (int t = 0; t < c.ntaps; ++t) {
       const int fr = (int)fdiv((unsigned)t, c.tap_ns_div), fs = t - fr * c.tap_ns;
@@ -306,7 +306,7 @@
     const int tap_u = c.ntaps > 1 ? (ks >> p.src_c_shift) : 0;
     const int chb = ks - (tap_u << p.src_c_shift);
     const int fru = (int)fdiv((unsigned)tap_u, c.tap_ns_div), fsu = tap_u - fru * c.tap_ns;
-    const int disp = (fru * p.src_w + fsu) * p.src_c;
+    const int disp = fru * p.row_pitch + fsu * p.x_pitch;
     const unsigned sdelta = (unsigned)(((DGRAD ? -disp : disp) + chb) * SP_BYTES);
     unsigned kb = (unsigned)ks * (unsigned)SP_BYTES;
     if (DGRAD) {
@@ -432,7 +432,7 @@
   const char *dy = reinterpret_cast<const char *>(p.dy);
   const char *x = reinterpret_cast<const char *>(p.x);
   const __amdgpu_buffer_rsrc_t rs_a = make_rsrc(dy + m_begin * p.cout * SP_BYTES, (long long)SP_BYTES * m_count * p.cout);
-  const long long x_img_elems = (long long)p.h * p.w * p.cin;
+  const long long x_img_elems = p.x_img_stride;
   const __amdgpu_buffer_rsrc_t rs_b = make_rsrc(x + img0 * x_img_elems * SP_BYTES, p.x_bytes - (long long)SP_BYTES * img0 * x_img_elems);
   const int i_row = tid / A_TPR, i_v0 = tid % A_TPR;
   unsigned a_off[A_CPT];
@@ -458,9 +458,9 @@
     const int fr = (int)fdiv((unsigned)tap, p.s_div), fs = tap - fr * p.s;
     i_dy[j] = fr - p.pad;
     i_dx[j] = fs - p.pad_w;
-    i_tconst[j] = (unsigned)((i_dy[j] * p.w + i_dx[j]) * p.cin + cc) * (unsigned)SP_BYTES;
-  }
-  const unsigned row_bytes = (unsigned)(p.stride * p.w * p.cin) * (unsigned)SP_BYTES, col_bytes = (unsigned)(p.stride_w * p.cin) * (unsigned)SP_BYTES;
+    i_tconst[j] = (unsigned)(i_dy[j] * p.row_pitch + i_dx[j] * p.x_pitch + cc) * (unsigned)SP_BYTES;
+  }
+  const unsigned row_bytes = (unsigned)(p.stride * p.row_pitch) * (unsigned)SP_BYTES, col_bytes = (unsigned)(p.stride_w * p.x_pitch) * (unsigned)SP_BYTES;
   const unsigned img_bytes = (unsigned)x_img_elems * (unsigned)SP_BYTES;
   int s_oy = 0, s_ox = 0;
   unsigned s_imgoff = 0;
@@ -675,6 +675,47 @@
   }
 }
 
+__global__ __launch_bounds__(256) void stem_pack_kernel(const float4 *__restrict__ x, uint4 *__restrict__ xp, long long n, int h, int w) {
+  const int wp = (w >> 1) + 4;
+  for (long long i = (long long)blockIdx.x * 256 + threadIdx.x; i < n; i += (long long)gridDim.x * 256) {
+    const int pp = (int)(i % wp);
+    const long long row = i / wp;
+    const int c0 = 2 * pp - 4;
+    float v[8] = {0.f, 0.f, 0.f, 0.f, 0.f, 0.f, 0.f, 0.f};
+    if (c0 >= 0 && c0 < w) {
+      const float4 a = x[row * w + c0], b = x[row * w + c0 + 1];
+      v[0] = a.x; v[1] = a.y; v[2] = a.z; v[3] = a.w; v[4] = b.x; v[5] = b.y; v[6] = b.z; v[7] = b.w;
+    }
+    uint4 q1, q2;
+    split2_chunk(v, q1, q2);
+    xp[SP_NP * i] = q1;
+    xp[SP_NP * i + 1] = q2;
+  }
+}
+
+__global__ __launch_bounds__(256) void stem_pack_nchw_kernel(const float *__restrict__ x, uint4 *__restrict__ xp, long long n, int h, int w) {
+  const int wp = (w >> 1) + 4;
+  const long long plane = (long long)h * w;
+  for (long long i = (long long)blockIdx.x * 256 + threadIdx.x; i < n; i += (long long)gridDim.x * 256) {
+    const int pp = (int)(i % wp);
+    const long long row = i / wp;
+    const long long img = row / h;
+    const int yy = (int)(row - img * h);
+    const int c0 = 2 * pp - 4;
+    float v[8] = {0.f, 0.f, 0.f, 0.f, 0.f, 0.f, 0.f, 0.f};
+    if (c0 >= 0 && c0 < w) {
+      const float *src = x + img * 3 * plane + (long long)yy * w + c0;
+      const float2 r = *reinterpret_cast<const float2 *>(src), g = *reinterpret_cast<const float2 *>(src + plane),
+                   b = *reinterpret_cast<const float2 *>(src + 2 * plane);
+      v[0] = r.x; v[1] = g.x; v[2] = b.x; v[4] = r.y; v[5] = g.y; v[6] = b.y;
+    }
+    uint4 q1, q2;
+    split2_chunk(v, q1, q2);
+    xp[SP_NP * i] = q1;
+    xp[SP_NP * i + 1] = q2;
+  }
+}
+
 static int validate_split(const mvg_conv_desc *d) {
   if (validate(d)) return 2;
   MVG_REQUIRE(d->cin % 32 == 0 && d->cout % 32 == 0, "split conv: cin and cout must be multiples of 32 (got %d, %d)", d->cin,
@@ -813,7 +854,8 @@
 };
 
 static int fprop_split_impl(const mvg_conv_desc *d, const void *x_sp, const float *x_sinv, const void *w_sp, const float *w_sinv,
-                            void *y, float *stats, void *stream, const SplitAffine *aff, int stride_w = -1, int pad_w = -1) {
+                            void *y, float *stats, void *stream, const SplitAffine *aff, int stride_w = -1, int pad_w = -1,
+                            int x_pitch = 0, int row_pitch = 0) {
   if (stride_w < 0 && validate_split(d)) return 2;
   IgemmParams p;
   memset(&p, 0, sizeof(p));
@@ -834,10 +876,10 @@
     p.out_sinv = aff->out_sinv;
     p.bias_absmax = aff->bias_absmax;
   }
-  if (fprop_geometry(p, d, SP_BYTES, SP_BYTES, "split conv", stride_w, pad_w)) return 2;
+  if (fprop_geometry(p, d, SP_BYTES, SP_BYTES, "split conv", stride_w, pad_w, x_pitch, row_pitch)) return 2;
   MVG_REQUIRE(p.rows_per_group * (long long)d->cout < (1ll << 31), "split conv: a group of the output exceeds 2^31 elements");
   const double flops = 2.0 * d->groups * (double)p.rows_per_group * d->cout * d->r * d->s * d->cin * (stride_w >= 0 ? 147.0 / 224.0 : 1.0);
-  const double bytes = (double)SP_BYTES * (d->groups * (double)d->n * d->h * d->w * d->cin + (double)d->cout * d->r * d->s * d->cin) +
+  const double bytes = (double)SP_BYTES * (d->groups * (double)d->n * (double)p.src_img_stride + (double)d->cout * d->r * d->s * d->cin) +
                        4.0 * d->groups * (double)p.rows_per_group * d->cout;
   const bool lin = d->r == 1 && d->s == 1 && d->h == 1 && d->w == 1;
   ProfScope ps(lin ? MVG_K_LINEAR_FPROP : MVG_K_CONV_FPROP, (hipStream_t)stream, flops, bytes);
@@ -952,7 +994,7 @@
 
 static int wgrad_split_impl(const mvg_conv_desc *d, const void *x_sp, const void *dy_sp, const float *dy_sinv, float *dw, float *workspace,
                             int splits, int accumulate, void *stream, int stride_w = -1, int pad_w = -1, const float *x_sinv = nullptr,
-                            bool slabs_only = false) {
+                            bool slabs_only = false, int x_pitch = 0, int row_pitch = 0) {
   if (stride_w < 0 && validate_split(d)) return 2;
   WgradParams p;
   memset(&p, 0, sizeof(p));
@@ -960,7 +1002,8 @@
   p.dy = (const float *)dy_sp;
   p.dy_sinv = dy_sinv;
   p.x_sinv = x_sinv;
-  if (wgrad_geometry(p, d, SP_BYTES, 16, dw, nullptr, workspace, splits, accumulate, "wgrad_split", stride_w, pad_w)) return 2;
+  if (wgrad_geometry(p, d, SP_BYTES, 16, dw, nullptr, workspace, splits, accumulate, "wgrad_split", stride_w, pad_w, x_pitch, row_pitch))
+    return 2;
   int bm, bn;
   wgrad_split_tile(d, bm, bn);
   p.mtiles = ceil_div(d->cout, bm);
@@ -969,7 +1012,7 @@
   const bool lin = d->r == 1 && d->s == 1 && d->h == 1 && d->w == 1;
   {
     const double flops = 2.0 * (double)p.pixels * d->cout * d->r * d->s * d->cin * (stride_w >= 0 ? 147.0 / 224.0 : 1.0);
-    const double bytes = (double)SP_BYTES * ((double)d->groups * d->n * d->h * d->w * d->cin + (double)p.pixels * d->cout) +
+    const double bytes = (double)SP_BYTES * ((double)d->groups * d->n * (double)p.x_img_stride + (double)p.pixels * d->cout) +
                          4.0 * (double)d->cout * d->r * d->s * d->cin;
     ProfScope ps(lin ? MVG_K_LINEAR_WGRAD : MVG_K_CONV_WGRAD, st, flops, bytes);
     MVG_REQUIRE((long long)p.mtiles * p.ntiles * splits < (1LL << 31), "wgrad_split: grid too large");
@@ -1127,4 +1170,47 @@
   return wgrad_split_impl(&rw, xw_sp, dy_sp, dy_sinv, dw_rw, workspace, splits, accumulate, stream, 1, 0);
 }
 
-}
+static void stem_packed_pitches(const mvg_conv_desc *rw, int *x_pitch, int *row_pitch) {
+  *x_pitch = 8;
+  *row_pitch = (rw->w + 4) * 8;
+}
+
+static int stem_pack_launch(bool nchw, const float *x, void *xp_sp, int64_t images, int h, int w, void *stream) {
+  MVG_REQUIRE(x && xp_sp && images > 0 && h > 0 && w > 0 && w % 2 == 0, "stem_pack: bad arguments (even width)");
+  hipStream_t st = (hipStream_t)stream;
+  const long long n = images * h * (w / 2 + 4);
+  ProfScope ps(MVG_K_LAYOUT, st, 0.0, (nchw ? 12.0 : 16.0) * (double)images * h * w + 32.0 * (double)n);
+  long long blocks = (n + 255) / 256;
+  if (blocks > 16384) blocks = 16384;
+  if (nchw) hipLaunchKernelGGL(stem_pack_nchw_kernel, dim3((unsigned)blocks), dim3(256), 0, st, x, (uint4 *)xp_sp, n, h, w);
+  else hipLaunchKernelGGL(stem_pack_kernel, dim3((unsigned)blocks), dim3(256), 0, st, (const float4 *)x, (uint4 *)xp_sp, n, h, w);
+  return check_launch(nchw ? "stem_pack_nchw" : "stem_pack");
+}
+
+int mvg_stem_pack_split(const float *x_nhwc4, void *xp_sp, int64_t images, int h, int w, void *stream) {
+  return stem_pack_launch(false, x_nhwc4, xp_sp, images, h, w, stream);
+}
+
+int mvg_stem_pack_split_nchw(const float *x_nchw, void *xp_sp, int64_t images, int h, int w, void *stream) {
+  return stem_pack_launch(true, x_nchw, xp_sp, images, h, w, stream);
+}
+
+int mvg_stem_fprop_split_packed(const mvg_conv_desc *d, const void *xp_sp, const void *w_sp, const float *w_sinv, float *y, float *stats,
+                                void *stream) {
+  mvg_conv_desc rw;
+  if (stem_desc(d, &rw)) return 2;
+  int xp, rp;
+  stem_packed_pitches(&rw, &xp, &rp);
+  return fprop_split_impl(&rw, xp_sp, nullptr, w_sp, w_sinv, y, stats, stream, nullptr, 1, 0, xp, rp);
+}
+
+int mvg_stem_wgrad_split_packed(const mvg_conv_desc *d, const void *xp_sp, const void *dy_sp, const float *dy_sinv, float *dw_rw,
+                                float *workspace, int splits, int accumulate, void *stream) {
+  mvg_conv_desc rw;
+  if (stem_desc(d, &rw)) return 2;
+  int xp, rp;
+  stem_packed_pitches(&rw, &xp, &rp);
+  return wgrad_split_impl(&rw, xp_sp, dy_sp, dy_sinv, dw_rw, workspace, splits, accumulate, stream, 1, 0, nullptr, false, xp, rp);
+}
+
+}
diff --git a/rot-mvgaze_amd/ops.py b/rot-mvgaze_amd/ops.py
--- a/rot-mvgaze_amd/ops.py
+++ b/rot-mvgaze_amd/ops.py
@@ -246,6 +246,48 @@
           "stem_wgrad_split")
 
 
+def stem_packed_empty(*lead, H: int, W: int, device) -> Tensor:
+    assert W % 2 == 0
+    xp = sp_empty(*lead, H, W // 2 + 4, 8, device=device)
+    xp.sinv = None
+    return xp
+
+
+def stem_pack_split(x_nhwc4: Tensor) -> Tensor:
+    G, N, H, W, C = x_nhwc4.shape
+    assert C == 4 and W % 2 == 0 and x_nhwc4.dtype == torch.float32 and x_nhwc4.is_contiguous()
+    xp = stem_packed_empty(G, N, H=H, W=W, device=x_nhwc4.device)
+    check(lib().mvg_stem_pack_split(_p(x_nhwc4), _p(xp), G * N, H, W, _s()), "stem_pack_split")
+    return xp
+
+
+def stem_pack_split_nchw(x_nchw: Tensor, out: Tensor):
+    B, Cc, H, W = x_nchw.shape
+    assert Cc == 3 and W % 2 == 0 and x_nchw.dtype == torch.float32 and x_nchw.is_contiguous() and is_sp(out) and out.is_contiguous()
+    assert sp_shape(out) == (B, H, W // 2 + 4, 8)
+    check(lib().mvg_stem_pack_split_nchw(_p(x_nchw), _p(out), B, H, W, _s()), "stem_pack_split_nchw")
+
+
+def stem_packed_windows(xp: Tensor) -> Tensor:
+    assert is_sp(xp) and xp.is_contiguous() and xp.shape[-3:] == (1, 2, 8)
+    *lead, H, wp = xp.shape[:-3]
+    st = xp.stride()
+    pair = st[len(lead) + 1]
+    return xp.as_strided((*lead, H, wp - 4, 4, 2, 8), (*st[:len(lead) + 1], pair, pair, 8, 1), xp.storage_offset())
+
+
+def stem_fprop_split_packed(d: ConvDesc, xp: Tensor, w_sp: Tensor, y: Tensor, stats: Optional[Tensor]):
+    assert is_sp(xp) and xp.is_contiguous() and sp_shape(xp)[-3:] == (d.h, d.w // 2 + 4, 8)
+    check(lib().mvg_stem_fprop_split_packed(C.byref(d), _p(xp), _p(w_sp), _sinv(w_sp), _p(y), _p(stats), _s()), "stem_fprop_split_packed")
+
+
+def stem_wgrad_split_packed(d: ConvDesc, xp: Tensor, dy_sp: Tensor, dw_rw: Tensor, accumulate: bool = False):
+    assert is_sp(xp) and xp.is_contiguous() and sp_shape(xp)[-3:] == (d.h, d.w // 2 + 4, 8)
+    splits, ws = _wgrad_slabs(lib().mvg_stem_wgrad_splits_split, "stem_wgrad_splits_split", d, d.cout * 224, xp.device)
+    check(lib().mvg_stem_wgrad_split_packed(C.byref(d), _p(xp), _p(dy_sp), _sinv(dy_sp), _p(dw_rw), _p(ws), splits, int(accumulate), _s()),
+          "stem_wgrad_split_packed")
+
+
 def bn_relu_maxpool_bwd_reduce_split(g_pooled, argmax, y, mean, invstd, scale, shift, groups, n_per_group, h, w, c, ho, wo, s1, s2,
                                      dgamma, dbeta, accumulate, mx, gamma=None, dy_sinv=None):
     n = lib().mvg_bn_bwd_workspace_floats(groups, n_per_group * h * w, c)
```

Result: no change. 1647 samples/s (median of 6 runs) (+0.9%).
